# WilliamYi96/HGR-Net

Hardware: AMD Instinct MI355X
Metric: images/sec over 21K-class hierarchy, batch 512; hit@1 parity vs reference (higher is better)
Workload: dtype f16

## Files before the change

hgr-net_amd/_lib.py:

```python
from __future__ import annotations

import ctypes as C
import os
from pathlib import Path

import torch

_HERE = Path(__file__).resolve().parent
LIB_PATH = Path(os.environ.get("HGR_LIB", _HERE / "lib" / "libhgr.so"))

HGR_BF16, HGR_F16 = 0, 1
EPI_NONE, EPI_BIAS, EPI_BIAS_QUICKGELU, EPI_BIAS_RESIDUAL, EPI_BIAS_RELU, EPI_BIAS_ADD16_RELU, EPI_ACCUM, EPI_QGELU_GRAD16 = 0, 1, 2, 3, 4, 5, 6, 7

_p, _i, _l, _f = C.c_void_p, C.c_int, C.c_int64, C.c_float

SIGNATURES = {
    "hgr_gemm_nt": [_p, _l, _p, _l, _p, _l, _p, _p, _l, _i, _i, _i, _i, _i, _i, _p],
    "hgr_gemm_set_tile": [_i],
    "hgr_gemm_set_tail": [_i, _i],
    "hgr_gemm_set_persist": [_i],
    "hgr_gemm_set_p8": [_i],
    "hgr_im2col_patches": [_p, _p, _i, _i, _i, _i, _i, _p],
    "hgr_im2col_patches_ex": [_p, _p, _i, _i, _i, _i, _i, _i, _i, _p],
    "hgr_vit_assemble": [_p, _p, _p, _i, _i, _i, _p],
    "hgr_preprocess_bicubic": [_p, _p, _p, _p, _p, _p, _i, _p, _p, _i, _p, _p, C.POINTER(C.c_float), C.POINTER(C.c_float), _i, _i, _p],
    "hgr_im2col_patches_u8": [_p, _p, _i, _i, _i, _i, _i, _i, C.POINTER(C.c_float), C.POINTER(C.c_float), _i, _p],
    "hgr_vit_embed_ln": [_p, _p, _p, _p, _p, _p, _i, _i, _i, _f, _p],
    "hgr_layernorm": [_p, _p, _p, _p, _i, _i, _l, _p, _f, _i, _i, _p],
    "hgr_mha": [_p, _p, _i, _i, _i, _i, _i, _p],
    "hgr_mha_rows": [_p, _p, _i, _i, _i, _i, _i, _i, _p],
    "hgr_mha_stats": [_p, _p, _p, _i, _i, _i, _i, _i, _p],
    "hgr_text_embed": [_p, _l, _p, _p, _p, _i, _i, _i, _i, _p],
    "hgr_eot_index": [_p, _l, _p, _i, _i, _p],
    "hgr_l2norm_rows": [_p, _p, _p, _i, _i, _i, _p],
    "hgr_topk_rows": [_p, _l, _p, _i, _i, _p, _p, _i, _p],
    "hgr_level_argmax": [_p, _l, _p, _i, _p, _i, _p, _p, _i, _p],
    "hgr_eval_rows": [_p, _l, _i, _p, _p, _p, _i, _i, _p, _p, _p, _i, _i, _p, _p, _p, _i, _p],
    "hgr_conv3x3_nhwc": [_p, _p, _p, _p, _i, _i, _i, _i, _i, _i, _i, _i, _p],
    "hgr_conv3x3_pool2_nhwc": [_p, _p, _p, _p, _i, _i, _i, _i, _i, _i, _i, _p],
    "hgr_stem_conv1": [_p, _p, _p, _p, _i, _i, _i, _i, _i, _p],
    "hgr_stem_im2col": [_p, _p, _i, _i, _i, _p],
    "hgr_avgpool2_nhwc": [_p, _p, _i, _i, _i, _i, _i, _p],
    "hgr_attnpool_tokens": [_p, _p, _p, _i, _i, _i, _i, _p],
    "hgr_attnpool_attend": [_p, _p, _p, _p, _i, _i, _i, _i, _p],
    "hgr_stem7_pool": [_p, _p, _p, _p, _i, _i, _i, _i, _p],
    "hgr_stem7_im2col": [_p, _p, _i, _i, _i, _i, _p],
    "hgr_maxpool3s2_nhwc": [_p, _p, _i, _i, _i, _i, _i, _p],
    "hgr_subsample2_nhwc": [_p, _p, _i, _i, _i, _i, _i, _p],
    "hgr_meanpool_nhwc": [_p, _p, _i, _i, _i, _i, _i, _i, _p],
    "hgr_transpose16": [_p, _l, _p, _l, _i, _i, _p],
    "hgr_transpose16_colsum": [_p, _l, _p, _l, _i, _i, _i, _p, _i, _f, _p, _p],
    "hgr_colsum": [_p, _l, _i, _i, _i, _i, _p, _i, _f, _p, _p],
    "hgr_cast16": [_p, _p, _l, _i, _p],
    "hgr_cast16_transpose": [_p, _l, _p, _l, _p, _l, _i, _i, _i, _p],
    "hgr_quickgelu16": [_p, _p, _p, _l, _i, _i, _p],
    "hgr_layernorm_bwd": [_p, _i, _p, _p, _p, _p, _p, _p, _i, _i, _l, _p, _f, _i, _p],
    "hgr_layernorm_bwd_cast": [_p, _i, _p, _p, _p, _p, _p, _p, _p, _i, _i, _l, _p, _f, _i, _p],
    "hgr_layernorm_bwd_cast_colsum": [_p, _i, _p, _p, _p, _p, _p, _p, _p, _p, _i, _i, _l, _p, _f, _i, _p],
    "hgr_layernorm_bwd_scratch_floats": [_i, _i],
    "hgr_mha_bwd": [_p, _p, _p, _p, _i, _i, _i, _i, _i, _p],
    "hgr_mha_bwd_stats": [_p, _p, _p, _p, _p, _i, _i, _i, _i, _i, _p],
    "hgr_mha_bwd_colsum": [_p, _p, _p, _p, _p, _p, _i, _i, _i, _i, _i, _p],
    "hgr_ce_rows": [_p, _l, _p, _i, _i, _f, _p, _p, _l, _p],
    "hgr_l2norm_bwd": [_p, _p, _p, _i, _i, _i, _p],
    "hgr_matmul_f32": [_p, _l, _l, _p, _l, _l, _p, _l, _i, _i, _i, _f, _i, _p],
    "hgr_embed_scatter_add": [_p, _l, _p, _p, _i, _i, _i, _i, _p],
    "hgr_rows_axpy": [_p, _l, _p, _p, _i, _i, _f, _p],
    "hgr_rows_gather": [_p, _p, _p, _i, _i, _p],
    "hgr_ctx_splice": [_p, _p, _p, _i, _i, _i, _i, _p],
    "hgr_ctx_splice_bwd": [_p, _p, _i, _i, _i, _i, _p],
    "hgr_sumsq": [_p, _l, _p, _p],
    "hgr_eval_counters": [_p, _i, _p, _i, _p, _p, _i, _p, _p, _i, _p, _i, _p],
    "hgr_eval_counters_rows": [_p, _i, _p, _p, _p, _i, _p, _p, _p, _i, _p, _i, _p],
    "hgr_eval_report_rows": [_p, _i, _p, _p, _p, _i, _p, _p, _p, _i, _p, _i, _p],
    "hgr_path_scores": [_p, _l, _p, _l, _i, _p, _p, _p, _i, _p],
    "hgr_subtree_hedge": [_p, _l, _i, _p, _p, _p, _f, _p, _i, _p, _p, _p, _l, _i, _p],
    "hgr_hedge_counters_rows": [_p, _i, _p, _p, _p, _i, _p, _i, _p],
    "hgr_set_ranks": [_p, _l, _i, _p, _p, _i, _p, _p, _p, _i, _p],
    "hgr_set_counters_rows": [_p, _p, _i, _p, _p, _i, _p, _p, _p, _i, _p, _i, _p],
    "hgr_dgp_score_rows": [_p, _l, _i, _i, _i, _f, _p, _i, _p, _i, _p, _p, _p, _p, _i, _i, _p],
    "hgr_dot_f32":[_p, _p, _l, _p, _f, _i, _p],
    "hgr_conv3x3_nhwc_plain": [_p, _p, _p, _i, _i, _i, _i, _i, _i, _i, _p],
    "hgr_gemm_nt_splitk": [_p, _l, _p, _l, _p, _l, _i, _i, _i, _i, _i, _p],
    "hgr_gemm_tn_splitk": [_p, _l, _p, _l, _p, _l, _i, _i, _i, _i, _i, _p],
    "hgr_gemm_tn_tile": [_i, _i],
    "hgr_gemm_plan_capture": [_p, _i],
    "hgr_conv3x3_wgrad_splitk": [_p, _l, _p, _p, _l, _i, _i, _i, _i, _i, _i, _i, _p],
    "hgr_relu_bwd16": [_p, _p, _p, _l, _i, _p],
    "hgr_add16": [_p, _p, _p, _l, _i, _p],
    "hgr_avgpool2_bwd_nhwc": [_p, _p, _i, _i, _i, _i, _i, _p],
    "hgr_attnpool_tokens_bwd": [_p, _p, _i, _i, _i, _i, _p],
    "hgr_im2col3x3_t": [_p, _p, _i, _i, _i, _i, _l, _i, _p],
    "hgr_bn_fold": [_p, _p, _p, _p, _p, _f, _p, _p, _i, _i, _i, _i, _i, _p],
    "hgr_bn_unfold_grad": [_p, _l, _p, _p, _p, _p, _p, _f, _p, _p, _p, _i, _i, _i, _p],
    "hgr_csr_group_aggregate": [_p, _l, _p, _p, _p, _p, _i, _p, _p, _p, _p, _i, _p, _p, _p, _p, _i, _p, _p, _l, _i, _f, _i, _p],
    "hgr_csr_group_att_grad": [_p, _l, _p, _p, _l, _p, _l, _p, _l, _p, _p, _p, _p, _i, _p, _p, _p, _i, _p, _p, _p, _i, _p, _p, _i, _f, _p],
    "hgr_dgp_loss_head": [_p, _l, _p, _p, _l, _i, _i, _p, _p, _p, _l, _i, _p],
    "hgr_dropout_counter": [_p, _l, _p, _l, _i, _i, _i, _i, _i, _p],
    "hgr_adam_l2": [_p, _p, _p, _p, _l, _f, _f, _f, _f, _f, _i, _p],
    "hgr_cnzsl_std_chain_fwd": [_p, _l, _p, _p, _p, _p, _p, _p, _l, _p, _l, _p, _i, _i, _i, _f, _f, _p],
    "hgr_cnzsl_std_chain_bwd": [_p, _l, _p, _l, _p, _l, _p, _p, _p, _l, _p, _i, _i, _f, _p],
    "hgr_bias_relu_f32": [_p, _l, _p, _p, _l, _i, _i, _p],
    "hgr_relu_bwd_colsum_f32": [_p, _l, _p, _l, _p, _l, _p, _p, _i, _i, _p],
    "hgr_gemm_nt_res_stats": [_p, _l, _p, _l, _p, _p, _l, _p, _p, _i, _i, _i, _i, _p],
    "hgr_vit_head": [_p, _p, _l, _l, _p, _p, _f, _p, _p, _i, _i, _i, _i, _p],
    "hgr_gemm_nt_res_stats_guard": [_p, _l, _p, _l, _p, _p, _l, _p, _p, _f, _p, _i, _i, _i, _i, _p],
    "hgr_gemm_nt_res_stats_wide_ok": [_l, _l, _l, _l, _l, _l, _i],
    "hgr_gemm_nt_res_stats_wide": [_p, _l, _p, _l, _p, _p, _l, _p, _p, _f, _p, _i, _i, _i, _i, _p],
    "hgr_gemm_nt_ln": [_p, _l, _p, _l, _p, _l, _p, _p, _p, _f, _i, _i, _i, _i, _i, _p],
    "hgr_gemm_nt_ln_mha": [_p, _l, _p, _l, _p, _p, _p, _f, _p, _l, _i, _i, _i, _i, _i, _p],
    "hgr_gemm_nt_bias_gelu_dual": [_p, _l, _p, _l, _p, _l, _p, _l, _p, _i, _i, _i, _i, _p],
    "hgr_gemm_nt_qgelu_grad_colsum": [_p, _l, _p, _l, _p, _l, _p, _l, _p, _i, _i, _i, _i, _p],
    "hgr_vit_embed_ln_stats": [_p, _p, _p, _p, _p, _p, _p, _p, _i, _i, _i, _f, _i, _p],
    "hgr_vit_patch_embed_ln_ok": [_i, _i, _i, _i, _i],
    "hgr_vit_patch_embed_ln": [_p, _p, _p, _p, _p, _p, _p, _p, _p, _i, _i, _i, _i, _f, _i, _p],
    "hgr_row_stats16": [_p, _p, _p, _p, _i, _i, _i, _p],
    "hgr_pair_rows_f32": [_p, _p, _p, _i, _i, _l, _p, _i, _p],
    "hgr_logits_eval_workspace_bytes": [_i, _i],
    "hgr_logits_eval": [_p, _p, _i, _i, _i, _p, _p, _p, _i, _p, _p, _i, _p, _i, _i, _p, _p, _p, _p, _i, _p],
    "hgr_logits_eval_tile_stage": [_p, _p, _i, _i, _i, _p, _p, _p, _i, _p, _p, _i, _p, _i, _i, _p, _p, _p, _p, _i, _p],
    "hgr_logits_eval_row_stage": [_p, _p, _i, _i, _i, _p, _p, _p, _i, _p, _p, _i, _p, _i, _i, _p, _p, _p, _p, _i, _p],
    "hgr_comm_unique_id": [_p],
    "hgr_comm_init": [_i, _i, _p],
    "hgr_comm_destroy": [],
    "hgr_comm_rank": [],
    "hgr_comm_world": [],
    "hgr_allreduce": [_p, _p, _l, _i, _i, _p],
    "hgr_allgather": [_p, _p, _l, _i, _p],
    "hgr_broadcast": [_p, _l, _i, _i, _p],
    "hgr_adamw": [_p, _p, _p, _p, _l, _f, _f, _f, _f, _f, _i, _p, _f, _f, _p],
    "hgr_normal_counter": [_p, _l, _p, _i, _i, _i, _i, _l, _p],
    "hgr_free_gen_input": [_p, _l, _i, _p, _l, _p, _l, _i, _p, _i, _i, _i, _i, _i, _i, _i, _l, _p],
    "hgr_bias_act_rows": [_p, _l, _p, _p, _l, _l, _i, _i, _i, _i, _p],
    "hgr_free_fr_tail": [_p, _l, _p, _p, _l, _p, _l, _l, _i, _p, _l, _i, _i, _i, _i, _l, _p],
    "hgr_nll_rows16": [_p, _l, _p, _i, _i, _p, _p, _l, _p, _l, _i, _p],
    "hgr_adam_l2_cast16": [_p, _p, _l, _i, _f, _p, _p, _p, _l, _f, _f, _f, _f, _f, _i, _i, _p],
}


class GemmLaunch(C.Structure):
    _fields_ = [(name, C.c_int32) for name in ("kernel", "variant", "epilogue", "out_f32", "act", "grid_x", "grid_y", "tiles_m", "tiles_n", "total",
                                                "nbig", "big_panels", "tiles_m_half", "group", "m_fastest", "vec_ok", "row0", "rows")]


class HgrError(RuntimeError):
    pass


_lib = None


ABI_VERSION = 5


def load() -> C.CDLL:
    global _lib
    if _lib is not None:
        return _lib
    if not LIB_PATH.is_file():
        raise HgrError(f"{LIB_PATH} not found: build it with `python -c 'import __graft_entry__ as g; g.build()'` "
                       f"or `make -C {_HERE / 'csrc'}`; there is no CPU fallback")
    lib = C.CDLL(str(LIB_PATH))
    lib.hgr_abi_version.restype = _i
    lib.hgr_last_error.restype = C.c_char_p
    for name, argtypes in SIGNATURES.items():
        fn = getattr(lib, name)
        fn.argtypes = argtypes
        fn.restype = _l if name.endswith(("_scratch_floats", "_workspace_bytes")) else _i
    if lib.hgr_abi_version() != ABI_VERSION:
        raise HgrError(f"libhgr.so ABI {lib.hgr_abi_version()} != {ABI_VERSION} (include/hgr.h): stale build, run `make -C {_HERE / 'csrc'}`")
    _lib = lib
    return lib


import threading

_tls = threading.local()


def set_muted(on: bool) -> bool:
    prev = getattr(_tls, "muted", False)
    _tls.muted = bool(on)
    return prev


def muted() -> bool:
    return getattr(_tls, "muted", False)


def call(name: str, *args) -> None:
    if getattr(_tls, "muted", False):
        return
    lib = load()
    rc = getattr(lib, name)(*args)
    if rc != 0:
        raise HgrError(f"{name} failed ({rc}): {lib.hgr_last_error().decode()}")
```

hgr-net_amd/clip/model.py:

```python
from __future__ import annotations

import os
from collections import OrderedDict
from typing import Dict, Optional, Tuple, Union

import numpy as np
import torch
from torch import nn

from .. import ops
from .._lib import (EPI_BIAS, EPI_BIAS_ADD16_RELU, EPI_BIAS_QUICKGELU, EPI_BIAS_RELU, EPI_BIAS_RESIDUAL, EPI_NONE,
                    HgrError)


class QuickGELU(nn.Module):
    """Placeholder so ``mlp`` keeps the reference's child names (c_fc, gelu, c_proj); the activation
    itself is fused into the c_fc GEMM epilogue (HGR_EPI_BIAS_QUICKGELU)."""


class ResidualAttentionBlock(nn.Module):
    def __init__(self, d_model: int, n_head: int):
        super().__init__()
        self.attn = nn.MultiheadAttention(d_model, n_head)
        self.ln_1 = nn.LayerNorm(d_model)
        self.mlp = nn.Sequential(OrderedDict([("c_fc", nn.Linear(d_model, d_model * 4)), ("gelu", QuickGELU()),
                                              ("c_proj", nn.Linear(d_model * 4, d_model))]))
        self.ln_2 = nn.LayerNorm(d_model)


class Transformer(nn.Module):
    def __init__(self, width: int, layers: int, heads: int):
        super().__init__()
        self.width, self.layers, self.heads = width, layers, heads
        self.resblocks = nn.Sequential(*[ResidualAttentionBlock(width, heads) for _ in range(layers)])


class VisionTransformer(nn.Module):
    def __init__(self, input_resolution: int, patch_size: int, width: int, layers: int, heads: int, output_dim: int):
        super().__init__()
        self.input_resolution, self.output_dim, self.patch_size = input_resolution, output_dim, patch_size
        self.conv1 = nn.Conv2d(3, width, kernel_size=patch_size, stride=patch_size, bias=False)
        scale = width ** -0.5
        grid = input_resolution // patch_size
        self.class_embedding = nn.Parameter(scale * torch.randn(width))
        self.positional_embedding = nn.Parameter(scale * torch.randn(grid * grid + 1, width))
        self.ln_pre = nn.LayerNorm(width)
        self.transformer = Transformer(width, layers, heads)
        self.ln_post = nn.LayerNorm(width)
        self.proj = nn.Parameter(scale * torch.randn(width, output_dim))


class _Bottleneck(nn.Module):
    def __init__(self, inplanes, planes, stride=1):
        super().__init__()
        self.conv1 = nn.Conv2d(inplanes, planes, 1, bias=False)
        self.bn1 = nn.BatchNorm2d(planes)
        self.conv2 = nn.Conv2d(planes, planes, 3, padding=1, bias=False)
        self.bn2 = nn.BatchNorm2d(planes)
        self.conv3 = nn.Conv2d(planes, planes * 4, 1, bias=False)
        self.bn3 = nn.BatchNorm2d(planes * 4)
        self.stride = stride
        self.downsample = None
        if stride > 1 or inplanes != planes * 4:
            self.downsample = nn.Sequential(OrderedDict([("-1", nn.AvgPool2d(stride)),
                                                         ("0", nn.Conv2d(inplanes, planes * 4, 1, bias=False)),
                                                         ("1", nn.BatchNorm2d(planes * 4))]))


class _AttentionPool2d(nn.Module):
    def __init__(self, spacial_dim, embed_dim, num_heads, output_dim):
        super().__init__()
        self.positional_embedding = nn.Parameter(torch.randn(spacial_dim ** 2 + 1, embed_dim) / embed_dim ** 0.5)
        self.k_proj = nn.Linear(embed_dim, embed_dim)
        self.q_proj = nn.Linear(embed_dim, embed_dim)
        self.v_proj = nn.Linear(embed_dim, embed_dim)
        self.c_proj = nn.Linear(embed_dim, output_dim)
        self.num_heads = num_heads


class ModifiedResNet(nn.Module):

    def __init__(self, layers, output_dim, heads, input_resolution=224, width=64):
        super().__init__()
        self.output_dim, self.input_resolution = output_dim, input_resolution
        self.conv1 = nn.Conv2d(3, width // 2, 3, stride=2, padding=1, bias=False)
        self.bn1 = nn.BatchNorm2d(width // 2)
        self.conv2 = nn.Conv2d(width // 2, width // 2, 3, padding=1, bias=False)
        self.bn2 = nn.BatchNorm2d(width // 2)
        self.conv3 = nn.Conv2d(width // 2, width, 3, padding=1, bias=False)
        self.bn3 = nn.BatchNorm2d(width)
        inplanes = width
        for li, nb in enumerate(layers):
            planes = width * 2 ** li
            blocks = [_Bottleneck(inplanes, planes, 1 if li == 0 else 2)]
            inplanes = planes * 4
            blocks += [_Bottleneck(inplanes, planes) for _ in range(1, nb)]
            setattr(self, f"layer{li + 1}", nn.Sequential(*blocks))
        self.attnpool = _AttentionPool2d(input_resolution // 32, width * 32, heads, output_dim)


def _w16(t: torch.Tensor, dt: torch.dtype) -> torch.Tensor:
    return t.detach().to(dt).contiguous()


def _f32(t: torch.Tensor) -> torch.Tensor:
    return t.detach().float().contiguous()


class _Block16:

    def __init__(self, blk: ResidualAttentionBlock, dt: torch.dtype):
        self.ln1 = (_f32(blk.ln_1.weight), _f32(blk.ln_1.bias))
        self.ln2 = (_f32(blk.ln_2.weight), _f32(blk.ln_2.bias))
        self.w_in, self.b_in = _w16(blk.attn.in_proj_weight, dt), _f32(blk.attn.in_proj_bias)
        self.w_out, self.b_out = _w16(blk.attn.out_proj.weight, dt), _f32(blk.attn.out_proj.bias)
        self.w_fc, self.b_fc = _w16(blk.mlp.c_fc.weight, dt), _f32(blk.mlp.c_fc.bias)
        self.w_proj, self.b_proj = _w16(blk.mlp.c_proj.weight, dt), _f32(blk.mlp.c_proj.bias)
        self.wf_in, self.s_in, self.c_in = self._fold(blk.attn.in_proj_weight, blk.attn.in_proj_bias, blk.ln_1, dt)
        self.wf_fc, self.s_fc, self.c_fc = self._fold(blk.mlp.c_fc.weight, blk.mlp.c_fc.bias, blk.ln_2, dt)
        self.eps1, self.eps2 = float(blk.ln_1.eps), float(blk.ln_2.eps)

    @staticmethod
    def _fold(w, b, ln, dt):
        w32, g32, be32 = w.detach().float(), ln.weight.detach().float(), ln.bias.detach().float()
        wf = (w32 * g32[None, :]).to(dt).contiguous()
        return wf, wf.float().sum(dim=1).contiguous(), (w32 @ be32 + b.detach().float()).contiguous()


class _Workspace:

    def __init__(self):
        self._b: Dict[str, torch.Tensor] = {}
        self.epoch = 0

    def const(self, name: str, build) -> torch.Tensor:
        t = self._b.get("const." + name)
        if t is None:
            t = self._b["const." + name] = build()
            self.epoch += 1
        return t

    def get(self, name: str, shape, dtype, device) -> torch.Tensor:
        n = int(np.prod(shape))
        t = self._b.get(name)
        if t is None or t.numel() < n or t.dtype != dtype or t.device != device:
            t = torch.empty(n, dtype=dtype, device=device)
            self._b[name] = t
            self.epoch += 1
        return t[:n].view(*shape)


IMG_STREAMS = max(1, int(os.environ.get("HGR_IMG_STREAMS", "1")))
IMG_STREAMS_MIN_ROWS = 8192
CLS_LAST = os.environ.get("HGR_CLS_LAST", "1") != "0"
LN_FUSED = os.environ.get("HGR_LN_FUSED", "1") != "0"
QKV_MHA = os.environ.get("HGR_QKV_MHA", "1") != "0"
PATCH_FUSED = os.environ.get("HGR_PATCH_FUSED", "1") != "0"
PROJ_WIDE = {"0": 0, "2": 2}.get(os.environ.get("HGR_PROJ_WIDE", "1"), 1)
_CUS: Dict[int, int] = {}


def _proj_wide_wanted(m: int, n: int, k: int, dev: torch.device) -> bool:
    if PROJ_WIDE != 1:
        return PROJ_WIDE == 2
    idx = dev.index if dev.index is not None else torch.cuda.current_device()
    cus = _CUS.get(idx)
    if cus is None:
        cus = _CUS[idx] = torch.cuda.get_device_properties(idx).multi_processor_count
    return k >= 1024 and (m // 320) * (n // 256) * 8 >= 7 * cus


def ln_fusable(w: int, m: int = 0) -> bool:
    return LN_FUSED and w % 128 == 0 and m * 4 * w * 2 < 2 ** 32


def _run_blocks(x: Optional[torch.Tensor], blocks, heads: int, b: int, l: int, causal: bool, dt: torch.dtype, ws: _Workspace, tag: str,
                taps: Optional[dict] = None, tap_prefix: str = "", pair=None, stats: Optional[torch.Tensor] = None,
                flag: Optional[torch.Tensor] = None, cls_only_last: bool = False):
    m, w = (pair[0] if pair is not None else x).shape
    dev = (pair[0] if pair is not None else x).device
    qkv = ws.get(tag + ".qkv", (m, 3 * w), dt, dev)
    att = ws.get(tag + ".att", (m, w), dt, dev)
    u16 = ws.get(tag + ".u16", (m, 4 * w), dt, dev)
    if pair is not None:
        xh, xl = pair
        for i, k in enumerate(blocks):
            last_cls = cls_only_last and i == len(blocks) - 1 and l > 1 and 3 * w * l < (1 << 23)
            fused_attn = QKV_MHA and not last_cls and ops.ln_mha_ok(w, l, m, xh.stride(0))
            if last_cls:
                ch, cl = xh.view(b, l, w)[:, 0, :], xl.view(b, l, w)[:, 0, :]
                ops.gemm_nt_ln(xh, k.wf_in[w:], qkv[:, w:], k.s_in[w:], k.c_in[w:], stats, k.eps1, tag="kv")
                ops.split_point("class_token_tail")
                st_q = ws.get(tag + ".stats_q", (b, w // 64, 2), torch.float32, dev)
                idx = ws.const(f"cls_rows.{b}.{l}", lambda: (torch.arange(b, dtype=torch.int32, device=dev) * l).contiguous())
                ops.rows_gather(stats.view(b * l, -1), idx, st_q.view(b, -1))
                ops.gemm_nt_ln(ch, k.wf_in[:w], qkv.view(b, l, 3 * w)[:, 0, :w], k.s_in[:w], k.c_in[:w], st_q, k.eps1, tag="q_cls")
            elif fused_attn:
                ops.gemm_nt_ln_mha(xh, k.wf_in, att, k.s_in, k.c_in, stats, b, l, heads, causal, k.eps1)
            else:
                ops.gemm_nt_ln(xh, k.wf_in, qkv, k.s_in, k.c_in, stats, k.eps1, tag="qkv")
            if not fused_attn:
                ops.mha(qkv, att, b, l, heads, causal, q_rows=1 if last_cls else 0)
            if last_cls:
                ca = att.view(b, l, w)[:, 0, :]
                st_c = ws.get(tag + ".stats_cls", (b, w // 64, 2), torch.float32, dev)
                u_c = ws.get(tag + ".u16_cls", (b, 4 * w), dt, dev)
                ops.gemm_nt_res_stats(ca, k.w_out, ch, cl, k.b_out, st_c, tag="out_cls", flag=flag)
                ops.gemm_nt_ln(ch, k.wf_fc, u_c, k.s_fc, k.c_fc, st_c, k.eps2, quickgelu=True, tag="fc_cls")
                ops.gemm_nt_res_stats(u_c, k.w_proj, ch, cl, k.b_proj, st_c, tag="proj_cls", flag=flag)
                break
            ops.gemm_nt_res_stats(att, k.w_out, xh, xl, k.b_out, stats, tag="out", flag=flag)
            ops.gemm_nt_ln(xh, k.wf_fc, u16, k.s_fc, k.c_fc, stats, k.eps2, quickgelu=True, tag="fc")
            if (PROJ_WIDE and ops.gemm_nt_res_stats_wide_ok(m, w, 4 * w, u16.stride(0), k.w_proj.stride(0), xh.stride(0), dt)
                    and _proj_wide_wanted(m, w, 4 * w, dev)):
                ops.gemm_nt_res_stats_wide(u16, k.w_proj, xh, xl, k.b_proj, stats, tag="proj", flag=flag)
            else:
                ops.gemm_nt_res_stats(u16, k.w_proj, xh, xl, k.b_proj, stats, tag="proj", flag=flag)
            if taps is not None:
                taps[f"{tap_prefix}.resblocks.{i}"] = ops.pair_value(xh, xl).view(b, l, w)
        return None
    h16 = ws.get(tag + ".h16", (m, w), dt, dev)
    for i, k in enumerate(blocks):
        ops.layernorm(x, k.ln1[0], k.ln1[1], h16)
        ops.gemm_nt(h16, k.w_in, qkv, bias=k.b_in, epilogue=EPI_BIAS)
        ops.mha(qkv, att, b, l, heads, causal)
        ops.gemm_nt(att, k.w_out, x, bias=k.b_out, residual=x, epilogue=EPI_BIAS_RESIDUAL)
        ops.layernorm(x, k.ln2[0], k.ln2[1], h16)
        ops.gemm_nt(h16, k.w_fc, u16, bias=k.b_fc, epilogue=EPI_BIAS_QUICKGELU)
        ops.gemm_nt(u16, k.w_proj, x, bias=k.b_proj, residual=x, epilogue=EPI_BIAS_RESIDUAL)
        if taps is not None:
            taps[f"{tap_prefix}.resblocks.{i}"] = x.view(b, l, w).clone()
    return x



def _cpad(c: int) -> int:
    return (c + 63) // 64 * 64


def _fold(conv: nn.Conv2d, bn: nn.BatchNorm2d, dt: torch.dtype, cin_p: Optional[int] = None, cout_p: Optional[int] = None):
    w = conv.weight.detach().float()
    s = bn.weight.detach().float() / torch.sqrt(bn.running_var.detach().float() + bn.eps)
    b = bn.bias.detach().float() - bn.running_mean.detach().float() * s
    w = (w * s.view(-1, 1, 1, 1)).permute(0, 2, 3, 1)
    cout, kh, kw, cin = w.shape
    cin_p, cout_p = cin_p or cin, cout_p or cout
    k = kh * kw * cin_p
    kp = (k + 63) // 64 * 64
    out = torch.zeros(cout_p, kp, dtype=dt, device=w.device)
    out[:cout, :k].view(cout, kh, kw, cin_p)[..., :cin] = w.to(dt)
    bias = torch.zeros(cout_p, dtype=torch.float32, device=w.device)
    bias[:cout] = b
    return out.contiguous(), bias.contiguous()


class _RNBlock16:
    def __init__(self, blk, dt):
        cin, pl = blk.conv1.weight.shape[1], blk.conv1.weight.shape[0]
        cin_p, pl_p = _cpad(cin), _cpad(pl)
        self.c1 = _fold(blk.conv1, blk.bn1, dt, cin_p, pl_p)
        self.c2 = _fold(blk.conv2, blk.bn2, dt, pl_p, pl_p)
        self.c3 = _fold(blk.conv3, blk.bn3, dt, pl_p, None)
        self.down = _fold(blk.downsample[1], blk.downsample[2], dt, cin_p, None) if blk.downsample is not None else None
        self.stride = blk.stride
        self.planes = pl_p
        self.out = blk.conv3.weight.shape[0]


def _rn_prepare(v: "ModifiedResNet", dt: torch.dtype) -> dict:
    width = v.conv3.weight.shape[0]
    if width % 16:
        raise NotImplementedError(f"RN width {width}: channel counts must be multiples of 8 (the stem runs at width / 2)")
    p = {"stem": [_fold(v.conv1, v.bn1, dt), _fold(v.conv2, v.bn2, dt), _fold(v.conv3, v.bn3, dt, None, _cpad(width))]}
    p["blocks"] = [_RNBlock16(b, dt) for li in (1, 2, 3, 4) for b in getattr(v, f"layer{li}")]
    a = v.attnpool
    p["pos"] = _f32(a.positional_embedding)
    for nm in ("q_proj", "k_proj", "v_proj", "c_proj"):
        lin = getattr(a, nm)
        p[nm] = (_w16(lin.weight, dt), _f32(lin.bias))
    return p


def _rn_forward(v: "ModifiedResNet", p: dict, image: torch.Tensor, dt: torch.dtype, ws: _Workspace) -> torch.Tensor:
    dev = image.device
    b, _, r, _ = image.shape
    width = p["stem"][2][0].shape[0]
    h = (r - 1) // 2 + 1
    m = b * h * h
    (w1, b1), (w2, b2), (w3, b3) = p["stem"]
    a1 = ws.get("r.a", (m, w1.shape[0]), dt, dev)
    if r % 4 == 0 and w1.shape[0] <= 48:
        ops.stem_conv1(image, w1, b1, a1)
    else:
        col = ws.get("r.col", (m, 64), dt, dev)
        ops.stem_im2col(image, col)
        ops.gemm_nt(col, w1, a1, bias=b1, epilogue=EPI_BIAS_RELU)
    a2 = ws.get("r.b", (m, w2.shape[0]), dt, dev)
    ops.conv3x3_nhwc(a1, w2, b2, a2, b, h, h, w1.shape[0])
    if w2.shape[0] == 32 and width == 64 and h % 2 == 0:
        h //= 2
        x = ws.get("r.x0", (b * h * h, width), dt, dev)
        ops.conv3x3_pool2_nhwc(a2, w3, b3, x, b, 2 * h, 2 * h, 32)
    else:
        a3 = ws.get("r.c", (m, w3.shape[0]), dt, dev)
        ops.conv3x3_nhwc(a2, w3, b3, a3, b, h, h, w2.shape[0])
        h //= 2
        x = ws.get("r.x0", (b * h * h, width), dt, dev)
        ops.avgpool2_nhwc(a3, x, b, 2 * h, 2 * h, width)
    cin, flip = width, 0
    for k in p["blocks"]:
        m = b * h * h
        pl = k.planes
        t1 = ws.get("r.t1", (m, pl), dt, dev)
        ops.gemm_nt(x, k.c1[0], t1, bias=k.c1[1], epilogue=EPI_BIAS_RELU)
        t2 = ws.get("r.t2", (m, pl), dt, dev)
        ops.conv3x3_nhwc(t1, k.c2[0], k.c2[1], t2, b, h, h, pl)
        ho = h // k.stride
        mo = b * ho * ho
        xin = x
        if k.stride > 1:
            t2p = ws.get("r.t2p", (mo, pl), dt, dev)
            ops.avgpool2_nhwc(t2, t2p, b, h, h, pl)
            t2 = t2p
            if k.down is not None:
                xin = ws.get("r.xp", (mo, cin), dt, dev)
                ops.avgpool2_nhwc(x, xin, b, h, h, cin)
        idn = xin
        if k.down is not None:
            idn = ws.get("r.idn", (mo, k.out), dt, dev)
            ops.gemm_nt(xin, k.down[0], idn, bias=k.down[1], epilogue=EPI_BIAS)
        out = ws.get(f"r.out{flip}", (mo, k.out), dt, dev)
        ops.gemm_nt(t2, k.c3[0], out, bias=k.c3[1], residual=idn, epilogue=EPI_BIAS_ADD16_RELU)
        x, cin, h, flip = out, k.out, ho, flip ^ 1
    a = v.attnpool
    e, l = cin, h * h + 1
    tok = ws.get("r.tok", (b * l, e), dt, dev)
    ops.attnpool_tokens(x, p["pos"], tok, b, h, e)
    kk = ws.get("r.k", (b * l, e), dt, dev)
    vv = ws.get("r.v", (b * l, e), dt, dev)
    ops.gemm_nt(tok, p["k_proj"][0], kk, bias=p["k_proj"][1], epilogue=EPI_BIAS)
    ops.gemm_nt(tok, p["v_proj"][0], vv, bias=p["v_proj"][1], epilogue=EPI_BIAS)
    q = ws.get("r.q", (b, e), torch.float32, dev)
    ops.gemm_nt(tok.view(b, l * e)[:, :e], p["q_proj"][0], q, bias=p["q_proj"][1], epilogue=EPI_BIAS)
    o16 = ws.get("r.o", (b, e), dt, dev)
    ops.attnpool_attend(q, kk, vv, o16, b, l, a.num_heads)
    out = torch.empty((b, v.output_dim), dtype=torch.float32, device=dev)
    ops.gemm_nt(o16, p["c_proj"][0], out, bias=p["c_proj"][1], epilogue=EPI_BIAS)
    return out

class CLIP(nn.Module):

    def __init__(self, embed_dim: int, image_resolution: int, vision_layers: Union[Tuple[int, int, int, int], int],
                 vision_width: int, vision_patch_size: int, context_length: int, vocab_size: int,
                 transformer_width: int, transformer_heads: int, transformer_layers: int,
                 image_dtype: str = "f16", text_dtype: str = "f16"):
        super().__init__()
        self.context_length = context_length
        if isinstance(vision_layers, (tuple, list)):
            self.visual = ModifiedResNet(vision_layers, embed_dim, vision_width * 32 // 64, image_resolution, vision_width)
        else:
            self.visual = VisionTransformer(image_resolution, vision_patch_size, vision_width, vision_layers,
                                            vision_width // 64, embed_dim)
        self.transformer = Transformer(transformer_width, transformer_layers, transformer_heads)
        self.vocab_size = vocab_size
        self.token_embedding = nn.Embedding(vocab_size, transformer_width)
        self.positional_embedding = nn.Parameter(torch.empty(context_length, transformer_width).normal_(std=0.01))
        self.ln_final = nn.LayerNorm(transformer_width)
        self.text_projection = nn.Parameter(torch.empty(transformer_width, embed_dim).normal_(std=transformer_width ** -0.5))
        self.logit_scale = nn.Parameter(torch.ones([]) * np.log(1 / 0.07))
        self.image_dtype = ops.TORCH16[ops.dtype_code(image_dtype)]
        self.text_dtype = ops.TORCH16[ops.dtype_code(text_dtype)]
        self.text_chunk = 8192
        self._prep: dict = {}
        self._ws = _Workspace()
        self._ln_flags: Optional[torch.Tensor] = None
        self._ln_off: set = set()
        self._ln_checked: dict = {}
        self._img_tag = "v"

    def _ln_flag(self, tower: str, dev) -> torch.Tensor:
        if self._ln_flags is None or self._ln_flags.device != torch.device(dev):
            self._ln_flags = torch.zeros(2, dtype=torch.int32, device=dev)
        i = 0 if tower == "v" else 1
        return self._ln_flags[i:i + 1]

    def ln_guard_tripped(self) -> dict:
        if self._ln_flags is None:
            return {}
        bits = self._ln_flags.cpu().numpy().view(np.uint32)
        vals = bits.view(np.float32)
        return {t: float(vals[i]) for i, t in enumerate(("image", "text")) if bits[i]}

    def _ln_check(self, tower: str, dev) -> bool:
        fp = self._prep.get("fp")
        if self._ln_checked.get(tower) == fp or torch.cuda.is_current_stream_capturing():
            return False
        self._ln_checked[tower] = fp
        i = 0 if tower == "v" else 1
        bits = int(self._ln_flags[i].item()) & 0xFFFFFFFF
        if not bits:
            return False
        worst = float(np.array([bits], dtype=np.uint32).view(np.float32)[0])
        import warnings
        warnings.warn(f"hgr_net_amd: the {'image' if tower == 'v' else 'text'} tower's residual stream left the range the 16-bit LayerNorm-folded path "
                      f"is guarded for (a 64-column slot with sum of squares {worst:g} > {ops.LN_GUARD_SUMSQ:g}): this tower now runs with the fp32 "
                      f"stream and separate LayerNorm launches (the HGR_LN_FUSED=0 path).")
        self._ln_off.add(tower)
        self._ln_flags[i] = 0
        return True

    LN_POLL_EVERY = 64

    def poll_ln_guard(self, force: bool = False) -> bool:
        self._ln_polls = getattr(self, "_ln_polls", 0) + 1
        if self._ln_flags is None or torch.cuda.is_current_stream_capturing() or not (force or self._ln_polls % self.LN_POLL_EVERY == 0):
            return False
        tripped = self.ln_guard_tripped()
        if not tripped:
            return False
        import warnings
        for name, worst in tripped.items():
            t = "v" if name == "image" else "t"
            self._ln_off.add(t)
            warnings.warn(f"hgr_net_amd: the {name} tower's residual stream left the range the 16-bit LayerNorm-folded path is guarded for AFTER its "
                          f"first-pass check (slot sum of squares {worst:g} > {ops.LN_GUARD_SUMSQ:g}); up to {self.LN_POLL_EVERY} batches since the previous "
                          f"poll may hold inf / NaN features.  This tower now runs with the fp32 stream and separate LayerNorm launches.")
        self._ln_flags.zero_()
        return True

    @property
    def dtype(self):
        return self.visual.conv1.weight.dtype

    def _fingerprint(self):
        return (ops.WEIGHTS_GEN[0],) + tuple((p.data_ptr(), p._version) for p in self.parameters())

    def _prepared(self) -> dict:
        fp = self._fingerprint()
        if self._prep.get("fp") != fp:
            p: dict = {"fp": fp}
            self._ln_off.clear()
            self._ln_checked.clear()
            v = self.visual
            if isinstance(v, VisionTransformer):
                dt = self.image_dtype
                k = 3 * v.patch_size * v.patch_size
                kp = (k + 63) // 64 * 64
                wc = torch.zeros(v.conv1.weight.shape[0], kp, dtype=dt, device=v.conv1.weight.device)
                wc[:, :k] = v.conv1.weight.detach().reshape(v.conv1.weight.shape[0], -1).to(dt)
                p["conv_w"], p["kp"] = wc, kp
                p["conv_w_nhwc"] = v.conv1.weight.detach().permute(0, 2, 3, 1).reshape(v.conv1.weight.shape[0], -1).to(dt).contiguous()
                p["cls"], p["pos"] = _f32(v.class_embedding), _f32(v.positional_embedding)
                p["ln_pre"] = (_f32(v.ln_pre.weight), _f32(v.ln_pre.bias))
                p["ln_post"] = (_f32(v.ln_post.weight), _f32(v.ln_post.bias))
                p["proj_t"] = _w16(v.proj.detach().t(), dt)
                p["vblocks"] = [_Block16(b, dt) for b in v.transformer.resblocks]
            else:
                p["rn"] = _rn_prepare(v, self.image_dtype)
            dt = self.text_dtype
            p["tok"], p["tpos"] = _f32(self.token_embedding.weight), _f32(self.positional_embedding)
            p["ln_final"] = (_f32(self.ln_final.weight), _f32(self.ln_final.bias))
            p["tproj_t"] = _w16(self.text_projection.detach().t(), dt)
            p["tblocks"] = [_Block16(b, dt) for b in self.transformer.resblocks]
            self._prep = p
        return self._prep

    @torch.no_grad()
    def encode_image(self, image: torch.Tensor, taps: Optional[dict] = None) -> torch.Tensor:
        v = self.visual
        if not image.is_cuda:
            raise HgrError("encode_image needs a device tensor: the product path has no CPU fallback")
        p = self._prepared()
        dt, ws, dev = self.image_dtype, self._ws, image.device
        u8 = image.dtype == torch.uint8
        if u8:
            if not isinstance(v, VisionTransformer) or image.dim() != 4 or image.shape[-1] != 3 or (3 * v.patch_size ** 2) % 64:
                raise NotImplementedError("uint8 NHWC input is implemented for ViT towers with 3*P*P % 64 == 0")
            image = image.contiguous()
            b, r = image.shape[0], image.shape[1]
        else:
            image = image.float().contiguous()
            b, _, r, _ = image.shape
        if r != v.input_resolution:
            raise ValueError(f"expected {v.input_resolution}x{v.input_resolution} input, got {r}")
        if not isinstance(v, VisionTransformer):
            return _rn_forward(v, p["rn"], image, dt, ws)
        self.poll_ln_guard()
        out = torch.empty((b, v.output_dim), dtype=torch.float32, device=dev)
        ns = IMG_STREAMS if (taps is None and b >= 2 * IMG_STREAMS and b * (r // v.patch_size) ** 2 >= IMG_STREAMS_MIN_ROWS) else 1
        if ns == 1:
            tag = self._img_tag
            fused = self._vit_forward(image, p, out, tag, taps, u8)
            if fused and self._ln_check("v", dev):
                self._vit_forward(image, p, out, tag, taps, u8)
            return out
        main = torch.cuda.current_stream()
        side = self._side_streams(ns - 1, dev)
        cut = [b * i // ns for i in range(ns + 1)]
        fused = False
        for i in range(ns):
            st = main if i == 0 else side[i - 1]
            if i:
                st.wait_stream(main)
            with torch.cuda.stream(st):
                fused |= self._vit_forward(image[cut[i]:cut[i + 1]], p, out[cut[i]:cut[i + 1]], f"v{i}" if i else "v", None, u8)
        for st in side:
            main.wait_stream(st)
        if fused and self._ln_check("v", dev):
            self._vit_forward(image, p, out, "v", None, u8)
# ... 136 lines not shown
```

hgr-net_amd/csrc/hgr_gemm_common.h:

```cpp
#pragma once
#include "hgr_common.h"
#include <stdlib.h>
#include <type_traits>

namespace hgr_gemm {

constexpr int BK = 64;

struct GemmArgs {
    const char *A = nullptr; int64_t lda = 0;
    const char *W = nullptr; int64_t ldw = 0;
    void *C = nullptr; int64_t ldc = 0;
    const float *bias = nullptr;
    const float *res = nullptr; int64_t ldr = 0;
    int M = 0, N = 0, K = 0;
    int tiles_m = 0, tiles_n = 0;
    int m_fastest = 0;
    int vec_ok = 0;
    int dbg = 0;
    int cH = 0, cW = 0, cC = 0, cStride = 0, cHo = 0, cWo = 0;
    unsigned cMagic = 0;
    int cUni = 0;
    int kc = 0; int64_t csplit = 0;
    float *ln_stats = nullptr; int ln_slots = 0; float ln_eps = 0.f;
    void *ln_xh = nullptr, *ln_xl = nullptr; int64_t ln_ldx = 0;
    const float *ln_s = nullptr, *ln_c = nullptr;
    unsigned *ln_flag = nullptr; float ln_guard = 0.f;
    int group = 0;
    int nbig = 0, big_panels = 0, tiles_m_half = 0;
    float *colsum = nullptr; int colsum_units = 0;
    int total = 0;
};

inline int gemm_m_fastest(int M, int N, int K) { return (int64_t)N * K > (int64_t)M * K ? 1 : 0; }
inline GemmArgs gemm_args(const void *A, int64_t lda, const void *W, int64_t ldw, void *C, int64_t ldc, int M, int N, int K, bool vec_ok, int dbg) {
    GemmArgs a;
    a.A = (const char *)A; a.lda = lda; a.W = (const char *)W; a.ldw = ldw; a.C = C; a.ldc = ldc;
    a.M = M; a.N = N; a.K = K;
    a.m_fastest = gemm_m_fastest(M, N, K); a.vec_ok = vec_ok ? 1 : 0; a.dbg = dbg;
    return a;
}


static __device__ __attribute__((aligned(16))) unsigned int hgr_zero_page[4] = {0u, 0u, 0u, 0u};

__device__ __forceinline__ float quick_gelu(float v) {
    return v * __builtin_amdgcn_rcpf(1.0f + __builtin_amdgcn_exp2f(-1.702f * 1.4426950408889634f * v));
}


template <int DT> __device__ __forceinline__ typename T16<DT>::elem quick_gelu16(float v) {
    return mul16<DT>(v, __builtin_amdgcn_rcpf(1.0f + __builtin_amdgcn_exp2f(-1.702f * 1.4426950408889634f * v)));
}
template <int DT> __device__ __forceinline__ typename T16<DT>::elem quick_gelu_train16(float x) {
    const float z = 1.702f * x;
    return mul16<DT>(x, __builtin_amdgcn_rcpf(1.0f + __builtin_amdgcn_exp2f(-1.4426950408889634f * z)));
}
__device__ __forceinline__ float quick_gelu_grad(float x) {
    const float s = __builtin_amdgcn_rcpf(1.0f + __builtin_amdgcn_exp2f(-1.702f * 1.4426950408889634f * x));
    return s * (1.0f + 1.702f * x * (1.0f - s));
}
__device__ __forceinline__ float2 ln_finalize(float s1, float s2, float inv_k, float eps) {
    const float mean = s1 * inv_k;
    const float msq = mean * mean;
    return make_float2(mean, rsqrtf(fmaxf(__builtin_fmaf(s2, inv_k, -msq), 0.f) + eps));
}
__device__ __forceinline__ float ln_apply(float2 mr, float acc, float s_n, float c_n) {
    return __builtin_fmaf(mr.y, __builtin_fmaf(-mr.x, s_n, acc), c_n);
}

template <int DT, bool GELU> __device__ __forceinline__ u32x2 ln_out16(float2 mr, f32x4 acc, f32x4 s4, f32x4 c4);

constexpr float QG_K = -1.702f * 1.4426950408889634f;
__device__ __forceinline__ float ln_apply_gelu(float2 mr, float acc, float s_n, float c_n) {
    const float w = __builtin_fmaf(mr.y * QG_K, __builtin_fmaf(-mr.x, s_n, acc), c_n * QG_K);
    return w * __builtin_amdgcn_rcpf(__builtin_fmaf(QG_K, __builtin_amdgcn_exp2f(w), QG_K));
}

template <int DT, bool GELU> __device__ __forceinline__ u32x2 ln_out16(float2 mr, f32x4 acc, f32x4 s4, f32x4 c4) {
    u32x2 o;
    if (GELU) {
        const float rk = mr.y * QG_K;
        float w[4], r[4];
#pragma unroll
        for (int e = 0; e < 4; ++e) {
            w[e] = __builtin_fmaf(rk, __builtin_fmaf(-mr.x, s4[e], acc[e]), c4[e] * QG_K);
            r[e] = __builtin_amdgcn_rcpf(__builtin_fmaf(QG_K, __builtin_amdgcn_exp2f(w[e]), QG_K));
        }
        o[0] = mul_pack16<DT>(w[0], r[0], w[1], r[1]);
        o[1] = mul_pack16<DT>(w[2], r[2], w[3], r[3]);
    } else {
        float u[4];
#pragma unroll
        for (int e = 0; e < 4; ++e) u[e] = __builtin_fmaf(-mr.x, s4[e], acc[e]);
        o[0] = fma_pack16<DT>(mr.y, u[0], c4[0], mr.y, u[1], c4[1]);
        o[1] = fma_pack16<DT>(mr.y, u[2], c4[2], mr.y, u[3], c4[3]);
    }
    return o;
}

__host__ __device__ constexpr bool epi_has_bias(int epi) { return epi != HGR_EPI_NONE && epi != HGR_EPI_ACCUM && epi != HGR_EPI_QGELU_GRAD16; }
__host__ __device__ constexpr bool epi_has_idn16(int epi) { return epi == HGR_EPI_BIAS_ADD16_RELU || epi == HGR_EPI_QGELU_GRAD16; }

template <int DT, int EPI, bool OUT32>
__device__ __forceinline__ void store_quad(const GemmArgs &p, f32x4 v, int m, int n) {
    typedef typename T16<DT>::elem E;
    if (n + 3 < p.N && p.vec_ok) {
        if (epi_has_bias(EPI)) v += *(const f32x4 *)(p.bias + n);
        if (EPI == HGR_EPI_ACCUM) v += *(const f32x4 *)((const float *)p.C + (int64_t)m * p.ldc + n);
        const f32x4 v0 = v;
        f32x4 gq = (f32x4){0.f, 0.f, 0.f, 0.f};
        if (EPI == HGR_EPI_BIAS_QUICKGELU) {
#pragma unroll
            for (int e = 0; e < 4; ++e) v[e] = quick_gelu(v[e]);
        }
        if (EPI == HGR_EPI_BIAS_RESIDUAL) v += *(const f32x4 *)(p.res + (int64_t)m * p.ldr + n);
        if (epi_has_idn16(EPI)) {
            const typename T16<DT>::vec4 idn = *(const typename T16<DT>::vec4 *)((const E *)(const void *)p.res + (int64_t)m * p.ldr + n);
#pragma unroll
            for (int e = 0; e < 4; ++e) {
                if (EPI == HGR_EPI_QGELU_GRAD16) { gq[e] = quick_gelu_grad((float)idn[e]); v[e] = v[e] * gq[e]; }
                else v[e] = v[e] + (float)idn[e];
            }
        }
        if (EPI == HGR_EPI_BIAS_RELU || EPI == HGR_EPI_BIAS_ADD16_RELU) {
#pragma unroll
            for (int e = 0; e < 4; ++e) v[e] = fmaxf(v[e], 0.f);
        }
        if (OUT32) *(f32x4 *)((float *)p.C + (int64_t)m * p.ldc + n) = v;
        else if (EPI == HGR_EPI_BIAS_QUICKGELU || EPI == HGR_EPI_QGELU_GRAD16) {
            typename T16<DT>::vec4 o;
#pragma unroll
            for (int e = 0; e < 4; ++e) o[e] = EPI == HGR_EPI_BIAS_QUICKGELU ? quick_gelu16<DT>(v0[e]) : mul16<DT>(v0[e], gq[e]);
            *(typename T16<DT>::vec4 *)((E *)p.C + (int64_t)m * p.ldc + n) = o;
        } else *(typename T16<DT>::vec4 *)((E *)p.C + (int64_t)m * p.ldc + n) = cvt4<DT>(v[0], v[1], v[2], v[3]);
        return;
    }
    for (int e = 0; e < 4 && n + e < p.N; ++e) {
        float x = v[e];
        if (epi_has_bias(EPI)) x += p.bias[n + e];
        if (EPI == HGR_EPI_ACCUM) x += ((const float *)p.C)[(int64_t)m * p.ldc + n + e];
        const float x0 = x;
        float gx = 0.f;
        if (EPI == HGR_EPI_BIAS_QUICKGELU) x = quick_gelu(x);
        if (EPI == HGR_EPI_BIAS_RESIDUAL) x += p.res[(int64_t)m * p.ldr + n + e];
        if (EPI == HGR_EPI_BIAS_ADD16_RELU) x += (float)((const E *)(const void *)p.res)[(int64_t)m * p.ldr + n + e];
        if (EPI == HGR_EPI_QGELU_GRAD16) { gx = quick_gelu_grad((float)((const E *)(const void *)p.res)[(int64_t)m * p.ldr + n + e]); x *= gx; }
        if (EPI == HGR_EPI_BIAS_RELU || EPI == HGR_EPI_BIAS_ADD16_RELU) x = fmaxf(x, 0.f);
        if (OUT32) ((float *)p.C)[(int64_t)m * p.ldc + n + e] = x;
        else if (EPI == HGR_EPI_BIAS_QUICKGELU) ((E *)p.C)[(int64_t)m * p.ldc + n + e] = quick_gelu16<DT>(x0);
        else if (EPI == HGR_EPI_QGELU_GRAD16) ((E *)p.C)[(int64_t)m * p.ldc + n + e] = mul16<DT>(x0, gx);
        else ((E *)p.C)[(int64_t)m * p.ldc + n + e] = (E)x;
    }
}

template <int DT, int EPI>
__device__ __forceinline__ f32x4 load_addend(const GemmArgs &p, int m, int n) {
    typedef typename T16<DT>::elem E;
    if (EPI == HGR_EPI_ACCUM) return *(const f32x4 *)((const float *)p.C + (int64_t)m * p.ldc + n);
    if (EPI == HGR_EPI_BIAS_RESIDUAL) return *(const f32x4 *)(p.res + (int64_t)m * p.ldr + n);
    if (epi_has_idn16(EPI)) {
        const typename T16<DT>::vec4 idn = *(const typename T16<DT>::vec4 *)((const E *)(const void *)p.res + (int64_t)m * p.ldr + n);
        return (f32x4){(float)idn[0], (float)idn[1], (float)idn[2], (float)idn[3]};
    }
    return (f32x4){0.f, 0.f, 0.f, 0.f};
}

template <int DT, int EPI, bool OUT32>
__device__ __forceinline__ void store_quad_full(const GemmArgs &p, f32x4 v, f32x4 bq, f32x4 addend, int m, int n) {
    typedef typename T16<DT>::elem E;
    if (epi_has_bias(EPI)) v += bq;
    if (!OUT32 && (EPI == HGR_EPI_BIAS_QUICKGELU || EPI == HGR_EPI_QGELU_GRAD16)) {
        typename T16<DT>::vec4 o;
#pragma unroll
        for (int e = 0; e < 4; ++e) o[e] = EPI == HGR_EPI_BIAS_QUICKGELU ? quick_gelu16<DT>(v[e]) : mul16<DT>(v[e], quick_gelu_grad(addend[e]));
        *(typename T16<DT>::vec4 *)((E *)p.C + (int64_t)m * p.ldc + n) = o;
        return;
    }
    if (EPI == HGR_EPI_BIAS_QUICKGELU) {
#pragma unroll
        for (int e = 0; e < 4; ++e) v[e] = quick_gelu(v[e]);
    }
    if (EPI == HGR_EPI_ACCUM || EPI == HGR_EPI_BIAS_RESIDUAL || EPI == HGR_EPI_BIAS_ADD16_RELU) v += addend;
    if (EPI == HGR_EPI_QGELU_GRAD16) {
#pragma unroll
        for (int e = 0; e < 4; ++e) v[e] *= quick_gelu_grad(addend[e]);
    }
    if (EPI == HGR_EPI_BIAS_RELU || EPI == HGR_EPI_BIAS_ADD16_RELU) {
#pragma unroll
        for (int e = 0; e < 4; ++e) v[e] = fmaxf(v[e], 0.f);
    }
    if (OUT32) *(f32x4 *)((float *)p.C + (int64_t)m * p.ldc + n) = v;
    else *(typename T16<DT>::vec4 *)((E *)p.C + (int64_t)m * p.ldc + n) = cvt4<DT>(v[0], v[1], v[2], v[3]);
}


__device__ __forceinline__ __amdgpu_buffer_rsrc_t dma_rsrc(const void *base) {
    return __builtin_amdgcn_make_buffer_rsrc(const_cast<void *>(base), 0, (int)0xFFFFFFFFu, 0x00020000);
}
__device__ __forceinline__ void dma16(__amdgpu_buffer_rsrc_t rsrc, unsigned voff, int soff, char *lds_dst) {
    __builtin_amdgcn_raw_ptr_buffer_load_lds(rsrc, (AS3 void *)lds_dst, 16, (int)voff, soff, 0, 0);
}

template <int N> __device__ __forceinline__ void rwait() {
    static_assert(N >= 0 && N <= 63, "vmcnt is a 6-bit field");
    __builtin_amdgcn_sched_barrier(0);
    asm volatile("s_waitcnt vmcnt(%0) lgkmcnt(0)\n\ts_barrier" ::"n"(N) : "memory");
    __builtin_amdgcn_sched_barrier(0);
}
#define HGR_RWAIT(N) hgr_gemm::rwait<N>()
#define HGR_RBAR() do { __builtin_amdgcn_sched_barrier(0); \
    asm volatile("s_waitcnt lgkmcnt(0)\n\ts_barrier" ::: "memory"); __builtin_amdgcn_sched_barrier(0); } while (0)
#define HGR_MBAR() do { __builtin_amdgcn_sched_barrier(0); \
    asm volatile("s_barrier" ::: "memory"); __builtin_amdgcn_sched_barrier(0); } while (0)


template <int NR, int NW, int NV, int M_, int NM = 16>
__device__ __forceinline__ void mfma16_interleave_step() {
    if constexpr (M_ < NM) {
        __builtin_amdgcn_sched_group_barrier(0x008, 1, 0);
        constexpr int DR = (M_ + 1) * NR / NM - M_ * NR / NM, DW = (M_ + 1) * NW / NM - M_ * NW / NM, DV = (M_ + 1) * NV / NM - M_ * NV / NM;
        if constexpr (DR > 0) __builtin_amdgcn_sched_group_barrier(0x100, DR, 0);
        if constexpr (DW > 0) __builtin_amdgcn_sched_group_barrier(0x200, DW, 0);
        if constexpr (DV > 0) __builtin_amdgcn_sched_group_barrier(0x020, DV, 0);
        mfma16_interleave_step<NR, NW, NV, M_ + 1, NM>();
    }
}
template <int NR, int NW, int NV>
__device__ __forceinline__ void mfma16_interleave() { mfma16_interleave_step<NR, NW, NV, 0>(); }
template <int NR, int NW, int NV>
__device__ __forceinline__ void mfma8_interleave() { mfma16_interleave_step<NR, NW, NV, 0, 8>(); }


__device__ __forceinline__ int xcd_first_tile(int ntiles, int xcd) {
    const int q8 = ntiles >> 3, r8 = ntiles & 7;
    return xcd < r8 ? xcd * (q8 + 1) : r8 * (q8 + 1) + (xcd - r8) * q8;
}
__device__ __forceinline__ int xcd_tile_count(int ntiles, int xcd) { return (ntiles >> 3) + (xcd < (ntiles & 7) ? 1 : 0); }

__device__ __forceinline__ void ln_row_sums(const f32x4 *sp, int slots, float &s1, float &s2) {
    float a1 = 0.f, a2 = 0.f;
    auto fixed = [&](auto nq_tag) {
        constexpr int NQ = decltype(nq_tag)::value;
        f32x4 t[NQ];
#pragma unroll
        for (int i = 0; i < NQ; ++i) t[i] = sp[i];
#pragma unroll
        for (int i = 0; i < NQ; ++i) { a1 += t[i][0] + t[i][2]; a2 += t[i][1] + t[i][3]; }
    };
    switch (slots) {
        case 4: fixed(std::integral_constant<int, 2>()); break;
        case 8: fixed(std::integral_constant<int, 4>()); break;
        case 10: fixed(std::integral_constant<int, 5>()); break;
        case 12: fixed(std::integral_constant<int, 6>()); break;
        case 16: fixed(std::integral_constant<int, 8>()); break;
        default:
            for (int i = 0; i < slots / 2; ++i) { const f32x4 t = sp[i]; a1 += t[0] + t[2]; a2 += t[1] + t[3]; }
    }
    s1 = a1; s2 = a2;
}

template <int DT> __device__ __forceinline__ void pair_pass_values(f32x4 lo4, f32x4 hi4, f32x4 b8lo, f32x4 b8hi, typename T16<DT>::vec8 oh, u32x2 ol, float (&v)[8]) {
    v[0] = (lo4[0] + b8lo[0]) + pair_dec4<DT, 0>(oh[0], ol[0]); v[1] = (lo4[1] + b8lo[1]) + pair_dec4<DT, 1>(oh[1], ol[0]);
    v[2] = (lo4[2] + b8lo[2]) + pair_dec4<DT, 2>(oh[2], ol[0]); v[3] = (lo4[3] + b8lo[3]) + pair_dec4<DT, 3>(oh[3], ol[0]);
    v[4] = (hi4[0] + b8hi[0]) + pair_dec4<DT, 0>(oh[4], ol[1]); v[5] = (hi4[1] + b8hi[1]) + pair_dec4<DT, 1>(oh[5], ol[1]);
    v[6] = (hi4[2] + b8hi[2]) + pair_dec4<DT, 2>(oh[6], ol[1]); v[7] = (hi4[3] + b8hi[3]) + pair_dec4<DT, 3>(oh[7], ol[1]);
}
template <int DT> __device__ __forceinline__ void pair_pass_split(const float (&v)[8], u32x4 &nh, u32x2 &nl) {
    unsigned tq[8];
#pragma unroll
    for (int e2 = 0; e2 < 4; ++e2) nh[e2] = pair_split2<DT>(v[2 * e2], v[2 * e2 + 1], tq[2 * e2], tq[2 * e2 + 1]);
    unsigned n0, n1;
    pair_put_q<DT, 0>(n0, tq[0]); pair_put_q<DT, 1>(n0, tq[1]); pair_put_q<DT, 2>(n0, tq[2]); pair_put_q<DT, 3>(n0, tq[3]);
    pair_put_q<DT, 0>(n1, tq[4]); pair_put_q<DT, 1>(n1, tq[5]); pair_put_q<DT, 2>(n1, tq[6]); pair_put_q<DT, 3>(n1, tq[7]);
    nl = (u32x2){n0, n1};
}
__device__ __forceinline__ void pair_pass_sums(const float (&v)[8], float &s1, float &s2) {
    s1 = ((v[0] + v[1]) + (v[2] + v[3])) + ((v[4] + v[5]) + (v[6] + v[7]));
    s2 = (__builtin_fmaf(v[0], v[0], v[1] * v[1]) + __builtin_fmaf(v[2], v[2], v[3] * v[3])) +
         (__builtin_fmaf(v[4], v[4], v[5] * v[5]) + __builtin_fmaf(v[6], v[6], v[7] * v[7]));
}
template <int CTRL> __device__ __forceinline__ void pair_pass_dpp_stage(float (&s1)[2], float (&s2)[2]) {
#pragma unroll
    for (int q = 0; q < 2; ++q) {
        s1[q] += __builtin_bit_cast(float, __builtin_amdgcn_update_dpp(0, __builtin_bit_cast(int, s1[q]), CTRL, 0xF, 0xF, true));
        s2[q] += __builtin_bit_cast(float, __builtin_amdgcn_update_dpp(0, __builtin_bit_cast(int, s2[q]), CTRL, 0xF, 0xF, true));
    }
}
__device__ __forceinline__ void pair_pass_reduce(float (&s1)[2], float (&s2)[2]) {
    pair_pass_dpp_stage<0xB1>(s1, s2); pair_pass_dpp_stage<0x4E>(s1, s2); pair_pass_dpp_stage<0x141>(s1, s2);
}

template <int DT, int MT, int MODE, int PA, int PW0, int PW1, typename Issue1, typename Issue2>
__device__ __forceinline__ void pingpong_ktile(const char *st, int offA, int offW, int sw0, int sw1, f32x4 (&acc)[MT][8],
                                               typename T16<DT>::vec8 (&wf)[4][2], typename T16<DT>::vec8 (&af)[MT][2], Issue1 issue1, Issue2 issue2) {
    typedef typename T16<DT>::vec8 vec8;
#pragma unroll
    for (int j = 0; j < 4; ++j) {
        wf[j][0] = *(const vec8 *)(st + PW0 + offW + j * 2048 + sw0);
        wf[j][1] = *(const vec8 *)(st + PW0 + offW + j * 2048 + sw1);
    }
#pragma unroll
    for (int i = 0; i < MT; ++i) {
        af[i][0] = *(const vec8 *)(st + PA + offA + i * 2048 + sw0);
        af[i][1] = *(const vec8 *)(st + PA + offA + i * 2048 + sw1);
    }
    if (MODE <= 1) issue1();
    if (MODE <= 1) rwait<MT + 4>(); else rwait<0>();
    __builtin_amdgcn_s_setprio(1);
#pragma unroll
    for (int kk = 0; kk < 2; ++kk)
#pragma unroll
        for (int i = 0; i < MT; ++i)
#pragma unroll
            for (int j = 0; j < 4; ++j) acc[i][j] = T16<DT>::mfma16(wf[j][kk], af[i][kk], acc[i][j]);
    __builtin_amdgcn_s_setprio(0);
    HGR_MBAR();
#pragma unroll
    for (int j = 0; j < 4; ++j) {
        wf[j][0] = *(const vec8 *)(st + PW1 + offW + j * 2048 + sw0);
        wf[j][1] = *(const vec8 *)(st + PW1 + offW + j * 2048 + sw1);
    }
    if (MODE == 0) issue2();
    if (MODE == 0) rwait<MT + 4>(); else if (MODE == 1) rwait<2>(); else HGR_RBAR();
    __builtin_amdgcn_s_setprio(1);
#pragma unroll
    for (int kk = 0; kk < 2; ++kk)
#pragma unroll
        for (int i = 0; i < MT; ++i)
#pragma unroll
            for (int j = 0; j < 4; ++j) acc[i][4 + j] = T16<DT>::mfma16(wf[j][kk], af[i][kk], acc[i][4 + j]);
    __builtin_amdgcn_s_setprio(0);
    HGR_MBAR();
}

enum { V128_PLAIN = 0, V128_TALL = 1, V128_CONV = 2, V128_CONV_TALL = 3 };
void launch_128(const GemmArgs &a, int dtype, int epi, bool out32, int variant, dim3 grid, hipStream_t s);
void launch_256(const GemmArgs &a, int dtype, int epi, bool out32, bool conv, dim3 grid, hipStream_t s);
void launch_duo(const GemmArgs &a, int dtype, int epi, bool out32, int ln, dim3 grid, hipStream_t s);
bool p8_covers(int M, int N, int K);
void launch_p8(const GemmArgs &a, int dtype, int act, dim3 grid, hipStream_t s);

struct SlabArgs {
    const char *A = nullptr; int64_t lda = 0;
    const char *W = nullptr; int64_t ldw = 0;
    int M = 0, K = 0, Np = 0;
    const int *tpos = nullptr, *epos = nullptr;
    unsigned long long *ev_key = nullptr;
    float *ev_tmax = nullptr, *ev_m2 = nullptr; int *ev_p1 = nullptr;
    int S = 0;
    int dbg = 0;
};
void launch_logits_slab(const SlabArgs &a, int dtype, hipStream_t s);

}
```

hgr-net_amd/csrc/hgr_norm.hip:

```cpp
#include "hgr_launch.h"

namespace {

constexpr int MAXV = 16;

template <int DT, bool OUT32, int NV>
__global__ __launch_bounds__(256) void layernorm_rows(const float *__restrict__ x, const float *__restrict__ gamma,
                                                      const float *__restrict__ beta, void *__restrict__ y,
                                                      int rows, int W, int64_t row_mul, const int32_t *__restrict__ row_idx, float eps) {
    const int lane = threadIdx.x & 63;
    const int row = blockIdx.x * 4 + (threadIdx.x >> 6);
    if (row >= rows) return;
    const int64_t src = (int64_t)row * row_mul + (row_idx ? row_idx[row] : 0);
    const f32x4 *xr = (const f32x4 *)(x + src * W);
    const int nv = W >> 2;
    f32x4 v[NV];
    float s = 0.f;
#pragma unroll
    for (int i = 0; i < NV; ++i) {
        const int c = i * 64 + lane;
        if (i * 64 < nv) {
            v[i] = (c < nv) ? xr[c] : (f32x4){0.f, 0.f, 0.f, 0.f};
            s += v[i][0] + v[i][1] + v[i][2] + v[i][3];
        }
    }
    const float mean = wave_sum(s) / (float)W;
    float q = 0.f;
#pragma unroll
    for (int i = 0; i < NV; ++i) {
        const int c = i * 64 + lane;
        if (i * 64 < nv && c < nv) {
#pragma unroll
            for (int e = 0; e < 4; ++e) { const float d = v[i][e] - mean; q += d * d; }
        }
    }
    const float rstd = rsqrtf(wave_sum(q) / (float)W + eps);
    const f32x4 *gv = (const f32x4 *)gamma, *bv = (const f32x4 *)beta;
#pragma unroll
    for (int i = 0; i < NV; ++i) {
        const int c = i * 64 + lane;
        if (i * 64 < nv && c < nv) {
            const f32x4 ga = gv[c], be = bv[c];
            f32x4 o;
#pragma unroll
            for (int e = 0; e < 4; ++e) o[e] = (v[i][e] - mean) * rstd * ga[e] + be[e];
            if (OUT32) ((f32x4 *)((float *)y + (int64_t)row * W))[c] = o;
            else ((typename T16<DT>::vec4 *)((typename T16<DT>::elem *)y + (int64_t)row * W))[c] = cvt4<DT>(o[0], o[1], o[2], o[3]);
        }
    }
}

template <int NV, int DT = HGR_F16, bool STATS = false>
__global__ __launch_bounds__(256) void vit_embed_ln(const float *__restrict__ patches, const float *__restrict__ cls,
                                                    const float *__restrict__ pos, const float *__restrict__ gamma,
                                                    const float *__restrict__ beta, float *__restrict__ x,
                                                    int B, int G, int W, float eps, void *__restrict__ xh = nullptr, void *__restrict__ xl = nullptr,
                                                    float *__restrict__ stats = nullptr) {
    const int lane = threadIdx.x & 63;
    const int L = G + 1;
    const int row = blockIdx.x * 4 + (threadIdx.x >> 6);
    if (row >= B * L) return;
    const int b = row / L, t = row - b * L;
    const f32x4 *src = (const f32x4 *)(t == 0 ? cls : patches + ((int64_t)b * G + (t - 1)) * W);
    const f32x4 *pr = (const f32x4 *)(pos + (int64_t)t * W);
    const int nv = W >> 2;
    f32x4 v[NV];
    float s = 0.f;
#pragma unroll
    for (int i = 0; i < NV; ++i) {
        const int c = i * 64 + lane;
        if (i * 64 < nv) {
            v[i] = (c < nv) ? (src[c] + pr[c]) : (f32x4){0.f, 0.f, 0.f, 0.f};
            s += v[i][0] + v[i][1] + v[i][2] + v[i][3];
        }
    }
    HGR_VIT_LN_ROW_BODY
}

template <int DT>
__global__ __launch_bounds__(256) void row_stats16(const float *__restrict__ x, void *__restrict__ xh, void *__restrict__ xl, float *__restrict__ stats, int rows, int W) {
    const int lane = threadIdx.x & 63;
    const int row = blockIdx.x * 4 + (threadIdx.x >> 6);
    if (row >= rows) return;
    const f32x4 *xr = (const f32x4 *)(x + (int64_t)row * W);
    const int nv = W >> 2;
    for (int c0 = 0; c0 < nv; c0 += 64) {
        const int c = c0 + lane;
        const bool ok = c < nv;
        const f32x4 v = ok ? xr[c] : (f32x4){0.f, 0.f, 0.f, 0.f};
        const float s1 = row16_sum((v[0] + v[1]) + (v[2] + v[3]));
        const float s2 = row16_sum((v[0] * v[0] + v[1] * v[1]) + (v[2] * v[2] + v[3] * v[3]));
        if (ok) {
            typename T16<DT>::vec4 nh;
            unsigned nl = 0u;
#pragma unroll
            for (int e = 0; e < 4; ++e) { unsigned q; typename T16<DT>::elem h; pair_split<DT>(v[e], h, q); nh[e] = h; nl |= q << (8 * e); }
            ((typename T16<DT>::vec4 *)((typename T16<DT>::elem *)xh + (int64_t)row * W))[c] = nh;
            ((unsigned *)((unsigned char *)xl + (int64_t)row * W))[c] = nl;
            if ((lane & 15) == 0) *(float2 *)(stats + ((int64_t)row * (W >> 6) + (c >> 4)) * 2) = make_float2(s1, s2);
        }
    }
}

template <int DT>
__global__ __launch_bounds__(256) void pair_rows_f32(const void *__restrict__ xh, const void *__restrict__ xl, float *__restrict__ out, int rows, int W,
                                                     int64_t row_mul, const int32_t *__restrict__ row_idx) {
    const int lane = threadIdx.x & 63;
    const int row = blockIdx.x * 4 + (threadIdx.x >> 6);
    if (row >= rows) return;
    const int64_t src = (int64_t)row * row_mul + (row_idx ? row_idx[row] : 0);
    for (int c = lane; c < (W >> 2); c += 64) {
        const typename T16<DT>::vec4 h = ((const typename T16<DT>::vec4 *)((const typename T16<DT>::elem *)xh + src * W))[c];
        const unsigned l = ((const unsigned *)((const unsigned char *)xl + src * W))[c];
        ((f32x4 *)(out + (int64_t)row * W))[c] = (f32x4){pair_dec<DT>(h[0], l & 255u), pair_dec<DT>(h[1], (l >> 8) & 255u), pair_dec<DT>(h[2], (l >> 16) & 255u), pair_dec<DT>(h[3], l >> 24)};
    }
}

template <int DT, int NV>
__global__ __launch_bounds__(256) void l2norm_rows(const float *__restrict__ x, void *__restrict__ y16, float *__restrict__ y32, int rows, int D) {
    const int lane = threadIdx.x & 63;
    const int row = blockIdx.x * 4 + (threadIdx.x >> 6);
    if (row >= rows) return;
    const f32x4 *xr = (const f32x4 *)(x + (int64_t)row * D);
    const int nv = D >> 2;
    f32x4 v[NV];
    float s = 0.f;
#pragma unroll
    for (int i = 0; i < NV; ++i) {
        const int c = i * 64 + lane;
        if (i * 64 < nv) {
            v[i] = (c < nv) ? xr[c] : (f32x4){0.f, 0.f, 0.f, 0.f};
            s += v[i][0] * v[i][0] + v[i][1] * v[i][1] + v[i][2] * v[i][2] + v[i][3] * v[i][3];
        }
    }
    const float inv = 1.0f / sqrtf(wave_sum(s));
#pragma unroll
    for (int i = 0; i < NV; ++i) {
        const int c = i * 64 + lane;
        if (i * 64 < nv && c < nv) {
            const f32x4 o = v[i] * inv;
            if (y32) ((f32x4 *)(y32 + (int64_t)row * D))[c] = o;
            if (y16) ((typename T16<DT>::vec4 *)((typename T16<DT>::elem *)y16 + (int64_t)row * D))[c] = cvt4<DT>(o[0], o[1], o[2], o[3]);
        }
    }
}


template <int DT, int NV>
__global__ __launch_bounds__(256) void vit_head(const void *__restrict__ xh, const void *__restrict__ xl, int64_t ldx, int64_t row_mul,
                                                const float *__restrict__ gamma, const float *__restrict__ beta, float eps,
                                                const void *__restrict__ projt, float *__restrict__ out, int B, int W, int D) {
    typedef typename T16<DT>::elem E;
    typedef typename T16<DT>::vec8 vec8;
    typedef typename T16<DT>::vec4 vec4;
    extern __shared__ __attribute__((aligned(16))) char hs[];
    const int tid = threadIdx.x, lane = tid & 63, wave = tid >> 6;
    const int row0 = blockIdx.x * 16, col0 = blockIdx.y * 128;
    const int RS = W * 2 + 16;
    const int nv = W >> 2;
    const f32x4 *gv = (const f32x4 *)gamma, *bv = (const f32x4 *)beta;
    f32x4 v[4][NV];
#pragma unroll
    for (int q4 = 0; q4 < 4; ++q4) {
        const int row = min(row0 + wave * 4 + q4, B - 1);
        const E *ph = (const E *)xh + (int64_t)row * row_mul * ldx;
        const unsigned char *pl = (const unsigned char *)xl + (int64_t)row * row_mul * ldx;
#pragma unroll
        for (int i = 0; i < NV; ++i) {
            const int c = i * 64 + lane;
            if (i * 64 < nv) {
                const int cc = min(c, nv - 1);
                const vec4 h4 = ((const vec4 *)ph)[cc];
                const unsigned l4 = ((const unsigned *)pl)[cc];
#pragma unroll
                for (int e = 0; e < 4; ++e) v[q4][i][e] = c < nv ? pair_dec<DT>(h4[e], (l4 >> (8 * e)) & 255u) : 0.f;
            }
        }
    }
#pragma unroll
    for (int q4 = 0; q4 < 4; ++q4) {
        const int rr = wave * 4 + q4;
        float s = 0.f;
#pragma unroll
        for (int i = 0; i < NV; ++i)
            if (i * 64 < nv) s += v[q4][i][0] + v[q4][i][1] + v[q4][i][2] + v[q4][i][3];
        const float mean = wave_sum(s) / (float)W;
        float q = 0.f;
#pragma unroll
        for (int i = 0; i < NV; ++i) {
            const int c = i * 64 + lane;
            if (i * 64 < nv && c < nv) {
#pragma unroll
                for (int e = 0; e < 4; ++e) { const float d = v[q4][i][e] - mean; q += d * d; }
            }
        }
        const float rstd = rsqrtf(wave_sum(q) / (float)W + eps);
#pragma unroll
        for (int i = 0; i < NV; ++i) {
            const int c = i * 64 + lane;
            if (i * 64 < nv && c < nv) {
                const f32x4 ga = gv[c], be = bv[c];
                f32x4 o;
#pragma unroll
                for (int e = 0; e < 4; ++e) o[e] = (v[q4][i][e] - mean) * rstd * ga[e] + be[e];
                *(vec4 *)(hs + rr * RS + c * 8) = cvt4<DT>(o[0], o[1], o[2], o[3]);
            }
        }
    }
    __syncthreads();
    const int r = lane & 15, g = lane >> 4;
    f32x4 acc[2] = {(f32x4){0.f, 0.f, 0.f, 0.f}, (f32x4){0.f, 0.f, 0.f, 0.f}};
    const E *w0 = (const E *)projt + (int64_t)min(col0 + wave * 32 + r, D - 1) * W + g * 8;
    const E *w1 = (const E *)projt + (int64_t)min(col0 + wave * 32 + 16 + r, D - 1) * W + g * 8;
    const char *hb = hs + r * RS + g * 16;
    const int ks = W >> 5;
    for (int kk = 0; kk < ks; kk += 8) {
        vec8 f0[8], f1[8];
#pragma unroll
        for (int u = 0; u < 8; ++u) {
            const int kq = min(kk + u, ks - 1);
            f0[u] = *(const vec8 *)(w0 + kq * 32); f1[u] = *(const vec8 *)(w1 + kq * 32);
        }
#pragma unroll
        for (int u = 0; u < 8; ++u) {
            if (kk + u < ks) {
                const vec8 xf = *(const vec8 *)(hb + (kk + u) * 64);
                acc[0] = T16<DT>::mfma16(f0[u], xf, acc[0]);
                acc[1] = T16<DT>::mfma16(f1[u], xf, acc[1]);
            }
        }
    }
    if (row0 + r < B) {
#pragma unroll
        for (int t = 0; t < 2; ++t) {
            const int n = col0 + wave * 32 + t * 16 + g * 4;
            if (n + 3 < D) *(f32x4 *)(out + (int64_t)(row0 + r) * D + n) = acc[t];
            else
                for (int e = 0; e < 4 && n + e < D; ++e) out[(int64_t)(row0 + r) * D + n + e] = acc[t][e];
        }
    }
}

}

extern "C" int hgr_layernorm(const float *x, const float *gamma, const float *beta, void *y, int rows, int W,
                             int64_t row_mul, const int32_t *row_idx, float eps, int dtype, int out_f32, void *stream) {
    HGR_REQUIRE(x && gamma && beta && y, "hgr_layernorm: null operand");
    HGR_REQUIRE(rows >= 1 && W >= 4 && W % 4 == 0 && W <= 4 * 64 * MAXV, "hgr_layernorm: rows=%d W=%d unsupported (W %% 4 == 0, W <= %d)", rows, W, 4 * 64 * MAXV);
    HGR_REQUIRE(hgr_aligned(x, 16) && hgr_aligned(gamma, 16) && hgr_aligned(beta, 16) && hgr_aligned(y, 16), "hgr_layernorm: operands must be 16-byte aligned");
    HGR_REQUIRE(dtype == HGR_BF16 || dtype == HGR_F16, "hgr_layernorm: bad dtype %d", dtype);
    HGR_REQUIRE(row_mul >= 1, "hgr_layernorm: row_mul must be >= 1");
    dim3 grid((rows + 3) / 4), block(256);
    hipStream_t s = (hipStream_t)stream;
    hgr_by_nv_pow2((W / 4 + 63) / 64, [&](auto nv) {
        if (out_f32) hipLaunchKernelGGL((layernorm_rows<HGR_BF16, true, nv.value>), grid, block, 0, s, x, gamma, beta, y, rows, W, row_mul, row_idx, eps);
        else hgr_by_dtype(dtype, [&](auto dt) { hipLaunchKernelGGL((layernorm_rows<dt.value, false, nv.value>), grid, block, 0, s, x, gamma, beta, y, rows, W, row_mul, row_idx, eps); });
    });
    HGR_CHECK_LAUNCH("hgr_layernorm");
    return HGR_OK;
}

extern "C" int hgr_vit_embed_ln(const float *patches, const float *class_embedding, const float *positional_embedding,
                                const float *gamma, const float *beta, float *x, int B, int G, int W, float eps, void *stream) {
    HGR_REQUIRE(patches && class_embedding && positional_embedding && gamma && beta && x, "hgr_vit_embed_ln: null operand");
    HGR_REQUIRE(B >= 1 && G >= 1 && W >= 4 && W % 4 == 0 && W <= 4 * 64 * MAXV, "hgr_vit_embed_ln: B=%d G=%d W=%d unsupported", B, G, W);
    HGR_REQUIRE(hgr_aligned(patches, 16) && hgr_aligned(class_embedding, 16) && hgr_aligned(positional_embedding, 16) &&
                hgr_aligned(gamma, 16) && hgr_aligned(beta, 16) && hgr_aligned(x, 16), "hgr_vit_embed_ln: operands must be 16-byte aligned");
    const int rows = B * (G + 1);
    hgr_by_nv_pow2((W / 4 + 63) / 64, [&](auto nv) {
        hipLaunchKernelGGL((vit_embed_ln<nv.value>), dim3((rows + 3) / 4), dim3(256), 0, (hipStream_t)stream, patches, class_embedding, positional_embedding, gamma, beta, x, B, G, W, eps); });
    HGR_CHECK_LAUNCH("hgr_vit_embed_ln");
    return HGR_OK;
}

extern "C" int hgr_l2norm_rows(const float *x, void *y16, float *y32, int rows, int D, int dtype, void *stream) {
    HGR_REQUIRE(x && (y16 || y32), "hgr_l2norm_rows: null operand");
    HGR_REQUIRE(rows >= 1 && D >= 4 && D % 4 == 0 && D <= 4 * 64 * MAXV, "hgr_l2norm_rows: rows=%d D=%d unsupported", rows, D);
    HGR_REQUIRE(hgr_aligned(x, 16) && hgr_aligned(y16, 8) && hgr_aligned(y32, 16), "hgr_l2norm_rows: misaligned operand");
    HGR_REQUIRE(dtype == HGR_BF16 || dtype == HGR_F16, "hgr_l2norm_rows: bad dtype %d", dtype);
    dim3 grid((rows + 3) / 4), block(256);
    hgr_by_nv_pow2((D / 4 + 63) / 64, [&](auto nv) { hgr_by_dtype(dtype, [&](auto dt) {
        hipLaunchKernelGGL((l2norm_rows<dt.value, nv.value>), grid, block, 0, (hipStream_t)stream, x, y16, y32, rows, D); }); });
    HGR_CHECK_LAUNCH("hgr_l2norm_rows");
    return HGR_OK;
}


extern "C" int hgr_vit_embed_ln_stats(const float *patches, const float *class_embedding, const float *positional_embedding,
                                      const float *gamma, const float *beta, void *xh, void *xl, float *stats,
                                      int B, int G, int W, float eps, int dtype, void *stream) {
    HGR_REQUIRE(patches && class_embedding && positional_embedding && gamma && beta && xh && xl && stats, "hgr_vit_embed_ln_stats: null operand");
    HGR_REQUIRE(B >= 1 && G >= 1 && W >= 64 && W % 64 == 0 && W <= 4 * 64 * MAXV, "hgr_vit_embed_ln_stats: B=%d G=%d W=%d unsupported (W %% 64 == 0)", B, G, W);
    HGR_REQUIRE(hgr_aligned(patches, 16) && hgr_aligned(class_embedding, 16) && hgr_aligned(positional_embedding, 16) &&
                hgr_aligned(gamma, 16) && hgr_aligned(beta, 16) && hgr_aligned(xh, 8) && hgr_aligned(xl, 8) && hgr_aligned(stats, 8),
                "hgr_vit_embed_ln_stats: misaligned operand");
    HGR_REQUIRE(dtype == HGR_BF16 || dtype == HGR_F16, "hgr_vit_embed_ln_stats: bad dtype %d", dtype);
    const int rows = B * (G + 1);
    float *nox = nullptr;
    hgr_by_nv_pow2((W / 4 + 63) / 64, [&](auto nv) { hgr_by_dtype(dtype, [&](auto dt) {
        hipLaunchKernelGGL((vit_embed_ln<nv.value, dt.value, true>), dim3((rows + 3) / 4), dim3(256), 0, (hipStream_t)stream, patches, class_embedding, positional_embedding, gamma, beta, nox, B, G, W, eps, xh, xl, stats); }); });
    HGR_CHECK_LAUNCH("hgr_vit_embed_ln_stats");
    return HGR_OK;
}

extern "C" int hgr_row_stats16(const float *x, void *xh, void *xl, float *stats, int rows, int W, int dtype, void *stream) {
    HGR_REQUIRE(x && xh && xl && stats, "hgr_row_stats16: null operand");
    HGR_REQUIRE(rows >= 1 && W >= 64 && W % 64 == 0, "hgr_row_stats16: rows=%d W=%d unsupported (W %% 64 == 0)", rows, W);
    HGR_REQUIRE(hgr_aligned(x, 16) && hgr_aligned(xh, 8) && hgr_aligned(xl, 8) && hgr_aligned(stats, 8), "hgr_row_stats16: misaligned operand");
    HGR_REQUIRE(dtype == HGR_BF16 || dtype == HGR_F16, "hgr_row_stats16: bad dtype %d", dtype);
    hgr_by_dtype(dtype, [&](auto dt) { hipLaunchKernelGGL((row_stats16<dt.value>), dim3((rows + 3) / 4), dim3(256), 0, (hipStream_t)stream, x, xh, xl, stats, rows, W); });
    HGR_CHECK_LAUNCH("hgr_row_stats16");
    return HGR_OK;
}

extern "C" int hgr_pair_rows_f32(const void *xh, const void *xl, float *out, int rows, int W, int64_t row_mul, const int32_t *row_idx, int dtype, void *stream) {
    HGR_REQUIRE(xh && xl && out, "hgr_pair_rows_f32: null operand");
    HGR_REQUIRE(rows >= 1 && W >= 4 && W % 4 == 0 && row_mul >= 1, "hgr_pair_rows_f32: rows=%d W=%d row_mul=%lld unsupported", rows, W, (long long)row_mul);
    HGR_REQUIRE(hgr_aligned(xh, 8) && hgr_aligned(xl, 8) && hgr_aligned(out, 16), "hgr_pair_rows_f32: misaligned operand");
    HGR_REQUIRE(dtype == HGR_BF16 || dtype == HGR_F16, "hgr_pair_rows_f32: bad dtype %d", dtype);
    hgr_by_dtype(dtype, [&](auto dt) { hipLaunchKernelGGL((pair_rows_f32<dt.value>), dim3((rows + 3) / 4), dim3(256), 0, (hipStream_t)stream, xh, xl, out, rows, W, row_mul, row_idx); });
    HGR_CHECK_LAUNCH("hgr_pair_rows_f32");
    return HGR_OK;
}

extern "C" int hgr_vit_head(const void *xh, const void *xl, int64_t ldx, int64_t row_mul, const float *gamma, const float *beta, float eps,
                            const void *proj_t, float *out, int B, int W, int D, int dtype, void *stream) {
    HGR_REQUIRE(xh && xl && gamma && beta && proj_t && out, "hgr_vit_head: null operand");
    HGR_REQUIRE(B >= 1 && W >= 64 && W % 32 == 0 && W <= 1920 && D >= 1 && D % 4 == 0 && ldx >= W && ldx % 4 == 0 && row_mul >= 1,
                "hgr_vit_head: bad shape B=%d W=%d D=%d ldx=%lld (W %% 32 == 0, W <= 1920: 16 rows in 64 KB of LDS, D %% 4 == 0)", B, W, D, (long long)ldx);
    HGR_REQUIRE(hgr_aligned(xh, 8) && hgr_aligned(xl, 8) && hgr_aligned(gamma, 16) && hgr_aligned(beta, 16) && hgr_aligned(proj_t, 16) && hgr_aligned(out, 16),
                "hgr_vit_head: misaligned operand");
    HGR_REQUIRE(dtype == HGR_BF16 || dtype == HGR_F16, "hgr_vit_head: bad dtype %d", dtype);
    const size_t lds = (size_t)16 * (W * 2 + 16);
    dim3 grid((unsigned)((B + 15) / 16), (unsigned)((D + 127) / 128));
    hgr_by_nv_pow2((W / 4 + 63) / 64, [&](auto nv) { hgr_by_dtype(dtype, [&](auto dt) {
        hipLaunchKernelGGL((vit_head<dt.value, nv.value>), grid, dim3(256), lds, (hipStream_t)stream, xh, xl, ldx, row_mul, gamma, beta, eps, proj_t, out, B, W, D); }); });
    HGR_CHECK_LAUNCH("hgr_vit_head");
    return HGR_OK;
}
```

hgr-net_amd/model/clip_tree.py:

```python
from __future__ import annotations

import copy
import math
import os
import random
from typing import Optional, Sequence

import torch
import torch.nn as nn

from .. import clip, ops
from ..graphs import GraphCache
from ..hierarchy import build_hierarchy
from .._lib import HgrError

TEMPLATE = "a photo of a {}."

TAIL_OVERLAP = os.environ.get("HGR_TAIL_OVERLAP", "1") != "0"
LOGITS_SPLIT = os.environ.get("HGR_LOGITS_SPLIT", "class")


class _StopHead(Exception):
    """Raised by the split hook while the HEAD graph of a pipelined step is captured: the rest of the step belongs to the tail graph."""


def _classifier_part(slot: str):
    def fget(self):
        return self.__dict__.get(slot)

    def fset(self, value):
        self.__dict__[slot] = value
        self.__dict__["_cls_token"] = self.__dict__.get("_cls_token", 0) + 1
    return property(fget, fset)


class _Pipe:

    def __init__(self, dev):
        self.side = torch.cuda.Stream(device=dev, priority=int(os.environ.get("HGR_TAIL_PRIO", "-1")))
        self.cache = GraphCache(8, "all", pre_drop=self.drain)
        self.ok = None
        self.step = 0
        self.head_done = [torch.cuda.Event(), torch.cuda.Event()]
        self.tail_done = [torch.cuda.Event(), torch.cuda.Event()]
        for e in self.tail_done:
            e.record()

    def drain(self) -> None:
        main = torch.cuda.current_stream()
        main.wait_stream(self.side)
        main.synchronize()


class tree_model(nn.Module):
    zsl_weights = _classifier_part("_cls_zsl32")
    _zsl16 = _classifier_part("_cls_zsl16")

    def __init__(self, opts, candidates_train: Sequence[str], candidates_test: Sequence[str],
                 node_tokens: Optional[torch.Tensor] = None, clip_model: Optional[nn.Module] = None):
        super().__init__()
        self.opts = opts
        self.device = f"cuda:{opts.device}" if isinstance(opts.device, int) else opts.device
        self.save_path = "{}/{}/{}_{}_{}/".format(opts.folder, opts.exp_name, opts.weights, opts.out_ratio, opts.in_ratio)
        self.file_path = self.save_path + "clip_{}".format(opts.from_epoch)
        os.makedirs(self.save_path, exist_ok=True)

        import json
        with open(opts.graph_path, "r") as f:
            self.hierarchy = build_hierarchy(json.load(f))
        self.p2c, self.c2p, self.d2n, self.nodes, self.start_up = self.hierarchy.as_tuple()
        self.nodes_id = list(range(len(self.nodes)))

        if clip_model is None:
            clip_model, _ = clip.load(name=opts.arch, device=self.device, download_root="pretrained",
                                      image_dtype=getattr(opts, "image_dtype", "f16"),
                                      text_dtype=getattr(opts, "text_dtype", "f16"))
        self.clip_model = clip_model
        if getattr(opts, "fetch", False):
            self.clip_model.load_state_dict(torch.load(opts.fetch_path, map_location=self.device))
        if getattr(opts, "load", False):
            path = self.file_path if opts.load_path == "none" else opts.load_path
            self.clip_model.load_state_dict(torch.load(path, map_location=self.device))
            print("successfully loaded")
        self.clip_model.eval()
        for p in self.clip_model.parameters():
            p.requires_grad_(True)
        self.loss = nn.CrossEntropyLoss()

        self.n_ctx = int(getattr(opts, "n_ctx", 0) or 0)
        if node_tokens is None:
            tmpl = (" ".join(["X"] * self.n_ctx) + " {}.") if self.n_ctx else TEMPLATE
            node_tokens = clip.tokenize([tmpl.format(self._wordnet_name(n)) for n in self.nodes])
        self.ctx = None
        if self.n_ctx:
            wt = self.clip_model.transformer.width
            self.ctx = nn.Parameter(torch.empty(self.n_ctx, wt, device=self.device).normal_(std=0.02))
        if node_tokens.shape[0] != len(self.nodes):
            raise ValueError(f"node_tokens has {node_tokens.shape[0]} rows for {len(self.nodes)} nodes")
        self.node_tokens = node_tokens.long().to(self.device)

        self.resolution = self.clip_model.visual.input_resolution
        self.candidates_train, self.candidates_test = candidates_train, candidates_test
        index = {n: i for i, n in enumerate(self.nodes)}
        self.train_index = torch.tensor([index[c] for c in candidates_train]).to(self.device)
        self.test_index = torch.tensor([index[c] for c in candidates_test]).to(self.device)
        self.max_depth = max(self.d2n.keys())
        if opts.weights == "adaptive":
            num_layer = [len(self.d2n[layer]) for layer in self.d2n.keys()]
            self.layer_weight = nn.Parameter(((1.0 / torch.tensor(num_layer, dtype=torch.float32)) * opts.scale).to(self.device))

        self.train_index32 = self.train_index.to(torch.int32)
        self.test_index32 = self.test_index.to(torch.int32)
        self.depth32 = torch.from_numpy(self.hierarchy.depth).to(self.device)
        self.zsl_weights = None
        self._zsl16 = None
        self.use_graph = os.environ.get("HGR_GRAPH", "1") != "0"
        self._graph_cache = GraphCache(4, "oldest")
        self._pipe = None

    @staticmethod
    def _wordnet_name(wnid: str) -> str:
        try:
            from nltk.corpus import wordnet as wn
        except Exception as e:
            raise RuntimeError("WordNet (nltk) is not available: pass node_tokens= to tree_model") from e
        return wn.synset_from_pos_and_offset("n", int(wnid[1:])).name().split(".")[0].replace("_", " ")

    def save(self, opts, epoch):
        torch.save(self.clip_model.state_dict(), self.save_path + "clip_{}".format(epoch))

    @torch.no_grad()
    def update_classifier(self, group=None):
        n = len(self.nodes)
        if group is not None:
            from ..parallel import sharded_text_features
            feats = sharded_text_features(self.clip_model, self.node_tokens, group, ctx=self.ctx)
        else:
            feats = self.clip_model.encode_text(self.node_tokens, ctx=self.ctx)
        z32 = torch.empty_like(feats)
        z16 = torch.empty(feats.shape, dtype=self.clip_model.image_dtype, device=feats.device)
        ops.l2norm_rows(feats, y16=z16, y32=z32)
        self.zsl_weights, self._zsl16 = z32, z16
        assert z32.shape[0] == n

    @torch.no_grad()
    def forward(self, inputs, targets=None, static_output: bool = False):
        if self._zsl16 is None:
            raise HgrError("call update_classifier() before forward()")
        self.join_tail()
        if self.use_graph and inputs.is_cuda:
            return self._forward_graphed(inputs, static_output)
        return self._forward_eager(inputs)

    @torch.no_grad()
    def forward_eval(self, inputs, plan, k: int):
        if self._zsl16 is None:
            raise HgrError("call update_classifier() before forward_eval()")
        self.join_tail()
        plan.bind(self._eval_class_operand(), self._zsl16.shape[1])
        if self.use_graph and inputs.is_cuda:
            return self._forward_graphed(inputs, True, ("eval", plan, k))
        return self._forward_eager(inputs, ("eval", plan, k))

    def _generation(self, inputs, mode):
        cm = self.clip_model
        return (tuple(inputs.shape), inputs.dtype, self._cls_token, cm._ws.epoch, cm._fingerprint(), tuple(sorted(cm._ln_off)), mode)

    def _forward_graphed(self, inputs, static_output: bool = False, mode=None):
        self.clip_model.poll_ln_guard()
        cache = self._graph_cache
        if cache.renew(self._generation(inputs, mode)):
            self._forward_eager(inputs, mode)
            cache.gen = self._generation(inputs, mode)
        g, out = cache.lookup(inputs, 0, lambda buf, slot: self._capture(buf, mode))
        g.replay()
        return out if (static_output or mode is not None) else out.clone()

    def _eager_phase(self, inputs, mode, phase: str, tag: str):
        from .. import _lib
        seen = []
        if phase == "head":
            def hook(name):
                seen.append(name)
                raise _StopHead()
        else:
            def hook(name):
                seen.append(name)
                _lib.set_muted(False)
        prev_hook, prev_tag = ops.SPLIT_HOOK, self.clip_model._img_tag
        ops.SPLIT_HOOK, self.clip_model._img_tag = hook, tag
        out = None
        try:
            _lib.set_muted(phase == "tail")
            out = self._forward_eager(inputs, mode)
        except _StopHead:
            pass
        finally:
            _lib.set_muted(False)
            ops.SPLIT_HOOK, self.clip_model._img_tag = prev_hook, prev_tag
        return out, bool(seen)

    def _pipe_state(self, dev) -> _Pipe:
        if self._pipe is None:
            self._pipe = _Pipe(dev)
        return self._pipe

    def join_tail(self) -> None:
        if self._pipe is not None:
            torch.cuda.current_stream().wait_stream(self._pipe.side)

    @torch.no_grad()
    def forward_eval_overlapped(self, inputs, plan, k: int, consume) -> bool:
        if not (TAIL_OVERLAP and self.use_graph and inputs.is_cuda) or self._zsl16 is None:
            return False
        if inputs.dtype not in (torch.float32, torch.uint8) or not inputs.is_contiguous():
            return False
        from ..clip import model as _clip_model
        if _clip_model.IMG_STREAMS > 1:
            return False
        plan.bind(self._eval_class_operand(), self._zsl16.shape[1])
        mode = ("eval", plan, k)
        st = self._pipe_state(inputs.device)
        self.clip_model.poll_ln_guard()
        main = torch.cuda.current_stream()
        if self._generation(inputs, mode) != st.cache.gen:
            main.wait_stream(st.side)
            ok = True
            for tag in ("v", "v@1"):
                ok &= self._eager_phase(inputs, mode, "head", tag)[1]
                if ok:
                    self._eager_phase(inputs, mode, "tail", tag)
            main.synchronize()
            st.cache.renew(self._generation(inputs, mode))
            st.ok = ok
        if not st.ok:
            return False
        par = st.step & 1
        st.step += 1

        def capture(buf, par):
            tag = "v@1" if par else "v"
            epoch = self.clip_model._ws.epoch
            st.drain()
            gh, gt = torch.cuda.CUDAGraph(), torch.cuda.CUDAGraph()
            with torch.cuda.graph(gh):
                self._eager_phase(buf, mode, "head", tag)
            with torch.cuda.graph(gt):
                outs, _ = self._eager_phase(buf, mode, "tail", tag)
            if epoch != self.clip_model._ws.epoch:
                raise HgrError("workspace buffers moved during the capture of a pipelined evaluation step")
            return gh, gt, outs
        gh, gt, outs = st.cache.lookup(inputs, par, capture)
        main.wait_event(st.tail_done[par])
        gh.replay()
        st.head_done[par].record(main)
        with torch.cuda.stream(st.side):
            st.side.wait_event(st.head_done[par])
            gt.replay()
            consume(*outs)
            st.tail_done[par].record(st.side)
        return True

    def _capture(self, inputs, mode=None):
        self._forward_eager(inputs, mode)
        torch.cuda.current_stream().synchronize()
        g = torch.cuda.CUDAGraph()
        with torch.cuda.graph(g):
            out = self._forward_eager(inputs, mode)
        return g, out

    def _eval_class_operand(self):
        split = LOGITS_SPLIT if (LOGITS_SPLIT in ("class", "feat") and 2 * self._zsl16.shape[1] <= 1024) else ""
        if not split:
            return self._zsl16
        key = (split, self._cls_token)
        if getattr(self, "_zsl_split_key", None) != key:
            z16 = self._zsl16
            second = (self.zsl_weights.float() - z16.float()).to(z16.dtype) if split == "class" else z16
            self._zsl_split, self._zsl_split_key = torch.cat([z16, second], dim=1).contiguous(), key
        return self._zsl_split

    def _forward_eager(self, inputs, mode=None):
        feats = self.clip_model.encode_image(inputs)
        b, n = feats.shape[0], self._zsl16.shape[0]
        f16 = torch.empty(feats.shape, dtype=self._zsl16.dtype, device=feats.device)
        zc = self._eval_class_operand() if mode is None else mode[1].zsl
        if zc is not None and zc.shape[1] == 2 * feats.shape[1]:
            if LOGITS_SPLIT == "feat":
                f32 = torch.empty_like(feats)
                ops.l2norm_rows(feats, y16=f16, y32=f32)
                second = (f32 - f16.float()).to(f16.dtype)
            else:
                ops.l2norm_rows(feats, y16=f16)
                second = f16
            fin = torch.cat([f16, second], dim=1)
        else:
            ops.l2norm_rows(feats, y16=f16)
            fin, zc = f16, (self._zsl16 if mode is None else zc)
        if mode is not None:
            return ops.logits_eval(fin, mode[1], mode[2])
        ld = (n + 63) // 64 * 64
        logits = torch.empty((b, ld), dtype=torch.float32, device=feats.device)
        ops.gemm_nt(fin, zc, logits, n=n, tag="logits")
        return logits[:, :n]

    def get_contra_ids(self, method, target, depth=None, parents=None):
        nc = self.opts.num_compare
        if method == "random":
            ids = random.sample(self.train_index.tolist(), nc)
        elif method == "topk":
            low, high = min(self.d2n.keys()), max(self.d2n.keys())
            if depth - self.opts.k > low:
                low = depth - self.opts.k
            cand = []
            for d in range(low, depth):
                cand.extend(self.d2n[d])
            if depth == 0:
                cand.extend(self.d2n[depth])
            ids = list(set(cand) - set(parents))
            if len(ids) > nc:
                ids = random.sample(ids, nc)
        elif method == "brothers":
            if len(parents) > 1 and depth > 0:
                ids = copy.copy(self.p2c[parents[depth - 1]])
            else:
                ids = copy.copy(self.start_up)
            if len(ids) > nc:
                ids = random.sample(ids, nc)
        elif method == "near_simi":
            low, high = min(self.d2n.keys()), max(self.d2n.keys())
            low = max(low, depth - self.opts.k)
            high = min(high, depth + self.opts.k)
            cand = set()
            for d in range(low, high + 1):
                cand.update(self.d2n[d])
            cand = sorted(cand - set(parents) - set(self.p2c[target]) - {target})
            nc = min(nc, len(cand))
            with torch.no_grad():
                toks = self.node_tokens[torch.tensor([target] + cand, device=self.node_tokens.device)]
                f = self.clip_model.encode_text(toks, ctx=self.ctx.data if self.ctx is not None else None).float()
                f = f / f.norm(dim=-1, keepdim=True)
                order = (f[1:] @ f[0]).argsort(descending=True, stable=True)[:nc].tolist()
            ids = [cand[i] for i in order]
        else:
            raise NotImplementedError(f"sample_strategy {method!r} (the reference's 'simi' reads attributes that do not exist)")
        if target not in ids:
            ids.append(target)
        return ids, ids.index(target)

    def get_weights(self, method, max_depth=None, device=None):
        dev = self.device if device is None else device
        if method == "equal":
            return (torch.ones(max_depth) / max_depth).to(dev)
        if method == "decreasing":
            w = torch.arange(start=max_depth, end=0, step=-1).to(dev)
        elif method == "increasing":
            w = torch.arange(start=1, end=max_depth + 1).to(dev)
        elif method == "nl_increasing":
            w = (torch.arange(start=1, end=max_depth + 1) ** 3).to(dev)
        elif method == "nl_decreasing":
            w = (torch.arange(start=max_depth, end=0, step=-1) ** 3).to(dev)
        elif method == "adaptive":
            return torch.softmax(100 ** self.layer_weight[:max_depth], dim=0)
        else:
            raise ValueError(method)
        return w / w.sum()

    def outer_inner_plan(self, target: int):
        parents = copy.copy(self.c2p[target]) + [target]
        k = max(1, math.ceil(self.opts.out_ratio * len(parents)))
        outer = parents[::-1][:k]
        plan = []
        for k_loop, p_out in enumerate(outer):
            parents_in = copy.copy(self.c2p[p_out]) + [p_out]
            m = max(1, math.ceil(self.opts.in_ratio * len(parents_in)))
            inner = parents_in[::-1][:m]
            for m_loop, p_in in enumerate(inner):
                plan.append(dict(p_out=p_out, p_in=p_in, depth=parents_in.index(p_in), parents_in=parents_in,
                                 k_loop=k_loop, m_loop=m_loop, K=len(outer), M=len(inner)))
        return plan

    def train_batch(self, inputs, targets, training_method, sample_strategy):
        if getattr(self, "_trainer", None) is None:
            from ..training import OMTrainer
            self._trainer = OMTrainer(self, getattr(self.opts, "train_dtype", "bf16"))
        return self._trainer.train_batch(inputs, targets, training_method, sample_strategy)
```

hgr-net_amd/ops.py:

```python
from __future__ import annotations

import math
from typing import Optional

import torch

from . import _lib
from ._lib import (EPI_ACCUM, EPI_BIAS, EPI_BIAS_ADD16_RELU, EPI_BIAS_QUICKGELU, EPI_BIAS_RELU, EPI_BIAS_RESIDUAL, EPI_NONE, EPI_QGELU_GRAD16,
                   HGR_BF16, HGR_F16)

PROFILE = None

WEIGHTS_GEN = [0]

SPLIT_HOOK = None


def split_point(name: str) -> None:
    h = SPLIT_HOOK
    if h is not None:
        h(name)


TORCH16 = {HGR_BF16: torch.bfloat16, HGR_F16: torch.float16}
PAIR_LO = torch.uint8


def pair_value(xh: torch.Tensor, xl: torch.Tensor) -> torch.Tensor:
    out = torch.empty(xh.shape, dtype=torch.float32, device=xh.device)
    return pair_rows_f32(xh.contiguous(), xl.contiguous(), out)
DT_OF = {torch.bfloat16: HGR_BF16, torch.float16: HGR_F16}


def dtype_code(name) -> int:
    if name in (HGR_BF16, HGR_F16):
        return name
    return {"bf16": HGR_BF16, "bfloat16": HGR_BF16, "f16": HGR_F16, "fp16": HGR_F16, "float16": HGR_F16,
            torch.bfloat16: HGR_BF16, torch.float16: HGR_F16}[name]


def _stream() -> int:
    return torch.cuda.current_stream().cuda_stream


def _dev(t: Optional[torch.Tensor]) -> int:
    if t is None:
        return 0
    if not t.is_cuda:
        raise _lib.HgrError("libhgr ops need device tensors (no CPU path)")
    return t.data_ptr()


def gemm_nt(a: torch.Tensor, w: torch.Tensor, out: torch.Tensor, bias: Optional[torch.Tensor] = None,
            residual: Optional[torch.Tensor] = None, epilogue: int = EPI_NONE, n: Optional[int] = None, tag: str = "") -> torch.Tensor:
    assert a.dim() == 2 and w.dim() == 2 and out.dim() == 2 and a.dtype == w.dtype and a.stride(1) == 1 and w.stride(1) == 1
    m, k = a.shape
    nn = w.shape[0] if n is None else n
    assert w.shape[1] == k and out.shape[0] == m and out.shape[1] >= nn and out.stride(1) == 1
    out32 = out.dtype == torch.float32
    assert out32 or out.dtype == a.dtype
    if residual is not None:
        assert residual.stride(1) == 1 and residual.dtype == (a.dtype if epilogue in (EPI_BIAS_ADD16_RELU, EPI_QGELU_GRAD16) else torch.float32)
    prof = PROFILE
    if prof is not None:
        ev0, ev1 = torch.cuda.Event(enable_timing=True), torch.cuda.Event(enable_timing=True)
        ev0.record()
    _lib.call("hgr_gemm_nt", _dev(a), a.stride(0), _dev(w), w.stride(0), _dev(out), out.stride(0),
              _dev(bias), _dev(residual), residual.stride(0) if residual is not None else 0,
              m, nn, k, DT_OF[a.dtype], epilogue, 1 if out32 else 0, _stream())
    if prof is not None:
        ev1.record()
        byts = 2 * m * k + 2 * nn * k + (4 if out32 else 2) * m * nn + (4 * m * nn if residual is not None else 0)
        prof.append(("gemm_nt", ev0, ev1, 2.0 * m * nn * k, float(byts), tag))
    return out


def _prof_begin():
    if PROFILE is None:
        return None
    ev0, ev1 = torch.cuda.Event(enable_timing=True), torch.cuda.Event(enable_timing=True)
    ev0.record()
    return ev0, ev1


def _prof_end(ev, flops, byts, tag):
    if ev is not None:
        ev[1].record()
        PROFILE.append(("gemm_nt", ev[0], ev[1], float(flops), float(byts), tag))


LN_GUARD_SUMSQ = 16384.0 ** 2


def gemm_nt_res_stats(a: torch.Tensor, w: torch.Tensor, xh: torch.Tensor, xl: torch.Tensor, bias: torch.Tensor, stats: torch.Tensor,
                      tag: str = "", flag: Optional[torch.Tensor] = None) -> None:
    m, k = a.shape
    n = w.shape[0]
    assert a.dtype == w.dtype == xh.dtype and xl.dtype == PAIR_LO and xh.shape == xl.shape == (m, n) and xh.stride() == xl.stride()
    assert stats.dtype == torch.float32 and stats.numel() >= m * (n // 64) * 2 and a.stride(1) == w.stride(1) == xh.stride(1) == 1
    ev = _prof_begin()
    if flag is None:
        _lib.call("hgr_gemm_nt_res_stats", _dev(a), a.stride(0), _dev(w), w.stride(0), _dev(xh), _dev(xl), xh.stride(0), _dev(bias),
                  _dev(stats), m, n, k, DT_OF[a.dtype], _stream())
    else:
        assert flag.numel() == 1 and flag.element_size() == 4
        _lib.call("hgr_gemm_nt_res_stats_guard", _dev(a), a.stride(0), _dev(w), w.stride(0), _dev(xh), _dev(xl), xh.stride(0), _dev(bias),
                  _dev(stats), LN_GUARD_SUMSQ, _dev(flag), m, n, k, DT_OF[a.dtype], _stream())
    _prof_end(ev, 2.0 * m * n * k, 2 * m * k + 2 * n * k + 6 * m * n + 8 * m * (n // 64), tag)


def gemm_nt_res_stats_wide_ok(m: int, n: int, k: int, lda: int, ldw: int, ldx: int, dtype) -> bool:
    code = dtype if isinstance(dtype, int) else DT_OF.get(dtype, -1)
    return bool(_lib.load().hgr_gemm_nt_res_stats_wide_ok(int(m), int(n), int(k), int(lda), int(ldw), int(ldx), int(code)))


WIDE_CALLS = [0]


def gemm_nt_res_stats_wide(a: torch.Tensor, w: torch.Tensor, xh: torch.Tensor, xl: torch.Tensor, bias: torch.Tensor, stats: torch.Tensor,
                           tag: str = "", flag: Optional[torch.Tensor] = None) -> None:
    m, k = a.shape
    n = w.shape[0]
    assert a.dtype == w.dtype == xh.dtype and xl.dtype == PAIR_LO and xh.shape == xl.shape == (m, n) and xh.stride() == xl.stride()
    assert stats.dtype == torch.float32 and stats.numel() >= m * (n // 64) * 2 and a.stride(1) == w.stride(1) == xh.stride(1) == 1
    assert flag is None or (flag.numel() == 1 and flag.element_size() == 4)
    ev = _prof_begin()
    _lib.call("hgr_gemm_nt_res_stats_wide", _dev(a), a.stride(0), _dev(w), w.stride(0), _dev(xh), _dev(xl), xh.stride(0), _dev(bias),
              _dev(stats), LN_GUARD_SUMSQ if flag is not None else 0.0, _dev(flag), m, n, k, DT_OF[a.dtype], _stream())
    if not _lib.muted():
        WIDE_CALLS[0] += 1
    _prof_end(ev, 2.0 * m * n * k, 2 * m * k + 2 * n * k + 6 * m * n + 8 * m * (n // 64), tag)


def gemm_nt_bias_gelu_dual(a: torch.Tensor, w: torch.Tensor, pre: torch.Tensor, post: torch.Tensor, bias: torch.Tensor) -> None:
    assert a.dim() == 2 and w.dim() == 2 and a.dtype == w.dtype == pre.dtype == post.dtype and a.stride(1) == w.stride(1) == pre.stride(1) == post.stride(1) == 1
    m, k = a.shape
    n = w.shape[0]
    assert w.shape[1] == k and pre.shape == (m, n) and post.shape == (m, n) and bias.dtype == torch.float32 and bias.numel() == n
    _lib.call("hgr_gemm_nt_bias_gelu_dual", _dev(a), a.stride(0), _dev(w), w.stride(0), _dev(pre), pre.stride(0), _dev(post), post.stride(0),
              _dev(bias), m, n, k, DT_OF[a.dtype], _stream())


def gemm_nt_qgelu_grad_colsum(dy: torch.Tensor, wt: torch.Tensor, dx: torch.Tensor, pre: torch.Tensor, part: torch.Tensor) -> None:
    assert dy.dim() == 2 and wt.dim() == 2 and dy.dtype == wt.dtype == dx.dtype == pre.dtype and dy.stride(1) == wt.stride(1) == dx.stride(1) == pre.stride(1) == 1
    m, k = dy.shape
    n = wt.shape[0]
    assert wt.shape[1] == k and dx.shape == (m, n) and pre.shape == (m, n)
    assert part.dtype == torch.float32 and part.is_contiguous() and part.shape == ((m + 63) // 64, n)
    _lib.call("hgr_gemm_nt_qgelu_grad_colsum", _dev(dy), dy.stride(0), _dev(wt), wt.stride(0), _dev(dx), dx.stride(0), _dev(pre), pre.stride(0),
              _dev(part), m, n, k, DT_OF[dy.dtype], _stream())


def gelu_dual_ok(m: int, n: int, k: int, lda: int, ldw: int) -> bool:
    return n % 128 == 0 and k % 64 == 0 and k >= 128 and m * lda * 2 < (1 << 32) and n * ldw * 2 < (1 << 32)


def gemm_nt_ln(x16: torch.Tensor, wfold: torch.Tensor, out: torch.Tensor, ln_s: torch.Tensor, ln_c: torch.Tensor, stats: torch.Tensor,
               eps: float = 1e-5, quickgelu: bool = False, tag: str = "") -> torch.Tensor:
    m, k = x16.shape
    n = wfold.shape[0]
    assert x16.dtype == wfold.dtype == out.dtype and out.shape[0] == m and out.shape[1] >= n and ln_s.numel() == n and ln_c.numel() == n
    assert x16.stride(1) == wfold.stride(1) == out.stride(1) == 1 and stats.dtype == torch.float32 and stats.numel() >= m * (k // 64) * 2
    ev = _prof_begin()
    _lib.call("hgr_gemm_nt_ln", _dev(x16), x16.stride(0), _dev(wfold), wfold.stride(0), _dev(out), out.stride(0), _dev(ln_s), _dev(ln_c),
              _dev(stats), float(eps), m, n, k, DT_OF[x16.dtype], 1 if quickgelu else 0, _stream())
    _prof_end(ev, 2.0 * m * n * k, 2 * m * k + 2 * n * k + 2 * m * n, tag)
    return out


def gemm_nt_ln_mha(x16: torch.Tensor, wfold: torch.Tensor, att: torch.Tensor, ln_s: torch.Tensor, ln_c: torch.Tensor, stats: torch.Tensor,
                   b: int, l: int, heads: int, causal: bool, eps: float = 1e-5, tag: str = "qkv_mha") -> torch.Tensor:
    m, k = x16.shape
    w = heads * 64
    assert m == b * l and k == w and wfold.shape == (3 * w, k) and x16.dtype == wfold.dtype == att.dtype and att.shape == (m, w)
    assert x16.stride(1) == wfold.stride(1) == att.stride(1) == 1 and ln_s.numel() == ln_c.numel() == 3 * w
    assert stats.dtype == torch.float32 and stats.numel() >= m * (k // 64) * 2
    ev = _prof_begin()
    _lib.call("hgr_gemm_nt_ln_mha", _dev(x16), x16.stride(0), _dev(wfold), wfold.stride(0), _dev(ln_s), _dev(ln_c), _dev(stats), float(eps),
              _dev(att), att.stride(0), b, l, heads, 1 if causal else 0, DT_OF[x16.dtype], _stream())
    _prof_end(ev, 2.0 * m * 3 * w * k + 4.0 * b * heads * l * l * 64, 2 * m * k + 2 * 3 * w * k + 2 * m * w, tag)
    return att


def ln_mha_ok(w: int, l: int, rows: Optional[int] = None, ldx: Optional[int] = None) -> bool:
    if not (1 <= l <= 64 and w % 128 == 0):
        return False
    if rows is not None and rows * (ldx if ldx is not None else w) * 2 >= (1 << 32):
        return False
    return 3 * w * w * 2 < (1 << 32)


def vit_embed_ln_stats(patches, cls, pos, gamma, beta, xh, xl, stats, b, g, eps=1e-5):
    _lib.call("hgr_vit_embed_ln_stats", _dev(patches), _dev(cls), _dev(pos), _dev(gamma), _dev(beta), _dev(xh), _dev(xl), _dev(stats),
              b, g, xh.shape[1], eps, DT_OF[xh.dtype], _stream())


def vit_patch_embed_ln_ok(b: int, r: int, patch: int, w: int, dtype) -> bool:
    code = DT_OF.get(dtype, dtype if isinstance(dtype, int) else -1)
    return bool(_lib.load().hgr_vit_patch_embed_ln_ok(int(b), int(r), int(patch), int(w), int(code)))


def vit_patch_embed_ln(image: torch.Tensor, conv_w: torch.Tensor, cls, pos, gamma, beta, xh, xl, stats, patch: int, eps=1e-5) -> None:
    assert image.dtype == torch.float32 and image.dim() == 4 and image.shape[1] == 3 and image.shape[2] == image.shape[3] and image.is_contiguous()
    b, r = image.shape[0], image.shape[2]
    w, k = conv_w.shape
    gg = (r // patch) ** 2
    assert conv_w.is_contiguous() and k == 3 * patch * patch and conv_w.dtype == xh.dtype and xl.dtype == PAIR_LO
    assert xh.is_contiguous() and xl.is_contiguous() and xh.shape == xl.shape == (b * (gg + 1), w)
    assert stats.dtype == torch.float32 and stats.is_contiguous() and stats.numel() >= b * (gg + 1) * (w // 64) * 2
    ev = _prof_begin()
    _lib.call("hgr_vit_patch_embed_ln", _dev(image), _dev(conv_w), _dev(cls), _dev(pos), _dev(gamma), _dev(beta), _dev(xh), _dev(xl), _dev(stats),
              b, r, patch, w, eps, DT_OF[xh.dtype], _stream())
    rows = b * (gg + 1)
    _prof_end(ev, 2.0 * b * gg * w * k, 4 * b * 3 * r * r + 2 * w * k + 3 * rows * w + 8 * rows * (w // 64), "patch")


def row_stats16(x: torch.Tensor, xh: torch.Tensor, xl: torch.Tensor, stats: torch.Tensor) -> None:
    assert x.dtype == torch.float32 and x.is_contiguous() and xh.is_contiguous() and xl.is_contiguous() and xh.shape == xl.shape == x.shape
    assert xl.dtype == PAIR_LO and stats.numel() >= x.shape[0] * (x.shape[1] // 64) * 2
    _lib.call("hgr_row_stats16", _dev(x), _dev(xh), _dev(xl), _dev(stats), x.shape[0], x.shape[1], DT_OF[xh.dtype], _stream())


def pair_rows_f32(xh: torch.Tensor, xl: torch.Tensor, out: torch.Tensor, row_mul: int = 1, row_idx: Optional[torch.Tensor] = None) -> torch.Tensor:
    assert xh.is_contiguous() and xl.is_contiguous() and out.is_contiguous() and out.dtype == torch.float32 and out.shape[1] == xh.shape[1] and xl.dtype == PAIR_LO
    _lib.call("hgr_pair_rows_f32", _dev(xh), _dev(xl), _dev(out), out.shape[0], out.shape[1], row_mul, _dev(row_idx), DT_OF[xh.dtype], _stream())
    return out


def vit_head(xh: torch.Tensor, xl: torch.Tensor, row_mul: int, gamma: torch.Tensor, beta: torch.Tensor, eps: float, proj_t: torch.Tensor,
             out: torch.Tensor) -> torch.Tensor:
    assert xh.dtype == proj_t.dtype and xl.dtype == PAIR_LO and xh.stride() == xl.stride() and xh.stride(1) == 1
    assert out.dtype == torch.float32 and out.is_contiguous() and proj_t.is_contiguous() and proj_t.shape[1] == xh.shape[1] and out.shape[1] == proj_t.shape[0]
    ev = _prof_begin()
    _lib.call("hgr_vit_head", _dev(xh), _dev(xl), xh.stride(0), int(row_mul), _dev(gamma), _dev(beta), float(eps), _dev(proj_t), _dev(out),
              out.shape[0], xh.shape[1], out.shape[1], DT_OF[xh.dtype], _stream())
    _prof_end(ev, 2.0 * out.shape[0] * out.shape[1] * xh.shape[1], 0, "head")
    return out


def gemm_set_tile(tile: int) -> int:
    lib = _lib.load()
    prev = lib.hgr_gemm_set_tile(int(tile))
    if prev < 0:
        raise _lib.HgrError(f"hgr_gemm_set_tile failed ({prev}): {lib.hgr_last_error().decode()}")
    return prev


def gemm_set_tail(enabled: bool, full_panels: int = -1) -> int:
    lib = _lib.load()
    prev = lib.hgr_gemm_set_tail(1 if enabled else 0, int(full_panels))
    if prev < 0:
        raise _lib.HgrError(f"hgr_gemm_set_tail failed ({prev}): {lib.hgr_last_error().decode()}")
    return prev


def gemm_set_persist(enabled: bool) -> int:
    lib = _lib.load()
    prev = lib.hgr_gemm_set_persist(1 if enabled else 0)
    if prev < 0:
        raise _lib.HgrError(f"hgr_gemm_set_persist failed ({prev}): {lib.hgr_last_error().decode()}")
    return prev


def gemm_plan(fn) -> list:
    lib = _lib.load()
    out = (_lib.GemmLaunch * 4)()
    rc = lib.hgr_gemm_plan_capture(out, len(out))
    if rc:
        raise _lib.HgrError(f"hgr_gemm_plan_capture failed ({rc}): {lib.hgr_last_error().decode()}")
    try:
        fn()
    finally:
        unused = lib.hgr_gemm_plan_capture(None, 0)
    if unused:
        raise _lib.HgrError("gemm_plan: fn() made no call that hgr_gemm_plan_capture covers")
    return [{name: getattr(rec, name) for name, _ in rec._fields_} for rec in out if rec.kernel]


def im2col_patches(image: torch.Tensor, out: torch.Tensor, patch: int) -> torch.Tensor:
    b, c, r, r2 = image.shape
    assert c == 3 and r == r2 and image.dtype == torch.float32 and image.is_contiguous() and out.is_contiguous()
    _lib.call("hgr_im2col_patches", _dev(image), _dev(out), b, r, patch, out.shape[1], DT_OF[out.dtype], _stream())
    return out


def im2col_patches_tokens(image: torch.Tensor, out: torch.Tensor, patch: int, l: int) -> torch.Tensor:
    b, c, r, _ = image.shape
    assert image.dtype == torch.float32 and image.is_contiguous() and out.is_contiguous() and out.shape[0] == b * l
    _lib.call("hgr_im2col_patches_ex", _dev(image), _dev(out), b, r, patch, out.shape[1], l, 1, DT_OF[out.dtype], _stream())
    return out


CLIP_MEAN = (0.48145466, 0.4578275, 0.40821073)
CLIP_STD = (0.26862954, 0.26130258, 0.27577711)


def im2col_patches_u8(image: torch.Tensor, out: torch.Tensor, patch: int, mean=CLIP_MEAN, std=CLIP_STD) -> torch.Tensor:
    import ctypes
    b, r, r2, c = image.shape
    assert image.dtype == torch.uint8 and c == 3 and r == r2 and image.is_contiguous() and out.is_contiguous()
    g = r // patch
    m3, s3 = (ctypes.c_float * 3)(*mean), (ctypes.c_float * 3)(*std)
    _lib.call("hgr_im2col_patches_u8", _dev(image), _dev(out), b, r, patch, out.shape[1], g * g, 0, m3, s3, DT_OF[out.dtype], _stream())
    return out


def preprocess_bicubic(src: torch.Tensor, off: torch.Tensor, hw: torch.Tensor, tab: Optional[torch.Tensor], xb: torch.Tensor, xk: torch.Tensor, kx: int,
                       yb: torch.Tensor, yk: torch.Tensor, ky: int, out_u8: Optional[torch.Tensor], out_f32: Optional[torch.Tensor],
                       mean=CLIP_MEAN, std=CLIP_STD, b: int = 0, r: int = 0) -> None:
    import ctypes
    assert src.dtype == torch.uint8 and off.dtype == torch.int64 and all(t.dtype == torch.int32 for t in (hw, xb, xk, yb, yk))
    t = xb.numel() // (2 * r)
    assert off.numel() == b and hw.numel() == 2 * b and xb.numel() == 2 * t * r and xk.numel() == t * r * kx and yk.numel() == t * r * ky
    assert (tab is None and t == b) or (tab is not None and tab.dtype == torch.int32 and tab.numel() == b)
    assert out_u8 is None or (out_u8.dtype == torch.uint8 and out_u8.is_contiguous() and out_u8.numel() == b * r * r * 3)
    assert out_f32 is None or (out_f32.dtype == torch.float32 and out_f32.is_contiguous() and out_f32.numel() == b * r * r * 3)
    m3, s3 = (ctypes.c_float * 3)(*mean), (ctypes.c_float * 3)(*std)
    _lib.call("hgr_preprocess_bicubic", _dev(src), _dev(off), _dev(hw), _dev(tab), _dev(xb), _dev(xk), kx, _dev(yb), _dev(yk), ky,
              _dev(out_u8), _dev(out_f32), m3, s3, b, r, _stream())


def vit_assemble(t: torch.Tensor, cls: torch.Tensor, pos: torch.Tensor, b: int, l: int) -> torch.Tensor:
    _lib.call("hgr_vit_assemble", _dev(t), _dev(cls), _dev(pos), b, l, t.shape[1], _stream())
    return t


def vit_embed_ln(patches, cls, pos, gamma, beta, x, b, g, eps=1e-5):
    _lib.call("hgr_vit_embed_ln", _dev(patches), _dev(cls), _dev(pos), _dev(gamma), _dev(beta), _dev(x), b, g, x.shape[1], eps, _stream())
    return x


def layernorm(x: torch.Tensor, gamma, beta, out: torch.Tensor, rows: Optional[int] = None, row_mul: int = 1,
              row_idx: Optional[torch.Tensor] = None, eps: float = 1e-5) -> torch.Tensor:
    w = x.shape[-1]
    rows = out.shape[0] if rows is None else rows
    out32 = out.dtype == torch.float32
    _lib.call("hgr_layernorm", _dev(x), _dev(gamma), _dev(beta), _dev(out), rows, w, row_mul, _dev(row_idx), eps,
              HGR_BF16 if out32 else DT_OF[out.dtype], 1 if out32 else 0, _stream())
    return out


def mha(qkv: torch.Tensor, out: torch.Tensor, b: int, l: int, heads: int, causal: bool, stats: Optional[torch.Tensor] = None,
        q_rows: int = 0) -> torch.Tensor:
    assert qkv.is_contiguous() and out.is_contiguous() and qkv.shape[1] == 3 * heads * 64 and out.shape[1] == heads * 64
    if q_rows:
        assert stats is None
        _lib.call("hgr_mha_rows", _dev(qkv), _dev(out), b, l, heads, 1 if causal else 0, int(q_rows), DT_OF[qkv.dtype], _stream())
        return out
    if stats is not None:
        assert stats.dtype == torch.float32 and stats.is_contiguous() and stats.numel() == b * heads * l * 2
        _lib.call("hgr_mha_stats", _dev(qkv), _dev(out), _dev(stats), b, l, heads, 1 if causal else 0, DT_OF[qkv.dtype], _stream())
        return out
    _lib.call("hgr_mha", _dev(qkv), _dev(out), b, l, heads, 1 if causal else 0, DT_OF[qkv.dtype], _stream())
    return out


def text_embed(tokens: torch.Tensor, emb: torch.Tensor, pos: torch.Tensor, x: torch.Tensor, l: int) -> torch.Tensor:
    assert tokens.dtype == torch.int64 and tokens.stride(1) == 1
    n = tokens.shape[0]
    _lib.call("hgr_text_embed", _dev(tokens), tokens.stride(0), _dev(emb), _dev(pos), _dev(x), n, l, emb.shape[1], emb.shape[0], _stream())
    return x


def eot_index(tokens: torch.Tensor, out: torch.Tensor) -> torch.Tensor:
    assert tokens.dtype == torch.int64 and out.dtype == torch.int32
    _lib.call("hgr_eot_index", _dev(tokens), tokens.stride(0), _dev(out), tokens.shape[0], tokens.shape[1], _stream())
    return out


def l2norm_rows(x: torch.Tensor, y16: Optional[torch.Tensor] = None, y32: Optional[torch.Tensor] = None) -> None:
    assert x.dtype == torch.float32 and x.is_contiguous()
    dt = DT_OF[y16.dtype] if y16 is not None else HGR_BF16
    _lib.call("hgr_l2norm_rows", _dev(x), _dev(y16), _dev(y32), x.shape[0], x.shape[1], dt, _stream())


def topk_rows(logits: torch.Tensor, k: int, cols: Optional[torch.Tensor] = None, n_cols: Optional[int] = None,
              want_values: bool = False):
    assert logits.dtype == torch.float32 and logits.stride(1) == 1
    rows = logits.shape[0]
    nc = cols.numel() if cols is not None else (logits.shape[1] if n_cols is None else n_cols)
    idx = torch.empty((rows, k), dtype=torch.int32, device=logits.device)
    val = torch.empty((rows, k), dtype=torch.float32, device=logits.device) if want_values else None
    _lib.call("hgr_topk_rows", _dev(logits), logits.stride(0), _dev(cols), nc, k, _dev(idx), _dev(val), rows, _stream())
    return (idx, val) if want_values else idx


def level_argmax(logits: torch.Tensor, depth: torch.Tensor, n_levels: int, cols: Optional[torch.Tensor] = None,
                 n_cols: Optional[int] = None, want_top1: bool = False):
    assert logits.dtype == torch.float32 and logits.stride(1) == 1 and depth.dtype == torch.int32
    rows = logits.shape[0]
    nc = cols.numel() if cols is not None else (logits.shape[1] if n_cols is None else n_cols)
    out = torch.empty((rows, n_levels), dtype=torch.int32, device=logits.device)
    top1 = torch.empty((rows, 1), dtype=torch.int32, device=logits.device) if want_top1 else None
    _lib.call("hgr_level_argmax", _dev(logits), logits.stride(0), _dev(cols), nc, _dev(depth), n_levels, _dev(out), _dev(top1), rows, _stream())
    return (out, top1) if want_top1 else out


class EvalIndex:

    def __init__(self, depth: torch.Tensor, train_cols: torch.Tensor, test_cols: Optional[torch.Tensor], n_levels: int):
        import numpy as np
        d = depth.cpu().numpy()
        n = len(d)
        tr = train_cols.cpu().numpy().astype(np.int64)
        assert d.min() >= 0 and n_levels <= 32 and d[tr].max() < n_levels, "a subset node lies deeper than n_levels"
        assert len(set(tr.tolist())) == len(tr), "train columns must be distinct"
        lv = d[tr]
        filler = np.full(n_levels, -1, dtype=np.int32)
        for l in range(n_levels):
            other = np.nonzero(lv != l)[0]
            if other.size:
                filler[l] = int(other[0])
        tpos = np.full(n, -1, dtype=np.int32)
        tpos[tr] = np.arange(len(tr), dtype=np.int32)
        dev = depth.device
        self.n_nodes, self.n_levels, self.n_train = n, n_levels, len(tr)
        self.lvl8 = torch.from_numpy(np.minimum(d, 255).astype(np.uint8)).to(dev)
        self.train_pos = torch.from_numpy(tpos).to(dev)
        self.train_cols = train_cols.to(torch.int32).contiguous()
        self.filler = torch.from_numpy(filler).to(dev)
        self.test_pos = self.test_cols = None
        self.n_test = 0
        if test_cols is not None:
            te = test_cols.cpu().numpy().astype(np.int64)
            assert len(set(te.tolist())) == len(te), "test columns must be distinct"
            epos = np.full(n, -1, dtype=np.int32)
            epos[te] = np.arange(len(te), dtype=np.int32)
            self.test_pos = torch.from_numpy(epos).to(dev)
            self.test_cols = test_cols.to(torch.int32).contiguous()
            self.n_test = len(te)


def eval_rows(logits: torch.Tensor, index: EvalIndex, k: int):
    assert logits.dtype == torch.float32 and logits.stride(1) == 1 and logits.shape[1] >= index.n_nodes
    rows = logits.shape[0]
    dev = logits.device
    lvl = torch.empty((rows, index.n_levels), dtype=torch.int32, device=dev)
    top1 = torch.empty((rows, 1), dtype=torch.int32, device=dev)
    topk = torch.empty((rows, max(k, 1)), dtype=torch.int32, device=dev)
    _lib.call("hgr_eval_rows", _dev(logits), logits.stride(0), index.n_nodes, _dev(index.lvl8), _dev(index.train_pos), _dev(index.train_cols),
              index.n_train, index.n_levels, _dev(index.filler), _dev(index.test_pos), _dev(index.test_cols), index.n_test, k,
              _dev(lvl), _dev(top1), _dev(topk), rows, _stream())
    return lvl, top1, topk


class LogitsEvalPlan:
    SLICE, SLAB = 32, 96

    def __init__(self, index: EvalIndex):
        import numpy as np
        lvl = index.lvl8.cpu().numpy().astype(np.int64)
        tpos = index.train_pos.cpu().numpy()
        epos = index.test_pos.cpu().numpy() if index.test_pos is not None else np.full(len(lvl), -1, dtype=np.int32)
        cols, level_first = [], [0]
        for l in range(index.n_levels):
            c = np.nonzero(lvl == l)[0]
            pad = (-c.size) % self.SLICE
            cols.append(np.concatenate([c, np.full(pad, -1, dtype=np.int64)]))
            level_first.append(level_first[-1] + (c.size + pad) // self.SLICE)
        assert int((lvl >= index.n_levels).sum()) == 0, "a node lies deeper than n_levels"
        perm = np.concatenate(cols)
        tail = (-perm.size) % self.SLAB
        if tail or perm.size == 0:
            perm = np.concatenate([perm, np.full(tail or self.SLAB, -1, dtype=np.int64)])
        dev = index.lvl8.device
        valid = perm >= 0
        safe = np.where(valid, perm, 0)
        self.index = index
        self.n_perm = int(perm.size)
        self.perm = torch.from_numpy(safe).to(dev)
        self.valid = torch.from_numpy(valid).to(dev)
        self.tpos = torch.from_numpy(np.where(valid, tpos[safe], -1).astype(np.int32)).to(dev)
        self.epos = torch.from_numpy(np.where(valid, epos[safe], -1).astype(np.int32)).to(dev)
        self.level_first = torch.from_numpy(np.asarray(level_first, dtype=np.int32)).to(dev)
        self.zsl = None
        self._src = None
        self._ws = None

    MAX_SLICES = 1024

    @property
    def supported(self) -> bool:
        return self.n_perm // self.SLICE <= self.MAX_SLICES and self.index.n_levels <= 32

    def bind(self, zsl16: torch.Tensor, algo_d: Optional[int] = None) -> "LogitsEvalPlan":
        self.algo_d = int(algo_d or zsl16.shape[1])
        if self._src is not zsl16:
            z = zsl16[self.perm]
            z[~self.valid] = 0
            self.zsl, self._src = z.contiguous(), zsl16
        return self

    def workspace(self, rows: int, dev) -> torch.Tensor:
        need = int(_lib.load().hgr_logits_eval_workspace_bytes(rows, self.n_perm))
        if self._ws is None or self._ws.numel() < need or self._ws.device != torch.device(dev):
            self._ws = torch.empty(need, dtype=torch.uint8, device=dev)
        return self._ws


def logits_eval(feat16: torch.Tensor, plan: LogitsEvalPlan, k: int, stage: str = ""):
    ix = plan.index
    assert plan.zsl is not None, "LogitsEvalPlan.bind(zsl16) first"
    assert feat16.is_contiguous() and feat16.dtype == plan.zsl.dtype and feat16.shape[1] == plan.zsl.shape[1]
    rows, d = feat16.shape
    dev = feat16.device
    lvl = torch.empty((rows, ix.n_levels), dtype=torch.int32, device=dev)
    top1 = torch.empty((rows, 1), dtype=torch.int32, device=dev)
    topk = torch.empty((rows, max(k, 1)), dtype=torch.int32, device=dev)
    prof = PROFILE
    ev = _prof_begin()
    _lib.call({"": "hgr_logits_eval", "tile": "hgr_logits_eval_tile_stage", "row": "hgr_logits_eval_row_stage"}[stage],
              _dev(feat16), _dev(plan.zsl), rows, d, plan.n_perm, _dev(plan.tpos), _dev(plan.epos), _dev(plan.level_first),
              ix.n_levels, _dev(ix.filler), _dev(ix.train_cols), ix.n_train, _dev(ix.test_cols), ix.n_test, k,
              _dev(lvl), _dev(top1), _dev(topk), _dev(plan.workspace(rows, dev)), DT_OF[feat16.dtype], _stream())
    da = getattr(plan, "algo_d", d)
    _prof_end(ev, 2.0 * rows * ix.n_nodes * da, 2 * rows * da + 2 * ix.n_nodes * da, "logits_eval" + ("_" + stage if stage else ""))
    return lvl, top1, topk


def eval_counters(pred: torch.Tensor, targets: Optional[torch.Tensor], target: int, top1: torch.Tensor, lv: torch.Tensor,
                  parents: torch.Tensor, levels: torch.Tensor, acc: torch.Tensor) -> None:
    assert pred.dtype == top1.dtype == lv.dtype == parents.dtype == levels.dtype == torch.int32 and acc.dtype == torch.float64
    assert pred.is_contiguous() and lv.is_contiguous() and top1.is_contiguous() and acc.numel() == 9
    assert targets is None or (targets.dtype == torch.int64 and targets.is_contiguous() and targets.numel() == pred.shape[0])
    _lib.call("hgr_eval_counters", _dev(pred), pred.shape[1], _dev(targets), int(target), _dev(top1), _dev(lv), lv.shape[1], _dev(parents),
              _dev(levels), parents.numel(), _dev(acc), pred.shape[0], _stream())


def eval_counters_rows(pred: torch.Tensor, targets: torch.Tensor, top1: torch.Tensor, lv: torch.Tensor, anc_ptr: torch.Tensor,
                       anc_nodes: torch.Tensor, anc_levels: torch.Tensor, acc: torch.Tensor) -> None:
    assert pred.dtype == top1.dtype == lv.dtype == anc_ptr.dtype == anc_nodes.dtype == anc_levels.dtype == torch.int32 and acc.dtype == torch.float64
    assert pred.is_contiguous() and lv.is_contiguous() and top1.is_contiguous() and acc.numel() == 9
    assert anc_ptr.is_contiguous() and anc_nodes.is_contiguous() and anc_levels.is_contiguous() and anc_ptr.numel() >= 2
    assert targets is not None and targets.dtype == torch.int64 and targets.is_contiguous() and targets.numel() == pred.shape[0]
    assert top1.numel() == pred.shape[0] and lv.shape[0] == pred.shape[0]
    _lib.call("hgr_eval_counters_rows", _dev(pred), pred.shape[1], _dev(targets), _dev(top1), _dev(lv), lv.shape[1], _dev(anc_ptr),
              _dev(anc_nodes), _dev(anc_levels), anc_ptr.numel() - 1, _dev(acc), pred.shape[0], _stream())


REPORT_MAXL = 32
REPORT_DEPTH_COLS = ("rows", "hit@1", "hit@2", "hit@5", "hit@10", "hit@20", "anc_hit", "point", "edge", "chain")
REPORT_DEPTH = 0
REPORT_LEVEL = REPORT_DEPTH + (REPORT_MAXL + 1) * len(REPORT_DEPTH_COLS)
REPORT_DIST_BINS = 2 * REPORT_MAXL + 2
REPORT_DIST_UNKNOWN = 2 * REPORT_MAXL + 1
REPORT_DIST_TEST = REPORT_LEVEL + 2 * REPORT_MAXL
REPORT_DIST_ALL = REPORT_DIST_TEST + REPORT_DIST_BINS
REPORT_HEIGHT = REPORT_DIST_ALL + REPORT_DIST_BINS
REPORT_HEIGHT_K = (1, 2, 5, 10, 20)
REPORT_LEN = REPORT_HEIGHT + len(REPORT_HEIGHT_K)


def eval_report_rows(pred: torch.Tensor, targets: torch.Tensor, top1: torch.Tensor, lv: torch.Tensor, anc_ptr: torch.Tensor,
                     anc_nodes: torch.Tensor, anc_levels: torch.Tensor, table: torch.Tensor) -> None:
    assert pred.dtype == top1.dtype == lv.dtype == anc_ptr.dtype == anc_nodes.dtype == anc_levels.dtype == torch.int32
    assert table.dtype == torch.int64 and table.numel() == REPORT_LEN and table.is_contiguous()
    assert pred.is_contiguous() and lv.is_contiguous() and top1.is_contiguous()
    assert anc_ptr.is_contiguous() and anc_nodes.is_contiguous() and anc_levels.is_contiguous() and anc_ptr.numel() >= 2
    assert targets is not None and targets.dtype == torch.int64 and targets.is_contiguous() and targets.numel() == pred.shape[0]
    assert top1.numel() == pred.shape[0] and lv.shape[0] == pred.shape[0]
    _lib.call("hgr_eval_report_rows", _dev(pred), pred.shape[1], _dev(targets), _dev(top1), _dev(lv), lv.shape[1], _dev(anc_ptr),
              _dev(anc_nodes), _dev(anc_levels), anc_ptr.numel() - 1, _dev(table), pred.shape[0], _stream())


PATH_MAXL = 32


def path_scores(logits: torch.Tensor, anc_ptr: torch.Tensor, anc_nodes: torch.Tensor, wtab: torch.Tensor,
                out: Optional[torch.Tensor] = None) -> torch.Tensor:
    n_nodes = anc_ptr.numel() - 1
    assert logits.dim() == 2 and logits.dtype == torch.float32 and logits.stride(1) == 1 and logits.shape[1] >= n_nodes >= 1
    assert anc_ptr.dtype == anc_nodes.dtype == torch.int32 and anc_ptr.is_contiguous() and anc_nodes.is_contiguous()
    assert wtab.dtype == torch.float32 and wtab.shape == (PATH_MAXL + 1, PATH_MAXL) and wtab.is_contiguous()
    rows = logits.shape[0]
    if out is None:
        out = torch.empty((rows, n_nodes), dtype=torch.float32, device=logits.device)
    assert out.dim() == 2 and out.dtype == torch.float32 and out.stride(1) == 1 and out.shape[0] == rows and out.shape[1] >= n_nodes
    _lib.call("hgr_path_scores", _dev(logits), logits.stride(0), _dev(out), out.stride(0), n_nodes, _dev(anc_ptr), _dev(anc_nodes),
              _dev(wtab), rows, _stream())
    return out[:, :n_nodes]


HEDGE_MAXT = 8
HEDGE_MAXN = 36864
HEDGE_SCALE = 1 << 30
HEDGE_COL_NAMES = ("rows", "abstain", "exact", "ancestor", "below", "wrong", "sum_lpick", "sum_common", "sum_lt")
HEDGE_COL_HIST = len(HEDGE_COL_NAMES)
HEDGE_COLS = HEDGE_COL_HIST + REPORT_MAXL + 1


def hedge_thresholds(thetas) -> list:
    try:
        th = [float(t) for t in thetas]
    except TypeError:
        raise ValueError(f"hedge thresholds {thetas!r}: a sequence of numbers") from None
    if not 1 <= len(th) <= HEDGE_MAXT:
        raise ValueError(f"hedge: {len(th)} thresholds (1..{HEDGE_MAXT})")
    if not all(0.0 < t <= 1.0 for t in th):
        raise ValueError(f"hedge thresholds {th}: each in (0, 1]")
    if any(b <= a for a, b in zip(th, th[1:])):
        raise ValueError(f"hedge thresholds {th}: strictly increasing")
    return [int(math.ceil(t * HEDGE_SCALE)) for t in th]


def subtree_hedge(scores: torch.Tensor, cand_pos: Optional[torch.Tensor], anc_ptr: torch.Tensor, anc_nodes: torch.Tensor,
                  temperature: float, thr: torch.Tensor, pick: Optional[torch.Tensor] = None, pick_mass: Optional[torch.Tensor] = None,
                  mass_out: Optional[torch.Tensor] = None):
    n_nodes = anc_ptr.numel() - 1
    assert scores.dim() == 2 and scores.dtype == torch.float32 and scores.stride(1) == 1
    assert anc_ptr.dtype == anc_nodes.dtype == torch.int32 and anc_ptr.is_contiguous() and anc_nodes.is_contiguous()
    assert cand_pos is None or (cand_pos.dtype == torch.int32 and cand_pos.is_contiguous() and cand_pos.numel() == n_nodes)
    assert thr.dtype == torch.int32 and thr.dim() == 1 and thr.is_contiguous()
    rows, t = scores.shape[0], thr.numel()
    if pick is None:
        pick = torch.empty((rows, t), dtype=torch.int32, device=scores.device)
    if pick_mass is None:
        pick_mass = torch.empty((rows, t), dtype=torch.float32, device=scores.device)
    assert pick.dtype == torch.int32 and pick.shape == (rows, t) and pick.is_contiguous()
    assert pick_mass.dtype == torch.float32 and pick_mass.shape == (rows, t) and pick_mass.is_contiguous()
    assert mass_out is None or (mass_out.dim() == 2 and mass_out.dtype == torch.int32 and mass_out.stride(1) == 1 and mass_out.shape[0] == rows)
    _lib.call("hgr_subtree_hedge", _dev(scores), scores.stride(0), n_nodes, _dev(cand_pos), _dev(anc_ptr), _dev(anc_nodes), float(temperature),
              _dev(thr), t, _dev(pick), _dev(pick_mass), _dev(mass_out), mass_out.stride(0) if mass_out is not None else 0, rows, _stream())
    return pick, pick_mass


def hedge_counters_rows(pick: torch.Tensor, targets: torch.Tensor, anc_ptr: torch.Tensor, anc_nodes: torch.Tensor, table: torch.Tensor) -> None:
    assert pick.dtype == anc_ptr.dtype == anc_nodes.dtype == torch.int32 and pick.dim() == 2 and pick.is_contiguous()
    assert anc_ptr.is_contiguous() and anc_nodes.is_contiguous() and anc_ptr.numel() >= 2
    assert table.dtype == torch.int64 and table.shape == (pick.shape[1], HEDGE_COLS) and table.is_contiguous()
    assert targets is not None and targets.dtype == torch.int64 and targets.is_contiguous() and targets.numel() == pick.shape[0]
    _lib.call("hgr_hedge_counters_rows", _dev(pick), pick.shape[1], _dev(targets), _dev(anc_ptr), _dev(anc_nodes), anc_ptr.numel() - 1,
              _dev(table), pick.shape[0], _stream())


SETS_MAXS = 16
SETS_COL_NAMES = ("rows", "hit@1", "hit@2", "hit@5", "hit@10", "hit@20", "anc_hit", "point", "edge")
SETS_COLS = len(SETS_COL_NAMES)


def check_sets(sets, n_nodes: int) -> dict:
    try:
        items = [(str(k), [int(c) for c in (v.tolist() if hasattr(v, "tolist") else v)]) for k, v in dict(sets).items()]
    except (TypeError, ValueError):
        raise ValueError(f"sets {sets!r}: a mapping from a name to node ids") from None
    if not 1 <= len(items) <= SETS_MAXS:
        raise ValueError(f"sets: {len(items)} candidate sets (1..{SETS_MAXS})")
    for name, ids in items:
        if len(set(ids)) != len(ids):
            raise ValueError(f"sets[{name!r}]: a node id appears twice")
        bad = [c for c in ids if not 0 <= c < n_nodes]
        if bad:
            raise ValueError(f"sets[{name!r}]: node id {bad[0]} outside the hierarchy (0..{n_nodes - 1})")
    return dict(items)


class SetIndex:

    def __init__(self, eval_index: EvalIndex, sets):
        import numpy as np
        n = eval_index.n_nodes
        items = list(check_sets(sets, n).items())
        member = np.zeros(n, dtype=np.int32)
        for s, (name, ids) in enumerate(items):
            member[np.asarray(ids, dtype=np.int64)] |= np.int32(1 << s)
        key = np.full(n, -1, dtype=np.int64)
        if eval_index.test_pos is not None:
            key = eval_index.test_pos.cpu().numpy().astype(np.int64)
        rest = key < 0
        key[rest] = eval_index.n_test + np.arange(int(rest.sum()), dtype=np.int64)
        dev = eval_index.lvl8.device
        self.n_nodes, self.n_sets = n, len(items)
        self.names = tuple(name for name, _ in items)
        self.sizes = tuple(len(ids) for _, ids in items)
        self.member = torch.from_numpy(member).to(dev)
        self.tie_key = torch.from_numpy(key.astype(np.int32)).to(dev)

# ... 600 lines not shown
```

include/hgr.h:

```cpp
#ifndef HGR_H
#define HGR_H

#include <stdint.h>

#ifdef __cplusplus
extern "C" {
#endif

#define HGR_ABI_VERSION 5

enum { HGR_OK = 0, HGR_EINVAL = -1, HGR_EUNSUPPORTED = -2, HGR_ELAUNCH = -3 };

typedef enum { HGR_BF16 = 0, HGR_F16 = 1 } hgr_dtype_t;

typedef enum {
    HGR_EPI_NONE = 0,
    HGR_EPI_BIAS = 1,
    HGR_EPI_BIAS_QUICKGELU = 2,
    HGR_EPI_BIAS_RESIDUAL = 3,
    HGR_EPI_BIAS_RELU = 4,
    HGR_EPI_BIAS_ADD16_RELU = 5,
    HGR_EPI_ACCUM = 6,
    HGR_EPI_QGELU_GRAD16 = 7
} hgr_epilogue_t;

int hgr_abi_version(void);
const char *hgr_last_error(void);

int hgr_gemm_nt(const void *A, int64_t lda, const void *W, int64_t ldw, void *C, int64_t ldc,
                const float *bias, const void *residual, int64_t ldr,
                int M, int N, int K, int dtype, int epilogue, int out_f32, void *stream);

int hgr_gemm_set_tile(int tile);

int hgr_gemm_set_tail(int enabled, int full_panels);
int hgr_gemm_set_persist(int enabled);

int hgr_gemm_set_p8(int mode);

int hgr_im2col_patches(const float *image, void *out, int B, int R, int P, int Kp, int dtype, void *stream);
int hgr_im2col_patches_ex(const float *image, void *out, int B, int R, int P, int Kp, int rows_per_image, int row_offset,
                          int dtype, void *stream);
int hgr_im2col_patches_u8(const unsigned char *image, void *out, int B, int R, int P, int Kp, int rows_per_image,
                          int row_offset, const float *mean3, const float *std3, int dtype, void *stream);
int hgr_preprocess_bicubic(const unsigned char *src, const int64_t *off, const int *hw, const int *tab, const int *xb, const int *xk, int KX,
                           const int *yb, const int *yk, int KY, unsigned char *out_u8, float *out_f32,
                           const float *mean3, const float *std3, int B, int R, void *stream);

int hgr_vit_assemble(float *t, const float *class_embedding, const float *positional_embedding, int B, int L, int W, void *stream);

int hgr_vit_embed_ln(const float *patches, const float *class_embedding, const float *positional_embedding,
                     const float *gamma, const float *beta, float *x,
                     int B, int G, int W, float eps, void *stream);

int hgr_layernorm(const float *x, const float *gamma, const float *beta, void *y,
                  int rows, int W, int64_t row_mul, const int32_t *row_idx,
                  float eps, int dtype, int out_f32, void *stream);

int hgr_mha(const void *qkv, void *out, int B, int L, int heads, int causal, int dtype, void *stream);
int hgr_mha_rows(const void *qkv, void *out, int B, int L, int heads, int causal, int q_rows, int dtype, void *stream);
int hgr_mha_stats(const void *qkv, void *out, float *stats, int B, int L, int heads, int causal, int dtype, void *stream);

int hgr_text_embed(const int64_t *tokens, int64_t ld_tokens, const float *token_embedding,
                   const float *positional_embedding, float *x, int n, int L, int W, int vocab, void *stream);

int hgr_eot_index(const int64_t *tokens, int64_t ld_tokens, int32_t *eot, int n, int ctx, void *stream);

int hgr_l2norm_rows(const float *x, void *y16, float *y32, int rows, int D, int dtype, void *stream);

int hgr_topk_rows(const float *logits, int64_t ld, const int32_t *cols, int n_cols, int k,
                  int32_t *out_idx, float *out_val, int rows, void *stream);

int hgr_level_argmax(const float *logits, int64_t ld, const int32_t *cols, int n_cols,
                     const int32_t *depth, int n_levels, int32_t *out, int32_t *out_top1, int rows, void *stream);

int hgr_eval_rows(const float *logits, int64_t ld, int n_nodes, const unsigned char *lvl8, const int32_t *train_pos,
                  const int32_t *train_cols, int n_train, int n_levels, const int32_t *filler_pos, const int32_t *test_pos,
                  const int32_t *test_cols, int n_test, int k, int32_t *out_level, int32_t *out_top1, int32_t *out_topk,
                  int rows, void *stream);

int hgr_eval_counters(const int32_t *pred, int k, const int64_t *targets, int target, const int32_t *top1, const int32_t *lv,
                      int n_levels, const int32_t *parents, const int32_t *levels, int L, double *acc, int rows, void *stream);

int hgr_eval_counters_rows(const int32_t *pred, int k, const int64_t *targets, const int32_t *top1, const int32_t *lv, int n_levels,
                           const int32_t *anc_ptr, const int32_t *anc_nodes, const int32_t *anc_levels, int n_nodes,
                           double *acc, int rows, void *stream);

#define HGR_REPORT_MAXL 32
#define HGR_REPORT_DEPTH_COLS 10
enum { HGR_REPORT_COL_ROWS = 0, HGR_REPORT_COL_HIT1 = 1, HGR_REPORT_COL_HIT2 = 2, HGR_REPORT_COL_HIT5 = 3, HGR_REPORT_COL_HIT10 = 4,
       HGR_REPORT_COL_HIT20 = 5, HGR_REPORT_COL_ANC_HIT = 6, HGR_REPORT_COL_POINT = 7, HGR_REPORT_COL_EDGE = 8, HGR_REPORT_COL_CHAIN = 9 };
#define HGR_REPORT_DEPTH 0
#define HGR_REPORT_LEVEL (HGR_REPORT_DEPTH + (HGR_REPORT_MAXL + 1) * HGR_REPORT_DEPTH_COLS)
#define HGR_REPORT_DIST_BINS (2 * HGR_REPORT_MAXL + 2)
#define HGR_REPORT_DIST_UNKNOWN (2 * HGR_REPORT_MAXL + 1)
#define HGR_REPORT_DIST_TEST (HGR_REPORT_LEVEL + 2 * HGR_REPORT_MAXL)
#define HGR_REPORT_DIST_ALL (HGR_REPORT_DIST_TEST + HGR_REPORT_DIST_BINS)
#define HGR_REPORT_HEIGHT (HGR_REPORT_DIST_ALL + HGR_REPORT_DIST_BINS)
#define HGR_REPORT_LEN (HGR_REPORT_HEIGHT + 5)
int hgr_eval_report_rows(const int32_t *pred, int k, const int64_t *targets, const int32_t *top1, const int32_t *lv, int n_levels,
                         const int32_t *anc_ptr, const int32_t *anc_nodes, const int32_t *anc_levels, int n_nodes, int64_t *table,
                         int rows, void *stream);

#define HGR_PATH_MAXL 32
int hgr_path_scores(const float *logits, int64_t ld, float *scores, int64_t ld_out, int n_nodes, const int32_t *anc_ptr,
                    const int32_t *anc_nodes, const float *wtab , int rows, void *stream);

#define HGR_HEDGE_MAXT 8
#define HGR_HEDGE_MAXN 36864
int hgr_subtree_hedge(const float *scores, int64_t ld, int n_nodes, const int32_t *cand_pos, const int32_t *anc_ptr,
                      const int32_t *anc_nodes, float temperature, const uint32_t *thr, int n_thr, int32_t *pick, float *pick_mass,
                      uint32_t *mass_out, int64_t ld_mass, int rows, void *stream);

enum { HGR_HEDGE_COL_ROWS = 0, HGR_HEDGE_COL_ABSTAIN = 1, HGR_HEDGE_COL_EXACT = 2, HGR_HEDGE_COL_ANCESTOR = 3, HGR_HEDGE_COL_BELOW = 4,
       HGR_HEDGE_COL_WRONG = 5, HGR_HEDGE_COL_SUM_LPICK = 6, HGR_HEDGE_COL_SUM_COMMON = 7, HGR_HEDGE_COL_SUM_LT = 8, HGR_HEDGE_COL_HIST = 9 };
#define HGR_HEDGE_COLS (HGR_HEDGE_COL_HIST + HGR_REPORT_MAXL + 1)
int hgr_hedge_counters_rows(const int32_t *pick, int n_thr, const int64_t *targets, const int32_t *anc_ptr, const int32_t *anc_nodes,
                            int n_nodes, int64_t *table , int rows, void *stream);

#define HGR_SETS_MAXS 16
int hgr_set_ranks(const float *scores, int64_t ld, int n_nodes, const uint32_t *member, const int32_t *tie_key, int n_sets,
                  const int64_t *targets, int32_t *rank, int32_t *top1, int rows, void *stream);

#define HGR_SETS_COLS 9
int hgr_set_counters_rows(const int32_t *rank, const int32_t *top1, int n_sets, const int64_t *targets, const int32_t *lv, int n_levels,
                          const int32_t *anc_ptr, const int32_t *anc_nodes, const int32_t *anc_levels, int n_nodes,
                          int64_t *table , int rows, void *stream);

int hgr_dgp_score_rows(const void *table, int64_t ld, int table_f32, int n_cols, int n_masked, float mask_value, const int32_t *depth,
                       int n_levels, const int64_t *targets, int target, int32_t *rank, int32_t *top1, int32_t *lv, int32_t *pred,
                       int k_pred, int rows, void *stream);


int hgr_conv3x3_nhwc(const void *x, const void *w, const float *bias, void *out,
                     int B, int H, int W, int C, int Cout, int stride, int Kp, int dtype, void *stream);

int hgr_conv3x3_pool2_nhwc(const void *x, const void *w, const float *bias, void *out, int B, int H, int W, int C, int Cout,
                           int Kp, int dtype, void *stream);

int hgr_stem_conv1(const float *image, const void *w, const float *bias, void *out, int B, int R, int Cout, int Kp,
                   int dtype, void *stream);

int hgr_stem_im2col(const float *image, void *out, int B, int R, int dtype, void *stream);

int hgr_avgpool2_nhwc(const void *x, void *out, int B, int H, int W, int C, int dtype, void *stream);

int hgr_attnpool_tokens(const void *x, const float *pos, void *out, int B, int S, int C, int dtype, void *stream);

int hgr_attnpool_attend(const float *q, const void *k, const void *v, void *out, int B, int L, int heads,
                        int dtype, void *stream);

int hgr_stem7_pool(const float *image, const void *w, const float *bias, void *out, int B, int R, int Kp, int dtype, void *stream);
int hgr_stem7_im2col(const float *image, void *out, int B, int R, int Kp, int dtype, void *stream);
int hgr_maxpool3s2_nhwc(const void *x, void *out, int B, int H, int W, int C, int dtype, void *stream);
int hgr_subsample2_nhwc(const void *x, void *out, int B, int H, int W, int C, int dtype, void *stream);
int hgr_meanpool_nhwc(const void *x, void *out, int B, int H, int W, int C, int dtype, int out_f32, void *stream);


int hgr_gemm_tn_splitk(const void *P, int64_t ldp, const void *Q, int64_t ldq, float *partial, int64_t ldo,
                       int M, int Na, int Nb, int kc, int dtype, void *stream);
int hgr_gemm_tn_tile(int Na, int Nb);

enum { HGR_KERNEL_128 = 1, HGR_KERNEL_256 = 2, HGR_KERNEL_DUO = 3, HGR_KERNEL_P8 = 5, HGR_KERNEL_CONV_DIRECT = 6 };
typedef struct { int32_t kernel, variant, epilogue, out_f32, act, grid_x, grid_y, tiles_m, tiles_n, total,
                 nbig, big_panels, tiles_m_half, group, m_fastest, vec_ok, row0, rows; } hgr_gemm_launch;
int hgr_gemm_plan_capture(hgr_gemm_launch *out, int max_launches);

int hgr_conv3x3_wgrad_splitk(const void *dy, int64_t lddy, const void *x, float *partial, int64_t ldo,
                             int B, int H, int W, int C, int Cout, int kc, int dtype, void *stream);

int hgr_transpose16(const void *x, int64_t ldx, void *y, int64_t ldy, int rows, int cols, void *stream);

int hgr_transpose16_colsum(const void *x, int64_t ldx, void *y, int64_t ldy, int rows, int cols, int dtype,
                           float *out, int accumulate, float alpha, float *scratch, void *stream);

int hgr_colsum(const void *x, int64_t ldx, int rows, int cols, int x_f32, int dtype, float *out, int accumulate,
               float alpha, float *scratch, void *stream);

int hgr_cast16(const float *x, void *y, int64_t n, int dtype, void *stream);
int hgr_cast16_transpose(const float *x, int64_t ldx, void *y, int64_t ldy, void *yt, int64_t ldyt, int rows, int cols, int dtype, void *stream);

int hgr_quickgelu16(const void *a, const void *du, void *out, int64_t n, int backward, int dtype, void *stream);

int hgr_layernorm_bwd(const void *dy, int dy_f32, const float *x, const float *gamma, float *dx, float *dgamma,
                      float *dbeta, float *scratch, int rows, int W, int64_t row_mul, const int32_t *row_idx,
                      float eps, int dtype, void *stream);
int hgr_layernorm_bwd_cast(const void *dy, int dy_f32, const float *x, const float *gamma, float *dx, void *dx16, float *dgamma,
                           float *dbeta, float *scratch, int rows, int W, int64_t row_mul, const int32_t *row_idx, float eps,
                           int dtype, void *stream);
int hgr_layernorm_bwd_cast_colsum(const void *dy, int dy_f32, const float *x, const float *gamma, float *dx, void *dx16, float *dgamma,
                                  float *dbeta, float *dx16_colsum, float *scratch, int rows, int W, int64_t row_mul,
                                  const int32_t *row_idx, float eps, int dtype, void *stream);
int64_t hgr_layernorm_bwd_scratch_floats(int rows, int W);

int hgr_mha_bwd(const void *qkv, const void *out, const void *dout, void *dqkv, int B, int L, int heads, int causal, int dtype, void *stream);
int hgr_mha_bwd_stats(const void *qkv, const void *out, const void *dout, void *dqkv, const float *stats,
                      int B, int L, int heads, int causal, int dtype, void *stream);
int hgr_mha_bwd_colsum(const void *qkv, const void *out, const void *dout, void *dqkv, const float *stats, float *colsum_part,
                       int B, int L, int heads, int causal, int dtype, void *stream);

int hgr_conv3x3_nhwc_plain(const void *x, const void *w, void *out, int B, int H, int W, int C, int Cout, int Kp,
                           int dtype, void *stream);
int hgr_gemm_nt_splitk(const void *A, int64_t lda, const void *W, int64_t ldw, float *partial, int64_t ldc,
                       int M, int N, int K, int kc, int dtype, void *stream);
int hgr_relu_bwd16(const void *dy, const void *y, void *out, int64_t n, int dtype, void *stream);
int hgr_add16(const void *a, const void *b, void *out, int64_t n, int dtype, void *stream);
int hgr_avgpool2_bwd_nhwc(const void *dy, void *dx, int B, int H, int W, int C, int dtype, void *stream);
int hgr_attnpool_tokens_bwd(const void *dtok, void *dx, int B, int S, int C, int dtype, void *stream);
int hgr_im2col3x3_t(const void *xt, void *out, int B, int H, int W, int C, int64_t ld, int dtype, void *stream);
int hgr_bn_fold(const float *w, const float *gamma, const float *beta, const float *mean, const float *var, float eps,
                void *w16, float *bias, int Cout, int Cin, int khw, int Kp, int dtype, void *stream);
int hgr_bn_unfold_grad(const float *gwf, int64_t ldg, const float *gbf, const float *w, const float *gamma, const float *mean,
                       const float *var, float eps, float *g_w, float *g_gamma, float *g_beta, int Cout, int Cin, int khw,
                       void *stream);

int hgr_csr_group_aggregate(const float *support, int64_t ld_support, const int *item_row, const int *item_e0,
                            const int *item_e1, const int *item_slot, int n_items, const int *col, const float *inv_deg,
                            const unsigned char *grp, const float *att, int D, const float *bias,
                            const int *split_row, const int *split_slot0, const int *split_n, int n_split,
                            float *partial, float *out, int64_t ld_out, int C, float slope, int normalize, void *stream);

int hgr_csr_group_att_grad(const float *support, int64_t ld_support, const float *bias, const float *g, int64_t ld_g,
                           const float *y, int64_t ld_y, float *dout, int64_t ld_dout, const int *item_row,
                           const int *item_e0, const int *item_e1, const int *item_slot, int n_items, const int *col,
                           const float *inv_deg, const unsigned char *grp, int D, const int *split_row,
                           const int *split_slot0, const int *split_n, int n_split, float *partial, float *P, int C,
                           float slope, void *stream);

int hgr_dgp_loss_head(const float *O, int64_t ld_o, const int *rows, const float *F, int64_t ld_f, int n_t, int n,
                      float *loss_rows, float *loss, float *dout, int64_t ld_dout, int C, void *stream);

int hgr_dropout_counter(const float *x, int64_t ld_x, float *y, int64_t ld_y, int rows, int C, int seed, int step, int layer,
                        void *stream);

int hgr_adam_l2(float *p, const float *g, float *m, float *v, int64_t n, float lr, float beta1, float beta2, float eps, float wd,
                int step, void *stream);

int hgr_cnzsl_std_chain_fwd(const float *z, int64_t ld_z, const float *bias, float *running_mean1, float *running_var1,
                            float *running_mean2, float *running_var2, float *c, int64_t ld_c, float *a, int64_t ld_a,
                            float *stats, int S, int H, int train, float eps, float momentum, void *stream);

int hgr_cnzsl_std_chain_bwd(const float *dc, int64_t ld_dc, const float *a, int64_t ld_a, const float *z, int64_t ld_z,
                            const float *bias, const float *stats, float *dz, int64_t ld_dz, float *dbias, int S, int H,
                            float eps, void *stream);

int hgr_bias_relu_f32(const float *x, int64_t ld_x, const float *bias, float *y, int64_t ld_y, int rows, int C, void *stream);

int hgr_relu_bwd_colsum_f32(const float *dy, int64_t ld_dy, const float *y, int64_t ld_y, float *dx, int64_t ld_dx, float *db,
                            float *scratch, int rows, int C, void *stream);

int hgr_ce_rows(const float *logits, int64_t ld, const int32_t *labels, int rows, int n, float gscale,
                float *loss_rows, float *dlogits, int64_t ldd, void *stream);

int hgr_l2norm_bwd(const float *x, const float *dy, float *dx, int rows, int D, int accumulate, void *stream);

int hgr_matmul_f32(const float *A, int64_t sam, int64_t sak, const float *B, int64_t sbk, int64_t sbn, float *C,
                   int64_t ldc, int M, int N, int K, float alpha, int accumulate, void *stream);

int hgr_dot_f32(const float *a, const float *b, int64_t n, float *out, float alpha, int accumulate, void *stream);

int hgr_embed_scatter_add(const int64_t *tokens, int64_t ld_tokens, const float *dx, float *dtable, int n, int L,
                          int W, int vocab, void *stream);

int hgr_rows_axpy(float *dst, int64_t dst_mul, const int32_t *dst_idx, const float *src, int rows, int W, float alpha, void *stream);

int hgr_ctx_splice(float *x, const float *ctx, const float *positional_embedding, int n, int L, int W, int n_ctx, void *stream);
int hgr_ctx_splice_bwd(float *dx, float *dctx, int n, int L, int W, int n_ctx, void *stream);

int hgr_rows_gather(float *dst, const float *src, const int32_t *idx, int rows, int W, void *stream);

int hgr_sumsq(const float *x, int64_t n, float *out, void *stream);

int hgr_adamw(float *p, const float *g, float *m, float *v, int64_t n, float lr, float beta1, float beta2, float eps,
              float wd, int step, const float *sumsq_total, float max_norm, float grad_scale, void *stream);

int hgr_gemm_nt_res_stats(const void *A, int64_t lda, const void *W, int64_t ldw, void *xh, void *xl, int64_t ldx,
                          const float *bias, float *stats, int M, int N, int K, int dtype, void *stream);

int hgr_gemm_nt_res_stats_guard(const void *A, int64_t lda, const void *W, int64_t ldw, void *xh, void *xl, int64_t ldx,
                                const float *bias, float *stats, float guard_sumsq, uint32_t *flag,
                                int M, int N, int K, int dtype, void *stream);

int hgr_gemm_nt_res_stats_wide_ok(int64_t M, int64_t N, int64_t K, int64_t lda, int64_t ldw, int64_t ldx, int dtype);
int hgr_gemm_nt_res_stats_wide(const void *A, int64_t lda, const void *W, int64_t ldw, void *xh, void *xl, int64_t ldx,
                               const float *bias, float *stats, float guard_sumsq, uint32_t *flag,
                               int M, int N, int K, int dtype, void *stream);

int hgr_vit_head(const void *xh, const void *xl, int64_t ldx, int64_t row_mul, const float *gamma, const float *beta, float eps,
                 const void *proj_t, float *out, int B, int W, int D, int dtype, void *stream);
int hgr_gemm_nt_ln(const void *XH, int64_t ldx, const void *Wfold, int64_t ldw, void *C, int64_t ldc,
                   const float *ln_s, const float *ln_c, const float *stats, float eps,
                   int M, int N, int K, int dtype, int act, void *stream);

int hgr_gemm_nt_ln_mha(const void *XH, int64_t ldx, const void *Wfold, int64_t ldw, const float *ln_s, const float *ln_c,
                       const float *stats, float eps, void *att, int64_t ldatt, int B, int L, int heads, int causal,
                       int dtype, void *stream);

int hgr_gemm_nt_bias_gelu_dual(const void *A, int64_t lda, const void *W, int64_t ldw, void *pre, int64_t ldpre, void *post, int64_t ldpost,
                               const float *bias, int M, int N, int K, int dtype, void *stream);
int hgr_gemm_nt_qgelu_grad_colsum(const void *A, int64_t lda, const void *W, int64_t ldw, void *C, int64_t ldc, const void *pre, int64_t ldpre,
                                  float *colsum_part, int M, int N, int K, int dtype, void *stream);
int hgr_vit_embed_ln_stats(const float *patches, const float *class_embedding, const float *positional_embedding,
                           const float *gamma, const float *beta, void *xh, void *xl, float *stats,
                           int B, int G, int W, float eps, int dtype, void *stream);
int hgr_vit_patch_embed_ln_ok(int B, int R, int P, int W, int dtype);
int hgr_vit_patch_embed_ln(const float *image, const void *conv_w, const float *class_embedding, const float *positional_embedding,
                           const float *gamma, const float *beta, void *xh, void *xl, float *stats,
                           int B, int R, int P, int W, float eps, int dtype, void *stream);
int hgr_row_stats16(const float *x, void *xh, void *xl, float *stats, int rows, int W, int dtype, void *stream);
int hgr_pair_rows_f32(const void *xh, const void *xl, float *out, int rows, int W, int64_t row_mul, const int32_t *row_idx, int dtype, void *stream);

int64_t hgr_logits_eval_workspace_bytes(int rows, int n_perm);
int hgr_logits_eval(const void *feat16, const void *zsl_perm16, int rows, int D, int n_perm,
                    const int32_t *tpos_perm, const int32_t *epos_perm, const int32_t *level_first,
                    int n_levels, const int32_t *filler_pos, const int32_t *train_cols, int n_train,
                    const int32_t *test_cols, int n_test, int k,
                    int32_t *out_level, int32_t *out_top1, int32_t *out_topk, void *workspace, int dtype, void *stream);
int hgr_logits_eval_tile_stage(const void *feat16, const void *zsl_perm16, int rows, int D, int n_perm,
                    const int32_t *tpos_perm, const int32_t *epos_perm, const int32_t *level_first,
                    int n_levels, const int32_t *filler_pos, const int32_t *train_cols, int n_train,
                    const int32_t *test_cols, int n_test, int k,
                    int32_t *out_level, int32_t *out_top1, int32_t *out_topk, void *workspace, int dtype, void *stream);
int hgr_logits_eval_row_stage(const void *feat16, const void *zsl_perm16, int rows, int D, int n_perm,
                    const int32_t *tpos_perm, const int32_t *epos_perm, const int32_t *level_first,
                    int n_levels, const int32_t *filler_pos, const int32_t *train_cols, int n_train,
                    const int32_t *test_cols, int n_test, int k,
                    int32_t *out_level, int32_t *out_top1, int32_t *out_topk, void *workspace, int dtype, void *stream);

#define HGR_COMM_ID_BYTES 128
typedef enum { HGR_COMM_F32 = 0, HGR_COMM_F64 = 1, HGR_COMM_F16 = 2, HGR_COMM_BF16 = 3, HGR_COMM_I32 = 4, HGR_COMM_I64 = 5, HGR_COMM_U8 = 6 } hgr_comm_dtype_t;
typedef enum { HGR_COMM_SUM = 0, HGR_COMM_MAX = 1 } hgr_comm_op_t;

int hgr_comm_unique_id(void *id_out );
int hgr_comm_init(int rank, int world, const void *unique_id );
int hgr_comm_destroy(void);
int hgr_comm_rank(void);
int hgr_comm_world(void);
int hgr_allreduce(const void *send, void *recv, int64_t count, int dtype, int op, void *stream);
int hgr_allgather(const void *send, void *recv, int64_t count_per_rank, int dtype, void *stream);
int hgr_broadcast(void *buf, int64_t count, int dtype, int root, void *stream);

#define HGR_OUT_F32 2
#define HGR_ACT_LRELU02 0
#define HGR_ACT_SIGMOID 1
#define HGR_NLL_RESIDENT_COLS 18432

int hgr_normal_counter(float *z, int64_t ld_z, uint32_t *bits, int rows, int C, int seed, int stream_id, int64_t row0, void *stream);

int hgr_free_gen_input(void *out, int64_t ld_out, int out_type, const float *z, int64_t ld_z, const float *att, int64_t ld_att,
                       int att_rows, const int32_t *classes, int n_classes, int num, int rows, int nz, int A, int seed,
                       int stream_id, int64_t row0, void *stream);

int hgr_bias_act_rows(const float *x, int64_t ld_x, const float *bias, void *y, int64_t ld_y, int64_t col0, int out_type, int act,
                      int rows, int C, void *stream);

int hgr_free_fr_tail(const float *lantent, int64_t ld_l, const float *bias, const float *eps, int64_t ld_eps, void *y, int64_t ld_y,
                     int64_t col0, int out_type, float *mus, int64_t ld_mus, int rows, int A, int seed, int stream_id, int64_t row0,
                     void *stream);

int hgr_nll_rows16(const float *logits, int64_t ld, const int32_t *labels, int rows, int n, float *loss_rows, void *dlogits,
                   int64_t ld_d, float *logsm, int64_t ld_ls, int dtype, void *stream);

int hgr_adam_l2_cast16(float *p, const float *g, int64_t slice_stride, int n_slices, float alpha, float *m, float *v, void *w16,
                       int64_t n, float lr, float beta1, float beta2, float eps, float wd, int step, int dtype, void *stream);

#ifdef __cplusplus
}
#endif
#endif
```

Measured before the change: 110,000.

## Add small-M row GEMM kernels for class-token tail and fused replicated l2norm

Adds a new 32x64-tile GEMM kernel family with LN-folded and residual-stats epilogues for the last-layer class-token rows (M = batch). It reads strided per-row stats directly through a stats_mul stride, so the rows_gather copy is no longer needed. Smaller tiles give many more workgroups for the skinny M=512 GEMMs, which would otherwise underfill the GPU. It also adds an l2norm kernel that writes the normalized row twice, replacing l2norm followed by torch.cat. The risks are new kernel code on the hot path, deep-prefetch DMA waits that must match exactly, and possible numeric differences.

```diff
diff --git a/hgr-net_amd/_lib.py b/hgr-net_amd/_lib.py
--- a/hgr-net_amd/_lib.py
+++ b/hgr-net_amd/_lib.py
@@ -33,6 +33,7 @@
     "hgr_text_embed": [_p, _l, _p, _p, _p, _i, _i, _i, _i, _p],
     "hgr_eot_index": [_p, _l, _p, _i, _i, _p],
     "hgr_l2norm_rows": [_p, _p, _p, _i, _i, _i, _p],
+    "hgr_l2norm_rows_rep": [_p, _p, _l, _i, _i, _i, _i, _p],
     "hgr_topk_rows": [_p, _l, _p, _i, _i, _p, _p, _i, _p],
     "hgr_level_argmax": [_p, _l, _p, _i, _p, _i, _p, _p, _i, _p],
     "hgr_eval_rows": [_p, _l, _i, _p, _p, _p, _i, _i, _p, _p, _p, _i, _i, _p, _p, _p, _i, _p],
@@ -107,7 +108,11 @@
     "hgr_gemm_nt_res_stats_guard": [_p, _l, _p, _l, _p, _p, _l, _p, _p, _f, _p, _i, _i, _i, _i, _p],
     "hgr_gemm_nt_res_stats_wide_ok": [_l, _l, _l, _l, _l, _l, _i],
     "hgr_gemm_nt_res_stats_wide": [_p, _l, _p, _l, _p, _p, _l, _p, _p, _f, _p, _i, _i, _i, _i, _p],
+    "hgr_gemm_nt_res_stats_rows_ok": [_l, _l, _l, _l, _l, _l, _i],
+    "hgr_gemm_nt_res_stats_rows": [_p, _l, _p, _l, _p, _p, _l, _p, _p, _f, _p, _i, _i, _i, _i, _p],
     "hgr_gemm_nt_ln": [_p, _l, _p, _l, _p, _l, _p, _p, _p, _f, _i, _i, _i, _i, _i, _p],
+    "hgr_gemm_nt_ln_rows_ok": [_l, _l, _l, _l, _l, _l, _l, _i],
+    "hgr_gemm_nt_ln_rows": [_p, _l, _p, _l, _p, _l, _p, _p, _p, _l, _f, _i, _i, _i, _i, _i, _p],
     "hgr_gemm_nt_ln_mha": [_p, _l, _p, _l, _p, _p, _p, _f, _p, _l, _i, _i, _i, _i, _i, _p],
     "hgr_gemm_nt_bias_gelu_dual": [_p, _l, _p, _l, _p, _l, _p, _l, _p, _i, _i, _i, _i, _p],
     "hgr_gemm_nt_qgelu_grad_colsum": [_p, _l, _p, _l, _p, _l, _p, _l, _p, _i, _i, _i, _i, _p],
diff --git a/hgr-net_amd/clip/model.py b/hgr-net_amd/clip/model.py
--- a/hgr-net_amd/clip/model.py
+++ b/hgr-net_amd/clip/model.py
@@ -157,6 +157,7 @@
 QKV_MHA = os.environ.get("HGR_QKV_MHA", "1") != "0"
 PATCH_FUSED = os.environ.get("HGR_PATCH_FUSED", "1") != "0"
 PROJ_WIDE = {"0": 0, "2": 2}.get(os.environ.get("HGR_PROJ_WIDE", "1"), 1)
+CLS_ROWS = os.environ.get("HGR_CLS_ROWS", "1") != "0"
 _CUS: Dict[int, int] = {}
 
 
@@ -191,10 +192,19 @@
                 ch, cl = xh.view(b, l, w)[:, 0, :], xl.view(b, l, w)[:, 0, :]
                 ops.gemm_nt_ln(xh, k.wf_in[w:], qkv[:, w:], k.s_in[w:], k.c_in[w:], stats, k.eps1, tag="kv")
                 ops.split_point("class_token_tail")
-                st_q = ws.get(tag + ".stats_q", (b, w // 64, 2), torch.float32, dev)
-                idx = ws.const(f"cls_rows.{b}.{l}", lambda: (torch.arange(b, dtype=torch.int32, device=dev) * l).contiguous())
-                ops.rows_gather(stats.view(b * l, -1), idx, st_q.view(b, -1))
-                ops.gemm_nt_ln(ch, k.wf_in[:w], qkv.view(b, l, 3 * w)[:, 0, :w], k.s_in[:w], k.c_in[:w], st_q, k.eps1, tag="q_cls")
+                q_c = qkv.view(b, l, 3 * w)[:, 0, :w]
+                rows = (CLS_ROWS and stats.is_contiguous()
+                        and ops.gemm_nt_ln_rows_ok(b, w, w, ch.stride(0), k.wf_in.stride(0), q_c.stride(0), l, dt)
+                        and ops.gemm_nt_ln_rows_ok(b, 4 * w, w, ch.stride(0), k.wf_fc.stride(0), 4 * w, 1, dt)
+                        and ops.gemm_nt_res_stats_rows_ok(b, w, w, att.stride(0) * l, k.w_out.stride(0), ch.stride(0), dt)
+                        and ops.gemm_nt_res_stats_rows_ok(b, w, 4 * w, 4 * w, k.w_proj.stride(0), ch.stride(0), dt))
+                if rows:
+                    ops.gemm_nt_ln_rows(ch, k.wf_in[:w], q_c, k.s_in[:w], k.c_in[:w], stats, k.eps1, stats_mul=l, tag="q_cls")
+                else:
+                    st_q = ws.get(tag + ".stats_q", (b, w // 64, 2), torch.float32, dev)
+                    idx = ws.const(f"cls_rows.{b}.{l}", lambda: (torch.arange(b, dtype=torch.int32, device=dev) * l).contiguous())
+                    ops.rows_gather(stats.view(b * l, -1), idx, st_q.view(b, -1))
+                    ops.gemm_nt_ln(ch, k.wf_in[:w], q_c, k.s_in[:w], k.c_in[:w], st_q, k.eps1, tag="q_cls")
             elif fused_attn:
                 ops.gemm_nt_ln_mha(xh, k.wf_in, att, k.s_in, k.c_in, stats, b, l, heads, causal, k.eps1)
             else:
@@ -205,6 +215,11 @@
                 ca = att.view(b, l, w)[:, 0, :]
                 st_c = ws.get(tag + ".stats_cls", (b, w // 64, 2), torch.float32, dev)
                 u_c = ws.get(tag + ".u16_cls", (b, 4 * w), dt, dev)
+                if rows:
+                    ops.gemm_nt_res_stats_rows(ca, k.w_out, ch, cl, k.b_out, st_c, tag="out_cls", flag=flag)
+                    ops.gemm_nt_ln_rows(ch, k.wf_fc, u_c, k.s_fc, k.c_fc, st_c, k.eps2, quickgelu=True, tag="fc_cls")
+                    ops.gemm_nt_res_stats_rows(u_c, k.w_proj, ch, cl, k.b_proj, st_c, tag="proj_cls", flag=flag)
+                    break
                 ops.gemm_nt_res_stats(ca, k.w_out, ch, cl, k.b_out, st_c, tag="out_cls", flag=flag)
                 ops.gemm_nt_ln(ch, k.wf_fc, u_c, k.s_fc, k.c_fc, st_c, k.eps2, quickgelu=True, tag="fc_cls")
                 ops.gemm_nt_res_stats(u_c, k.w_proj, ch, cl, k.b_proj, st_c, tag="proj_cls", flag=flag)
diff --git a/hgr-net_amd/csrc/hgr_gemm_common.h b/hgr-net_amd/csrc/hgr_gemm_common.h
--- a/hgr-net_amd/csrc/hgr_gemm_common.h
+++ b/hgr-net_amd/csrc/hgr_gemm_common.h
@@ -280,15 +280,15 @@
     s2 = (__builtin_fmaf(v[0], v[0], v[1] * v[1]) + __builtin_fmaf(v[2], v[2], v[3] * v[3])) +
          (__builtin_fmaf(v[4], v[4], v[5] * v[5]) + __builtin_fmaf(v[6], v[6], v[7] * v[7]));
 }
-template <int CTRL> __device__ __forceinline__ void pair_pass_dpp_stage(float (&s1)[2], float (&s2)[2]) {
-#pragma unroll
-    for (int q = 0; q < 2; ++q) {
+template <int CTRL, int NQ> __device__ __forceinline__ void pair_pass_dpp_stage(float (&s1)[NQ], float (&s2)[NQ]) {
+#pragma unroll
+    for (int q = 0; q < NQ; ++q) {
         s1[q] += __builtin_bit_cast(float, __builtin_amdgcn_update_dpp(0, __builtin_bit_cast(int, s1[q]), CTRL, 0xF, 0xF, true));
         s2[q] += __builtin_bit_cast(float, __builtin_amdgcn_update_dpp(0, __builtin_bit_cast(int, s2[q]), CTRL, 0xF, 0xF, true));
     }
 }
-__device__ __forceinline__ void pair_pass_reduce(float (&s1)[2], float (&s2)[2]) {
-    pair_pass_dpp_stage<0xB1>(s1, s2); pair_pass_dpp_stage<0x4E>(s1, s2); pair_pass_dpp_stage<0x141>(s1, s2);
+template <int NQ> __device__ __forceinline__ void pair_pass_reduce(float (&s1)[NQ], float (&s2)[NQ]) {
+    pair_pass_dpp_stage<0xB1, NQ>(s1, s2); pair_pass_dpp_stage<0x4E, NQ>(s1, s2); pair_pass_dpp_stage<0x141, NQ>(s1, s2);
 }
 
 template <int DT, int MT, int MODE, int PA, int PW0, int PW1, typename Issue1, typename Issue2>
diff --git a/hgr-net_amd/csrc/hgr_gemm_rows.hip b/hgr-net_amd/csrc/hgr_gemm_rows.hip
--- /dev/null
+++ b/hgr-net_amd/csrc/hgr_gemm_rows.hip
@@ -0,0 +1,204 @@
+#include "hgr_gemm_common.h"
+#include "hgr_launch.h"
+
+namespace hgr_gemm {
+namespace {
+
+constexpr int RW_NT = 256, RW_BM = 32, RW_BN = 64;
+constexpr int RW_AHEAD = 4, RW_NS = RW_AHEAD + 1;
+constexpr int RW_PA = 0, RW_PW = RW_BM * 128;
+constexpr int RW_STAGE = (RW_BM + RW_BN) * 128;
+constexpr int RW_LDS = RW_NS * RW_STAGE;
+constexpr int RW_DMA = RW_STAGE / (RW_NT * 16);
+enum { RW_LN = 0, RW_LN_GELU = 1, RW_RES = 2 };
+static_assert(RW_DMA == 3 && RW_DMA * (RW_AHEAD - 1) <= 63, "the counted waits below assume 3 instructions per K-tile");
+
+struct RowsArgs {
+    const char *A; int64_t lda;
+    const char *W; int64_t ldw;
+    int M, N, K, tiles_m, tiles_n;
+    void *C; int64_t ldc;
+    const float *ln_s, *ln_c, *stats_in; int64_t stats_mul; float eps;
+    void *xh, *xl; int64_t ldx;
+    const float *bias; float *stats_out;
+    unsigned *flag; float guard;
+};
+
+template <int DT, int MODE>
+__global__ __launch_bounds__(RW_NT, 2) void gemm_nt_rows(RowsArgs p) {
+    typedef typename T16<DT>::vec8 vec8;
+    __shared__ __attribute__((aligned(1024))) char smem[RW_LDS];
+    const int tid = threadIdx.x;
+    const int lane = tid & 63;
+    const int wave = __builtin_amdgcn_readfirstlane(tid >> 6);
+    const int r = lane & 15, g = lane >> 4;
+
+    const int ntiles = p.tiles_m * p.tiles_n;
+    const int wg = xcd_first_tile(ntiles, (int)blockIdx.x & 7) + ((int)blockIdx.x >> 3);
+    const int m0 = (wg % p.tiles_m) * RW_BM, n0 = (wg / p.tiles_m) * RW_BN;
+
+    unsigned oA, oW[2];
+    {
+        const int pr = wave * 8 + (lane >> 3), c = (lane & 7) ^ (pr & 7);
+        oA = (unsigned)(((int64_t)min(m0 + pr, p.M - 1) * p.lda + c * 8) * 2);
+#pragma unroll
+        for (int i = 0; i < 2; ++i) oW[i] = (unsigned)(((int64_t)min(n0 + i * 32 + pr, p.N - 1) * p.ldw + c * 8) * 2);
+    }
+    char *const ldsw = smem + wave * 1024;
+    const __amdgpu_buffer_rsrc_t rA = dma_rsrc(p.A), rW = dma_rsrc(p.W);
+    auto issue = [&](int t, int stage) {
+        char *dst = ldsw + stage * RW_STAGE;
+        dma16(rA, oA, t * 128, dst + RW_PA);
+        dma16(rW, oW[0], t * 128, dst + RW_PW);
+        dma16(rW, oW[1], t * 128, dst + RW_PW + 4096);
+    };
+
+    f32x4 acc[2];
+    acc[0] = acc[1] = (f32x4){0.f, 0.f, 0.f, 0.f};
+    const int nk = p.K / BK;
+    const int offA = r * 128, offW = (wave * 16 + r) * 128;
+    const int sw0 = ((0 + g) ^ (r & 7)) * 16, sw1 = ((4 + g) ^ (r & 7)) * 16;
+
+    for (int t = 0; t < RW_AHEAD && t < nk; ++t) issue(t, t);
+    int rs = 0, is = RW_AHEAD;
+    for (int t = 0; t < nk; ++t) {
+        const int newer = min(RW_AHEAD - 1, nk - 1 - t);
+        if (newer == 3) rwait<3 * RW_DMA>(); else if (newer == 2) rwait<2 * RW_DMA>(); else if (newer == 1) rwait<RW_DMA>(); else rwait<0>();
+        if (t + RW_AHEAD < nk) issue(t + RW_AHEAD, is);
+        const char *st = smem + rs * RW_STAGE;
+        vec8 wf[2], af[2][2];
+        wf[0] = *(const vec8 *)(st + RW_PW + offW + sw0);
+        wf[1] = *(const vec8 *)(st + RW_PW + offW + sw1);
+#pragma unroll
+        for (int i = 0; i < 2; ++i) {
+            af[i][0] = *(const vec8 *)(st + RW_PA + offA + i * 2048 + sw0);
+            af[i][1] = *(const vec8 *)(st + RW_PA + offA + i * 2048 + sw1);
+        }
+#pragma unroll
+        for (int kk = 0; kk < 2; ++kk)
+#pragma unroll
+            for (int i = 0; i < 2; ++i) acc[i] = T16<DT>::mfma16(wf[kk], af[i][kk], acc[i]);
+        rs = rs == RW_NS - 1 ? 0 : rs + 1;
+        is = is == RW_NS - 1 ? 0 : is + 1;
+    }
+    HGR_RBAR();
+
+    const int row = tid >> 3, c8 = tid & 7;
+    const int m = m0 + row;
+    const bool ok = m < p.M;
+    const int mc = min(m, p.M - 1);
+    if constexpr (MODE != RW_RES) {
+        float2 *lnrow = (float2 *)smem;
+        char *outst = smem + 1024;
+        constexpr int RS = 144;
+        const int slots = p.K / 64;
+        if (tid < RW_BM) {
+            const f32x4 *sp = (const f32x4 *)(p.stats_in + (int64_t)min(m0 + tid, p.M - 1) * p.stats_mul * slots * 2);
+            float s1, s2;
+            ln_row_sums(sp, slots, s1, s2);
+            lnrow[tid] = ln_finalize(s1, s2, 1.0f / (float)p.K, p.eps);
+        }
+        const int n = n0 + wave * 16 + g * 4;
+        const f32x4 sq = *(const f32x4 *)(p.ln_s + n), cq = *(const f32x4 *)(p.ln_c + n);
+        __syncthreads();
+#pragma unroll
+        for (int i = 0; i < 2; ++i)
+            *(u32x2 *)(outst + (i * 16 + r) * RS + (wave * 16 + g * 4) * 2) = ln_out16<DT, MODE == RW_LN_GELU>(lnrow[i * 16 + r], acc[i], sq, cq);
+        __syncthreads();
+        if (ok) *(u32x4 *)((char *)p.C + ((int64_t)m * p.ldc + n0 + c8 * 8) * 2) = *(const u32x4 *)(outst + row * RS + c8 * 16);
+    } else {
+        constexpr int RS = 272;
+#pragma unroll
+        for (int i = 0; i < 2; ++i) *(f32x4 *)(smem + (i * 16 + r) * RS + (wave * 16 + g * 4) * 4) = acc[i];
+        char *hp = (char *)p.xh + ((int64_t)mc * p.ldx + n0 + c8 * 8) * 2;
+        char *lp = (char *)p.xl + ((int64_t)mc * p.ldx + n0 + c8 * 8);
+        const u32x4 ohb = *(const u32x4 *)hp;
+        const u32x2 ol = *(const u32x2 *)lp;
+        const f32x4 b8lo = *(const f32x4 *)(p.bias + n0 + c8 * 8), b8hi = *(const f32x4 *)(p.bias + n0 + c8 * 8 + 4);
+        __syncthreads();
+        const f32x4 lo4 = *(const f32x4 *)(smem + row * RS + c8 * 32);
+        const f32x4 hi4 = *(const f32x4 *)(smem + row * RS + c8 * 32 + 16);
+        float v[8];
+        pair_pass_values<DT>(lo4, hi4, b8lo, b8hi, __builtin_bit_cast(vec8, ohb), ol, v);
+        u32x4 nh;
+        u32x2 nl;
+        pair_pass_split<DT>(v, nh, nl);
+        if (ok) {
+            *(u32x4 *)hp = nh;
+            *(u32x2 *)lp = nl;
+        }
+        float s1[1], s2[1];
+        pair_pass_sums(v, s1[0], s2[0]);
+        pair_pass_reduce(s1, s2);
+        if (c8 == 0 && ok) {
+            *(float2 *)(p.stats_out + ((int64_t)m * (p.N >> 6) + (n0 >> 6)) * 2) = make_float2(s1[0], s2[0]);
+            const unsigned gbits = __float_as_uint(s2[0]);
+            if (p.flag && gbits > __float_as_uint(p.guard)) atomicMax(p.flag, gbits);
+        }
+    }
+}
+
+const char *rows_reject(int64_t M, int64_t N, int64_t K, int64_t lda, int64_t ldw, int64_t ldo, int dtype) {
+    if (dtype != HGR_BF16 && dtype != HGR_F16) return "bad dtype";
+    if (M < 1 || M > 2048) return "M must be in [1, 2048]";
+    if (N < 64 || N % 64 || N >= (1 << 20)) return "N must be a multiple of 64 below 2^20 (a tile owns whole 64-column statistic slots)";
+    if (K < 64 || K % 64) return "K must be a multiple of 64";
+    if (lda < K || ldw < K || lda % 8 || ldw % 8) return "lda / ldw must be >= K and multiples of 8";
+    if (ldo < N || ldo % 8 || ldo >= (1 << 23)) return "the output's leading dimension must be >= N, a multiple of 8 and < 2^23";
+    if (M * lda * 2 >= (1ll << 32) || N * ldw * 2 >= (1ll << 32)) return "operands beyond 4 GB";
+    return nullptr;
+}
+
+template <int MODE> void rows_launch(RowsArgs &a, int dtype, void *stream) {
+    a.tiles_m = (a.M + RW_BM - 1) / RW_BM; a.tiles_n = a.N / RW_BN;
+    const dim3 grid((unsigned)(a.tiles_m * a.tiles_n)), block(RW_NT);
+    hgr_by_dtype(dtype, [&](auto dt) { hipLaunchKernelGGL((gemm_nt_rows<dt.value, MODE>), grid, block, 0, (hipStream_t)stream, a); });
+}
+}
+}
+
+using namespace hgr_gemm;
+
+extern "C" int hgr_gemm_nt_ln_rows_ok(int64_t M, int64_t N, int64_t K, int64_t ldx, int64_t ldw, int64_t ldc, int64_t stats_mul, int dtype) {
+    if (rows_reject(M, N, K, ldx, ldw, ldc, dtype)) return 0;
+    return K % 128 == 0 && stats_mul >= 1 && stats_mul < (1 << 20) ? 1 : 0;
+}
+
+extern "C" int hgr_gemm_nt_ln_rows(const void *XH, int64_t ldx, const void *Wfold, int64_t ldw, void *C, int64_t ldc,
+                                   const float *ln_s, const float *ln_c, const float *stats, int64_t stats_mul, float eps,
+                                   int M, int N, int K, int dtype, int act, void *stream) {
+    const char *why = rows_reject(M, N, K, ldx, ldw, ldc, dtype);
+    HGR_REQUIRE(!why, "hgr_gemm_nt_ln_rows: M=%d N=%d K=%d ldx=%lld ldw=%lld ldc=%lld dtype=%d: %s", M, N, K, (long long)ldx, (long long)ldw, (long long)ldc, dtype, why);
+    HGR_REQUIRE(K % 128 == 0 && stats_mul >= 1 && stats_mul < (1 << 20), "hgr_gemm_nt_ln_rows: the row width K=%d must be a multiple of 128, stats_mul=%lld in [1, 2^20)", K, (long long)stats_mul);
+    HGR_REQUIRE(XH && Wfold && C && ln_s && ln_c && stats, "hgr_gemm_nt_ln_rows: null operand");
+    HGR_REQUIRE(hgr_aligned(XH, 16) && hgr_aligned(Wfold, 16) && hgr_aligned(C, 16) && hgr_aligned(ln_s, 16) && hgr_aligned(ln_c, 16) && hgr_aligned(stats, 16),
+                "hgr_gemm_nt_ln_rows: XH, Wfold, C, ln_s, ln_c and stats must be 16-byte aligned");
+    HGR_REQUIRE(act == 0 || act == 1, "hgr_gemm_nt_ln_rows: act must be 0 (none) or 1 (QuickGELU), got %d", act);
+    RowsArgs a = {};
+    a.A = (const char *)XH; a.lda = ldx; a.W = (const char *)Wfold; a.ldw = ldw; a.M = M; a.N = N; a.K = K;
+    a.C = C; a.ldc = ldc; a.ln_s = ln_s; a.ln_c = ln_c; a.stats_in = stats; a.stats_mul = stats_mul; a.eps = eps;
+    if (act) rows_launch<RW_LN_GELU>(a, dtype, stream); else rows_launch<RW_LN>(a, dtype, stream);
+    HGR_CHECK_LAUNCH("hgr_gemm_nt_ln_rows");
+    return HGR_OK;
+}
+
+extern "C" int hgr_gemm_nt_res_stats_rows_ok(int64_t M, int64_t N, int64_t K, int64_t lda, int64_t ldw, int64_t ldx, int dtype) {
+    return rows_reject(M, N, K, lda, ldw, ldx, dtype) == nullptr ? 1 : 0;
+}
+
+extern "C" int hgr_gemm_nt_res_stats_rows(const void *A, int64_t lda, const void *W, int64_t ldw, void *xh, void *xl, int64_t ldx,
+                                          const float *bias, float *stats, float guard_sumsq, uint32_t *flag,
+                                          int M, int N, int K, int dtype, void *stream) {
+    const char *why = rows_reject(M, N, K, lda, ldw, ldx, dtype);
+    HGR_REQUIRE(!why, "hgr_gemm_nt_res_stats_rows: M=%d N=%d K=%d lda=%lld ldw=%lld ldx=%lld dtype=%d: %s", M, N, K, (long long)lda, (long long)ldw, (long long)ldx, dtype, why);
+    HGR_REQUIRE(A && W && xh && xl && bias && stats, "hgr_gemm_nt_res_stats_rows: null operand");
+    HGR_REQUIRE(!flag || (guard_sumsq > 0.f && hgr_aligned(flag, 4)), "hgr_gemm_nt_res_stats_rows: flag needs guard_sumsq > 0 and 4-byte alignment");
+    HGR_REQUIRE(hgr_aligned(A, 16) && hgr_aligned(W, 16) && hgr_aligned(xh, 16) && hgr_aligned(xl, 16) && hgr_aligned(bias, 16) && hgr_aligned(stats, 8),
+                "hgr_gemm_nt_res_stats_rows: A, W, xh, xl and bias must be 16-byte, stats 8-byte aligned");
+    RowsArgs a = {};
+    a.A = (const char *)A; a.lda = lda; a.W = (const char *)W; a.ldw = ldw; a.M = M; a.N = N; a.K = K;
+    a.xh = xh; a.xl = xl; a.ldx = ldx; a.bias = bias; a.stats_out = stats; a.flag = flag; a.guard = guard_sumsq;
+    rows_launch<RW_RES>(a, dtype, stream);
+    HGR_CHECK_LAUNCH("hgr_gemm_nt_res_stats_rows");
+    return HGR_OK;
+}
diff --git a/hgr-net_amd/csrc/hgr_norm.hip b/hgr-net_amd/csrc/hgr_norm.hip
--- a/hgr-net_amd/csrc/hgr_norm.hip
+++ b/hgr-net_amd/csrc/hgr_norm.hip
@@ -141,6 +141,35 @@
             const f32x4 o = v[i] * inv;
             if (y32) ((f32x4 *)(y32 + (int64_t)row * D))[c] = o;
             if (y16) ((typename T16<DT>::vec4 *)((typename T16<DT>::elem *)y16 + (int64_t)row * D))[c] = cvt4<DT>(o[0], o[1], o[2], o[3]);
+        }
+    }
+}
+
+template <int DT, int NV>
+__global__ __launch_bounds__(256) void l2norm_rows_rep(const float *__restrict__ x, void *__restrict__ y16, int64_t ldy, int rows, int D, int rep) {
+    const int lane = threadIdx.x & 63;
+    const int row = blockIdx.x * 4 + (threadIdx.x >> 6);
+    if (row >= rows) return;
+    const f32x4 *xr = (const f32x4 *)(x + (int64_t)row * D);
+    const int nv = D >> 2;
+    f32x4 v[NV];
+    float s = 0.f;
+#pragma unroll
+    for (int i = 0; i < NV; ++i) {
+        const int c = i * 64 + lane;
+        if (i * 64 < nv) {
+            v[i] = (c < nv) ? xr[c] : (f32x4){0.f, 0.f, 0.f, 0.f};
+            s += v[i][0] * v[i][0] + v[i][1] * v[i][1] + v[i][2] * v[i][2] + v[i][3] * v[i][3];
+        }
+    }
+    const float inv = 1.0f / sqrtf(wave_sum(s));
+#pragma unroll
+    for (int i = 0; i < NV; ++i) {
+        const int c = i * 64 + lane;
+        if (i * 64 < nv && c < nv) {
+            const f32x4 o = v[i] * inv;
+            const typename T16<DT>::vec4 h = cvt4<DT>(o[0], o[1], o[2], o[3]);
+            for (int j = 0; j < rep; ++j) ((typename T16<DT>::vec4 *)((typename T16<DT>::elem *)y16 + (int64_t)row * ldy + (int64_t)j * D))[c] = h;
         }
     }
 }
@@ -285,6 +314,19 @@
     return HGR_OK;
 }
 
+extern "C" int hgr_l2norm_rows_rep(const float *x, void *y16, int64_t ldy, int rows, int D, int rep, int dtype, void *stream) {
+    HGR_REQUIRE(x && y16, "hgr_l2norm_rows_rep: null operand");
+    HGR_REQUIRE(rows >= 1 && D >= 4 && D % 4 == 0 && D <= 4 * 64 * MAXV, "hgr_l2norm_rows_rep: rows=%d D=%d unsupported", rows, D);
+    HGR_REQUIRE(rep >= 1 && rep <= 8 && ldy >= (int64_t)rep * D && ldy % 4 == 0, "hgr_l2norm_rows_rep: rep=%d must be in [1, 8], ldy=%lld >= rep * D and a multiple of 4", rep, (long long)ldy);
+    HGR_REQUIRE(hgr_aligned(x, 16) && hgr_aligned(y16, 8), "hgr_l2norm_rows_rep: misaligned operand");
+    HGR_REQUIRE(dtype == HGR_BF16 || dtype == HGR_F16, "hgr_l2norm_rows_rep: bad dtype %d", dtype);
+    dim3 grid((rows + 3) / 4), block(256);
+    hgr_by_nv_pow2((D / 4 + 63) / 64, [&](auto nv) { hgr_by_dtype(dtype, [&](auto dt) {
+        hipLaunchKernelGGL((l2norm_rows_rep<dt.value, nv.value>), grid, block, 0, (hipStream_t)stream, x, y16, ldy, rows, D, rep); }); });
+    HGR_CHECK_LAUNCH("hgr_l2norm_rows_rep");
+    return HGR_OK;
+}
+
 
 extern "C" int hgr_vit_embed_ln_stats(const float *patches, const float *class_embedding, const float *positional_embedding,
                                       const float *gamma, const float *beta, void *xh, void *xl, float *stats,
diff --git a/hgr-net_amd/model/clip_tree.py b/hgr-net_amd/model/clip_tree.py
--- a/hgr-net_amd/model/clip_tree.py
+++ b/hgr-net_amd/model/clip_tree.py
@@ -290,10 +290,9 @@
                 f32 = torch.empty_like(feats)
                 ops.l2norm_rows(feats, y16=f16, y32=f32)
                 second = (f32 - f16.float()).to(f16.dtype)
+                fin = torch.cat([f16, second], dim=1)
             else:
-                ops.l2norm_rows(feats, y16=f16)
-                second = f16
-            fin = torch.cat([f16, second], dim=1)
+                fin = ops.l2norm_rows_rep(feats, torch.empty((b, 2 * feats.shape[1]), dtype=f16.dtype, device=feats.device), 2)
         else:
             ops.l2norm_rows(feats, y16=f16)
             fin, zc = f16, (self._zsl16 if mode is None else zc)
diff --git a/hgr-net_amd/ops.py b/hgr-net_amd/ops.py
--- a/hgr-net_amd/ops.py
+++ b/hgr-net_amd/ops.py
@@ -132,6 +132,50 @@
     _prof_end(ev, 2.0 * m * n * k, 2 * m * k + 2 * n * k + 6 * m * n + 8 * m * (n // 64), tag)
 
 
+def gemm_nt_res_stats_rows_ok(m: int, n: int, k: int, lda: int, ldw: int, ldx: int, dtype) -> bool:
+    code = dtype if isinstance(dtype, int) else DT_OF.get(dtype, -1)
+    return bool(_lib.load().hgr_gemm_nt_res_stats_rows_ok(int(m), int(n), int(k), int(lda), int(ldw), int(ldx), int(code)))
+
+
+ROWS_CALLS = [0]
+
+
+def gemm_nt_res_stats_rows(a: torch.Tensor, w: torch.Tensor, xh: torch.Tensor, xl: torch.Tensor, bias: torch.Tensor, stats: torch.Tensor,
+                           tag: str = "", flag: Optional[torch.Tensor] = None) -> None:
+    m, k = a.shape
+    n = w.shape[0]
+    assert a.dtype == w.dtype == xh.dtype and xl.dtype == PAIR_LO and xh.shape == xl.shape == (m, n) and xh.stride() == xl.stride()
+    assert stats.dtype == torch.float32 and stats.numel() >= m * (n // 64) * 2 and a.stride(1) == w.stride(1) == xh.stride(1) == 1
+    assert flag is None or (flag.numel() == 1 and flag.element_size() == 4)
+    ev = _prof_begin()
+    _lib.call("hgr_gemm_nt_res_stats_rows", _dev(a), a.stride(0), _dev(w), w.stride(0), _dev(xh), _dev(xl), xh.stride(0), _dev(bias),
+              _dev(stats), LN_GUARD_SUMSQ if flag is not None else 0.0, _dev(flag), m, n, k, DT_OF[a.dtype], _stream())
+    if not _lib.muted():
+        ROWS_CALLS[0] += 1
+    _prof_end(ev, 2.0 * m * n * k, 2 * m * k + 2 * n * k + 6 * m * n + 8 * m * (n // 64), tag)
+
+
+def gemm_nt_ln_rows_ok(m: int, n: int, k: int, ldx: int, ldw: int, ldc: int, stats_mul: int, dtype) -> bool:
+    code = dtype if isinstance(dtype, int) else DT_OF.get(dtype, -1)
+    return bool(_lib.load().hgr_gemm_nt_ln_rows_ok(int(m), int(n), int(k), int(ldx), int(ldw), int(ldc), int(stats_mul), int(code)))
+
+
+def gemm_nt_ln_rows(x16: torch.Tensor, wfold: torch.Tensor, out: torch.Tensor, ln_s: torch.Tensor, ln_c: torch.Tensor, stats: torch.Tensor,
+                    eps: float = 1e-5, quickgelu: bool = False, stats_mul: int = 1, tag: str = "") -> torch.Tensor:
+    m, k = x16.shape
+    n = wfold.shape[0]
+    assert x16.dtype == wfold.dtype == out.dtype and out.shape[0] == m and out.shape[1] >= n and ln_s.numel() == n and ln_c.numel() == n
+    assert x16.stride(1) == wfold.stride(1) == out.stride(1) == 1 and stats.dtype == torch.float32 and stats.is_contiguous()
+    assert stats_mul >= 1 and stats.numel() >= ((m - 1) * stats_mul + 1) * (k // 64) * 2
+    ev = _prof_begin()
+    _lib.call("hgr_gemm_nt_ln_rows", _dev(x16), x16.stride(0), _dev(wfold), wfold.stride(0), _dev(out), out.stride(0), _dev(ln_s), _dev(ln_c),
+              _dev(stats), int(stats_mul), float(eps), m, n, k, DT_OF[x16.dtype], 1 if quickgelu else 0, _stream())
+    if not _lib.muted():
+        ROWS_CALLS[0] += 1
+    _prof_end(ev, 2.0 * m * n * k, 2 * m * k + 2 * n * k + 2 * m * n, tag)
+    return out
+
+
 def gemm_nt_bias_gelu_dual(a: torch.Tensor, w: torch.Tensor, pre: torch.Tensor, post: torch.Tensor, bias: torch.Tensor) -> None:
     assert a.dim() == 2 and w.dim() == 2 and a.dtype == w.dtype == pre.dtype == post.dtype and a.stride(1) == w.stride(1) == pre.stride(1) == post.stride(1) == 1
     m, k = a.shape
@@ -372,6 +416,13 @@
     assert x.dtype == torch.float32 and x.is_contiguous()
     dt = DT_OF[y16.dtype] if y16 is not None else HGR_BF16
     _lib.call("hgr_l2norm_rows", _dev(x), _dev(y16), _dev(y32), x.shape[0], x.shape[1], dt, _stream())
+
+
+def l2norm_rows_rep(x: torch.Tensor, y16: torch.Tensor, rep: int) -> torch.Tensor:
+    assert x.dtype == torch.float32 and x.is_contiguous() and y16.dim() == 2 and y16.stride(1) == 1
+    assert y16.shape[0] == x.shape[0] and y16.shape[1] >= rep * x.shape[1]
+    _lib.call("hgr_l2norm_rows_rep", _dev(x), _dev(y16), y16.stride(0), x.shape[0], x.shape[1], int(rep), DT_OF[y16.dtype], _stream())
+    return y16
 
 
 def topk_rows(logits: torch.Tensor, k: int, cols: Optional[torch.Tensor] = None, n_cols: Optional[int] = None,
diff --git a/include/hgr.h b/include/hgr.h
--- a/include/hgr.h
+++ b/include/hgr.h
@@ -67,6 +67,7 @@
 int hgr_eot_index(const int64_t *tokens, int64_t ld_tokens, int32_t *eot, int n, int ctx, void *stream);
 
 int hgr_l2norm_rows(const float *x, void *y16, float *y32, int rows, int D, int dtype, void *stream);
+int hgr_l2norm_rows_rep(const float *x, void *y16, int64_t ldy, int rows, int D, int rep, int dtype, void *stream);
 
 int hgr_topk_rows(const float *logits, int64_t ld, const int32_t *cols, int n_cols, int k,
                   int32_t *out_idx, float *out_val, int rows, void *stream);
@@ -285,6 +286,15 @@
 int hgr_gemm_nt_res_stats_wide(const void *A, int64_t lda, const void *W, int64_t ldw, void *xh, void *xl, int64_t ldx,
                                const float *bias, float *stats, float guard_sumsq, uint32_t *flag,
                                int M, int N, int K, int dtype, void *stream);
+
+int hgr_gemm_nt_res_stats_rows_ok(int64_t M, int64_t N, int64_t K, int64_t lda, int64_t ldw, int64_t ldx, int dtype);
+int hgr_gemm_nt_res_stats_rows(const void *A, int64_t lda, const void *W, int64_t ldw, void *xh, void *xl, int64_t ldx,
+                               const float *bias, float *stats, float guard_sumsq, uint32_t *flag,
+                               int M, int N, int K, int dtype, void *stream);
+int hgr_gemm_nt_ln_rows_ok(int64_t M, int64_t N, int64_t K, int64_t ldx, int64_t ldw, int64_t ldc, int64_t stats_mul, int dtype);
+int hgr_gemm_nt_ln_rows(const void *XH, int64_t ldx, const void *Wfold, int64_t ldw, void *C, int64_t ldc,
+                        const float *ln_s, const float *ln_c, const float *stats, int64_t stats_mul, float eps,
+                        int M, int N, int K, int dtype, int act, void *stream);
 
 int hgr_vit_head(const void *xh, const void *xl, int64_t ldx, int64_t row_mul, const float *gamma, const float *beta, float eps,
                  const void *proj_t, float *out, int B, int W, int D, int dtype, void *stream);
```

Result: no change. 109,700 (-0.3%).
